# HKUST-Aerial-Robotics/MIND

Measured on AMD Instinct MI355X. Metric: sim steps/sec (whole node) + scenario-tree nodes expanded/sec, AV2 demo scenes, higher is better.
Workload: dtype f32-class (bf16 hi+mid+lo split operands = 24 significand bits, six products, fp32 accumulate) pair kernel + ActorNet, f32 elsewhere in the predictor, f64 iLQR

## Files before the change

### include/mind_hip.h

```cpp
#ifndef MIND_HIP_H
#define MIND_HIP_H

#include <stddef.h>
#include <stdint.h>

#ifdef __cplusplus
extern "C" {
#endif

#define MIND_OK 0
#define MIND_EINVAL (-1)
#define MIND_ENOMEM (-2)
#define MIND_EHIP (-3)
#define MIND_ESTATE (-4)
#define MIND_ENOTFOUND (-5)

typedef struct mind_ctx mind_ctx;

int mind_ctx_create(int device, void *stream, mind_ctx **out);
int mind_ctx_destroy(mind_ctx *ctx);
const char *mind_last_error_string(mind_ctx *ctx);
int mind_ctx_synchronize(mind_ctx *ctx);

typedef struct {
  const char *name;
  const float *data;
  int64_t numel;
} mind_tensor_desc;

int mind_weights_load(mind_ctx *ctx, const mind_tensor_desc *tensors, int n_tensors);

typedef struct {
  int n_scenes;
  const int32_t *actor_off;
  const int32_t *lane_off;
  const float *actors;
  const float *lanes;
  const float *lane_feat;
  const float *actor_ctrs;
  const float *actor_vecs;
  const float *lane_ctrs;
  const float *lane_vecs;
  const float *const *rpe;
  const float *tgt_nodes;
  const float *tgt_rpe;
} mind_scene_batch;

typedef struct {
  float *cls;
  float *reg;
  float *vel;
  float *lane_feat;
  float *actor_emb;
  float *cls_emb;
} mind_pred_out;

int mind_predict_batch(mind_ctx *ctx, const mind_scene_batch *in, mind_pred_out *out);

typedef struct {
  float *cov_vel;
  float *param;
} mind_pred_aux;
int mind_predict_batch_aux(mind_ctx *ctx, const mind_scene_batch *in, mind_pred_out *out, const mind_pred_aux *aux);

#define MIND_BASIS_BEZIER 0
#define MIND_BASIS_MONOMIAL 1
int mind_set_decoder_basis(mind_ctx *ctx, int basis);
int mind_get_decoder_basis(mind_ctx *ctx);

#define MIND_CURVE_MAX_POINTS (1LL << 26)
int mind_curve_eval(mind_ctx *ctx, int basis, const float *param, long long n_rows, const double *tau, int n_tau,
                    float *reg, float *vel, float *cov_vel);
int mind_debug_curve_basis(int basis, const double *tau, int n_tau, float *T, float *Tp);

int mind_last_fusion_stats(mind_ctx *ctx, int *n_launches, float *total_ms, double *pairs_processed);
int mind_last_actor_stats(mind_ctx *ctx, int *layerwise, int *n_launches, int *n_chunks, float *total_ms);
int mind_last_token_stats(mind_ctx *ctx, int *layerwise, int *n_launches, int *n_chunks, float *total_ms);
int mind_last_token_stage_ms(mind_ctx *ctx, float *out_ms, int cap);
int mind_last_ilqr_stats(mind_ctx *ctx, float *kernel_ms, int *n_trees, int *workgroups_per_tree);
int mind_last_ilqr_profile(mind_ctx *ctx, double *out9);
int mind_last_ilqr_trace(mind_ctx *ctx, int tree, int phase, double *out, int cap_rows, int *n_rows);
int mind_set_profiling(mind_ctx *ctx, int enable);
int mind_debug_launch_times(mind_ctx *ctx, int kind, float *clock_ms, float *event_ms, int cap, int *n_clock, int *n_event);
int mind_debug_launch_clock(int n_blocks, int block_slots, int rate_khz, const long long *ops, int n_ops, const unsigned long long *stamps,
                            long long n_slots, double *out, int cap);

#define MIND_PAIR_F32 0
#define MIND_PAIR_BF16X3 1
#define MIND_PAIR_BF16 2
#define MIND_PAIR_BF16X6 3
int mind_set_pair_precision(mind_ctx *ctx, int mode);

int mind_set_tuning(mind_ctx *ctx, const char *name, int value);
int mind_get_tuning(mind_ctx *ctx, const char *name, int *value);
int mind_debug_tuning(int index, const char *name, const char *text, int value, const char **out_name, const char **out_env, int *out_value);
int mind_debug_live_handles(void);
int mind_get_pair_precision(mind_ctx *ctx);
int mind_debug_pack_bfrag(const float *w, int row_stride, uint32_t *out);

int mind_debug_pair_schedule(const int *scene_tokens, const int *scene_actors, int n_scenes, int n_cu, int last_layer, int *out_jobs, int cap,
                             int *out_info);

int mind_debug_predict_choice(const char *const *knob_names, const int *knob_values, int n_knobs, int pair_prec, int n_cu, int have_side,
                              const int *scene_actors, const int *scene_lanes, int n_scenes, long long *out, int cap);

int mind_debug_ilqr_plan(const char *const *knob_names, const int *knob_values, int n_knobs, int n_cu, int mode, int n_trees, const int *n_nodes,
                         const int32_t *parents, long long *out, int cap, int *bad);

int mind_debug_aime_book(int pred_len, int max_depth, int max_rounds, int n_agents, int world, int rank, int force, int n_rounds, const int *dec_len,
                         const float *dec, int n_tokens, int bytes_per_pair, int plan_chunk_mb, int per_scene, long long *out, int cap, char *msg,
                         int msg_cap);

int mind_debug_wait_word(const unsigned *word, unsigned want, double timeout_s, double (*clock)(void *user), void *user, int spins_per_look);

int mind_debug_actor_lw_plan(int n_actors, int np, int chunk, long long *out_launches, int cap, long long *out_info);

int mind_debug_token_lw_plan(int n_tokens, int mode, int chunk, long long *out_launches, int cap, long long *out_info);

int mind_debug_pack_conv_frag(const float *w, int co, int ci, int ksz, uint32_t *out, size_t cap);

int mind_debug_pack(const char *what, const float *w, int a, int b, int c, float *out, size_t cap);
int mind_debug_weight_image(const mind_tensor_desc *tensors, int n_tensors, float *blob, size_t blob_cap, char *names, size_t names_cap,
                            long long *entries, int entries_cap, long long *out_info, char *msg, int msg_cap);
int mind_debug_weight_bind(const mind_tensor_desc *tensors, int n_tensors, const char *drop, char *msg, int msg_cap);

int mind_debug_trig(mind_ctx *ctx, const double *x, int n, double *out);

int mind_debug_set_layers(mind_ctx *ctx, int n);
int64_t mind_debug_read(mind_ctx *ctx, const char *name, float *host, int64_t max_floats);

typedef struct {
  int n_nodes;
  const int32_t *parent;
  const float *prob;
  int n_agents;
  const float *agent_mean;
  const float *agent_cov;
  const double *field;
  const double *node_w;
} mind_cost_tree;

typedef struct {
  double dt, wheelbase;
  double w_des_state[6];
  double w_state_con[6];
  double state_lower[6], state_upper[6];
  double w_ctrl[2];
  double w_tgt, w_ego, w_ego_cov_offset, w_exo, w_exo_cov_offset, w_exo_cost_offset;
  double grid_res; int grid_w, grid_h;
  int max_iter;
} mind_ilqr_cfg;

typedef struct { int iterations; int converged; double J; double mu; } mind_ilqr_stats;

int mind_ilqr_solve_trees(mind_ctx *ctx, const mind_ilqr_cfg *cfg, const mind_cost_tree *trees,
                          int n_trees, const double *x0, const double *target_lane, int n_lane_pts,
                          double target_vel, int use_exo, const double *us_init, double *xs,
                          double *us, mind_ilqr_stats *stats);

int mind_ilqr_contingency(mind_ctx *ctx, const mind_ilqr_cfg *cfg_warm, const mind_ilqr_cfg *cfg_full,
                          const mind_cost_tree *trees, int n_trees, const double *x0,
                          const double *target_lane, int n_lane_pts, double target_vel, double *xs,
                          double *us, mind_ilqr_stats *stats_warm, mind_ilqr_stats *stats_full);
int mind_ilqr_contingency_begin(mind_ctx *ctx, const mind_ilqr_cfg *cfg_warm, const mind_ilqr_cfg *cfg_full,
                                const mind_cost_tree *trees, int n_trees, const double *x0,
                                const double *target_lane, int n_lane_pts, double target_vel, double *xs,
                                double *us, mind_ilqr_stats *stats_warm, mind_ilqr_stats *stats_full);
int mind_ilqr_contingency_begin_plan(mind_ctx *ctx, const mind_ilqr_cfg *cfg_warm, const mind_ilqr_cfg *cfg_full, const double *x0,
                                     const double *target_lane, int n_lane_pts, double target_vel, double *xs, double *us,
                                     mind_ilqr_stats *stats_warm, mind_ilqr_stats *stats_full);
int mind_ilqr_finish(mind_ctx *ctx);

typedef struct {
  int n_scenes;
  const int32_t *actor_off;
  const float *reg, *vel;
  const float *actor_ctrs, *actor_vecs;
  const float *rot, *orig;
  const float *cov_last;
  const int32_t *last;
  const float *target_lane;
  int n_lane_pts;
  const float *cls;
  const float *scen_prob;
  int lane_check;
  float dist_thres;
} mind_world_in;

typedef struct {
  float *world;
  float *topo;
  float *ego_end;
  float *sel, *sel_prob;
} mind_world_out;

int mind_aime_world(mind_ctx *ctx, const mind_world_in *in, const mind_world_out *out);

int mind_debug_aime_decide(mind_ctx *ctx, int n_scenes, const int32_t *actor_off, const int32_t *cmp, const float *cls, const float *scen_prob,
                           const float *topo, const float *ego_end, const float *world, int lane_check, float dist_thres, float prob_floor,
                           int fused, int by_value, float *sel, float *sel_prob, uint32_t *hit);

typedef struct {
  int n_scenes, n_agents, n_lanes;
  const float *pos, *ang, *vel;
  const float *types;
  const float *pad;
  const float *lane_ctrs, *lane_vecs;
  const float *target_lane;
  const float *target_lane_info;
  int n_lane_pts;
  float time_ahead, min_vel;
// ... 303 lines not shown
```

### mind_amd/_lib.py

```python
import ctypes as C
import os

_HERE = os.path.dirname(os.path.abspath(__file__))
LIB_PATH = os.environ.get("MIND_HIP_LIB", os.path.join(_HERE, "libmind_hip.so"))

WAIT_CLOCK = C.CFUNCTYPE(C.c_double, C.c_void_p)
MIND_OK = 0
MIND_EINVAL, MIND_ENOMEM, MIND_EHIP, MIND_ESTATE, MIND_ENOTFOUND = -1, -2, -3, -4, -5


class TensorDesc(C.Structure):
    _fields_ = [("name", C.c_char_p), ("data", C.POINTER(C.c_float)), ("numel", C.c_int64)]


class SceneBatch(C.Structure):
    _fields_ = [("n_scenes", C.c_int), ("actor_off", C.POINTER(C.c_int32)), ("lane_off", C.POINTER(C.c_int32)),
                ("actors", C.c_void_p), ("lanes", C.c_void_p), ("lane_feat", C.c_void_p),
                ("actor_ctrs", C.c_void_p), ("actor_vecs", C.c_void_p), ("lane_ctrs", C.c_void_p),
                ("lane_vecs", C.c_void_p), ("rpe", C.POINTER(C.c_void_p)), ("tgt_nodes", C.c_void_p),
                ("tgt_rpe", C.c_void_p)]


class PredOut(C.Structure):
    _fields_ = [("cls", C.c_void_p), ("reg", C.c_void_p), ("vel", C.c_void_p), ("lane_feat", C.c_void_p),
# ... 117 lines not shown


class AimeNode(C.Structure):
    _fields_ = [("round", C.c_int), ("scene", C.c_int), ("mode", C.c_int), ("parent", C.c_int), ("prob", C.c_float),
                ("cur_t", C.c_int), ("end_t", C.c_int), ("flags", C.c_int), ("dur", C.c_int), ("row_off", C.c_int64),
                ("tgt_pts", C.c_float * 22)]


class AimePlanOut(C.Structure):
    _fields_ = [("nodes", C.POINTER(AimeNode)), ("n_nodes", C.c_int), ("rows", C.POINTER(C.c_float)), ("n_row_floats", C.c_int64),
                ("n_expanded", C.c_int), ("n_rounds", C.c_int), ("root_flags", C.c_int), ("round_scenes", C.c_int * 32),
                ("pair_ms", C.c_float), ("pair_launches", C.c_int), ("n_trees", C.c_int), ("tree_top", C.POINTER(C.c_int32)),
                ("tree_off", C.POINTER(C.c_int32)), ("flat_parent", C.POINTER(C.c_int32)), ("flat_prob", C.POINTER(C.c_float)),
                ("flat_mean", C.POINTER(C.c_float)), ("flat_cov", C.POINTER(C.c_float)), ("solves_begun", C.c_int)]


class IlqrCfg(C.Structure):
    _fields_ = [("dt", C.c_double), ("wheelbase", C.c_double), ("w_des_state", C.c_double * 6),
                ("w_state_con", C.c_double * 6), ("state_lower", C.c_double * 6), ("state_upper", C.c_double * 6),
                ("w_ctrl", C.c_double * 2), ("w_tgt", C.c_double), ("w_ego", C.c_double),
                ("w_ego_cov_offset", C.c_double), ("w_exo", C.c_double), ("w_exo_cov_offset", C.c_double),
                ("w_exo_cost_offset", C.c_double), ("grid_res", C.c_double), ("grid_w", C.c_int), ("grid_h", C.c_int),
                ("max_iter", C.c_int)]


class IlqrStats(C.Structure):
    _fields_ = [("iterations", C.c_int), ("converged", C.c_int), ("J", C.c_double), ("mu", C.c_double)]


LOOP_TAN_FN = C.CFUNCTYPE(C.c_double, C.c_double)
LOOP_SINCOS_FN = C.CFUNCTYPE(None, C.c_double, C.POINTER(C.c_double))


class LoopDesc(C.Structure):
    _fields_ = [("n_tracks", C.c_int), ("n_steps", C.c_int), ("clamp_last", C.c_int), ("ego_state", C.c_void_p), ("ego_state_is_f32", C.c_int), ("ego_obs", C.c_void_p), ("ego_trig32", C.c_void_p),
                ("tan_fn", C.c_void_p), ("sincos_fn", C.c_void_p), ("exo_obs", C.c_void_p),
                ("exo_valid", C.c_void_p), ("timestep", C.c_void_p), ("type_slot", C.c_void_p),
                ("sim_step", C.c_double), ("plan_step", C.c_double), ("enable_time", C.c_double),
                ("wheelbase", C.c_double), ("max_speed", C.c_double), ("max_steer", C.c_double), ("max_acc", C.c_double), ("max_dec", C.c_double),
                ("n_lanes", C.c_int), ("lane_pts", C.c_void_p), ("lane_flags", C.c_void_p),
                ("n_lane_pts", C.c_int), ("target_lane", C.c_void_p), ("target_lane_info", C.c_void_p),
                ("time_ahead", C.c_double), ("min_vel", C.c_float), ("dist_thres", C.c_float), ("max_depth", C.c_int), ("max_rounds", C.c_int),
                ("pred_len", C.c_int), ("prob_floor", C.c_float),
                ("cfg_warm", C.c_void_p), ("cfg_full", C.c_void_p), ("solve_n_lane_pts", C.c_int), ("solve_lane", C.c_void_p), ("target_vel", C.c_double),
                ("eval_n_lane_pts", C.c_int), ("eval_lane_is_f32", C.c_int), ("eval_lane", C.c_void_p), ("speculative", C.c_int)]


class LoopTotals(C.Structure):
    _fields_ = [("plans", C.c_longlong), ("expansions", C.c_longlong), ("scen_trees", C.c_longlong), ("rounds", C.c_longlong),
                ("aime_s", C.c_double), ("ilqr_s", C.c_double), ("total_s", C.c_double),
                ("iterations", C.c_longlong), ("node_iterations", C.c_longlong), ("node_iterations_exo", C.c_longlong),
                ("warm_speculated", C.c_longlong), ("warm_hits", C.c_longlong),
                ("pair_ms", C.c_double), ("pair_launches", C.c_longlong), ("scene_n2", C.c_double), ("scene_n_a1", C.c_double),
                ("ilqr_ms", C.c_double), ("ilqr_launches", C.c_longlong), ("ilqr_trees", C.c_longlong), ("ilqr_workgroups_per_tree", C.c_int),
                ("ilqr_prof", C.c_double * 9), ("ilqr_node_steps", C.c_double)]


class LoopOut(C.Structure):
    _fields_ = [("planned", C.c_int), ("enabled", C.c_int), ("n_steps", C.c_longlong), ("n_plans", C.c_longlong), ("episode_steps", C.c_longlong),
                ("sim_time", C.c_double), ("last_trigger", C.c_double), ("state", C.c_double * 4), ("ctrl", C.c_double * 2),
                ("n_agents", C.c_int), ("n_trees", C.c_int), ("best", C.c_int), ("n_expanded", C.c_int), ("n_rounds", C.c_int), ("n_traj_nodes", C.c_int),
                ("costs", C.POINTER(C.c_double)), ("aime_s", C.c_double), ("ilqr_s", C.c_double), ("total_s", C.c_double),
                ("tot", LoopTotals)]


PLANNER_EGO_KEY = -(1 << 63)


class PlannerDesc(C.Structure):
    _fields_ = [("time_ahead", C.c_double), ("min_vel", C.c_float), ("dist_thres", C.c_float), ("max_depth", C.c_int), ("max_rounds", C.c_int),
                ("pred_len", C.c_int), ("prob_floor", C.c_float), ("cfg_warm", C.c_void_p), ("cfg_full", C.c_void_p), ("speculative", C.c_int),
                ("ego_type_slot", C.c_int)]


class PlannerOut(C.Structure):
    _fields_ = [("n_plans", C.c_longlong),
                ("n_agents", C.c_int), ("n_trees", C.c_int), ("best", C.c_int), ("n_expanded", C.c_int), ("n_rounds", C.c_int), ("n_traj_nodes", C.c_int),
                ("costs", C.POINTER(C.c_double)), ("ctrl", C.c_double * 2), ("aime_s", C.c_double), ("ilqr_s", C.c_double), ("total_s", C.c_double),
                ("tot", LoopTotals)]


EXPORTS = ["mind_ctx_create", "mind_ctx_destroy", "mind_last_error_string", "mind_ctx_synchronize",
           "mind_weights_load", "mind_predict_batch", "mind_last_fusion_stats", "mind_last_actor_stats", "mind_debug_actor_lw_plan", "mind_last_token_stats", "mind_last_token_stage_ms", "mind_debug_token_lw_plan", "mind_set_profiling", "mind_debug_launch_times", "mind_debug_launch_clock",
           "mind_ilqr_solve_trees", "mind_ilqr_contingency", "mind_ilqr_solve_fields", "mind_cost_eval", "mind_ilqr_score_trees", "mind_ilqr_gains", "mind_ilqr_policy_rollouts", "mind_lane_dist_field", "mind_aime_world", "mind_aime_rebase", "mind_debug_aime_decide", "mind_debug_set_layers",
           "mind_debug_read", "mind_set_pair_precision", "mind_get_pair_precision", "mind_debug_pack_bfrag", "mind_debug_pack_conv_frag", "mind_debug_pack", "mind_debug_weight_image", "mind_debug_weight_bind", "mind_debug_pair_schedule", "mind_debug_predict_choice", "mind_debug_ilqr_plan", "mind_debug_aime_book", "mind_set_tuning", "mind_get_tuning", "mind_debug_tuning", "mind_debug_live_handles", "mind_last_ilqr_stats", "mind_aime_plan", "mind_last_ilqr_profile", "mind_eval_traj_trees", "mind_last_ilqr_trace", "mind_ilqr_contingency_begin", "mind_ilqr_finish", "mind_fill_tracks", "mind_ilqr_contingency_begin_plan", "mind_debug_trig", "mind_aime_plan_begin", "mind_aime_plan_poll", "mind_aime_plan_finish", "mind_ctx_busy", "mind_ilqr_finish_plan",
           "mind_set_exchange", "mind_last_exchange_stats", "mind_debug_wait_word",
           "mind_predict_batch_aux", "mind_set_decoder_basis", "mind_get_decoder_basis", "mind_curve_eval", "mind_debug_curve_basis",
           "mind_audit_plan", "mind_audit_episode", "mind_debug_box_clearance",
           "mind_forecast_score", "mind_debug_forecast_score",
           "mind_audit_road_plan", "mind_audit_road_episode", "mind_debug_road_margin",
           "mind_audit_ttc", "mind_debug_box_ttc",
           "mind_loop_create", "mind_loop_destroy", "mind_loop_reset", "mind_loop_advance", "mind_loop_state", "mind_loop_last_plan", "mind_loop_export",
           "mind_planner_create", "mind_planner_destroy", "mind_planner_reset", "mind_planner_observe", "mind_planner_set_lanes", "mind_planner_set_target_lane",
           "mind_planner_set_solve_lane", "mind_planner_set_eval_lane", "mind_planner_plan", "mind_planner_last_plan", "mind_planner_export"]

EXCHANGE_FN = C.CFUNCTYPE(C.c_int, C.c_void_p, C.c_int, C.c_void_p, C.c_void_p, C.c_int64)
XCHG_ALLGATHER, XCHG_ALLREDUCE, XCHG_ALLTOALLV = 0, 1, 2

_lib = None


def load():
    global _lib
    if _lib is not None:
        return _lib
    if not os.path.exists(LIB_PATH):
        raise ImportError(f"{LIB_PATH} is missing: the HIP extension must be built (hipcc --offload-arch=gfx950); "
                          "there is no CPU fallback for the product path")
    lib = C.CDLL(LIB_PATH)
    lib.mind_ctx_create.argtypes = [C.c_int, C.c_void_p, C.POINTER(C.c_void_p)]
    lib.mind_ctx_destroy.argtypes = [C.c_void_p]
    lib.mind_last_error_string.argtypes = [C.c_void_p]
    lib.mind_last_error_string.restype = C.c_char_p
    lib.mind_ctx_synchronize.argtypes = [C.c_void_p]
    lib.mind_weights_load.argtypes = [C.c_void_p, C.POINTER(TensorDesc), C.c_int]
    lib.mind_predict_batch.argtypes = [C.c_void_p, C.POINTER(SceneBatch), C.POINTER(PredOut)]
    lib.mind_predict_batch_aux.argtypes = [C.c_void_p, C.POINTER(SceneBatch), C.POINTER(PredOut), C.POINTER(PredAux)]
    lib.mind_set_decoder_basis.argtypes = [C.c_void_p, C.c_int]
    lib.mind_get_decoder_basis.argtypes = [C.c_void_p]
    lib.mind_curve_eval.argtypes = [C.c_void_p, C.c_int, C.c_void_p, C.c_longlong, C.POINTER(C.c_double), C.c_int, C.c_void_p, C.c_void_p, C.c_void_p]
    lib.mind_debug_curve_basis.argtypes = [C.c_int, C.POINTER(C.c_double), C.c_int, C.POINTER(C.c_float), C.POINTER(C.c_float)]
    lib.mind_last_fusion_stats.argtypes = [C.c_void_p, C.POINTER(C.c_int), C.POINTER(C.c_float), C.POINTER(C.c_double)]
    lib.mind_last_actor_stats.argtypes = [C.c_void_p, C.POINTER(C.c_int), C.POINTER(C.c_int), C.POINTER(C.c_int), C.POINTER(C.c_float)]
    lib.mind_debug_actor_lw_plan.argtypes = [C.c_int, C.c_int, C.c_int, C.POINTER(C.c_longlong), C.c_int, C.POINTER(C.c_longlong)]
    lib.mind_last_token_stats.argtypes = [C.c_void_p, C.POINTER(C.c_int), C.POINTER(C.c_int), C.POINTER(C.c_int), C.POINTER(C.c_float)]
    lib.mind_last_token_stage_ms.argtypes = [C.c_void_p, C.POINTER(C.c_float), C.c_int]
    lib.mind_debug_token_lw_plan.argtypes = [C.c_int, C.c_int, C.c_int, C.POINTER(C.c_longlong), C.c_int, C.POINTER(C.c_longlong)]
    lib.mind_set_profiling.argtypes = [C.c_void_p, C.c_int]
    lib.mind_debug_launch_times.argtypes = [C.c_void_p, C.c_int, C.POINTER(C.c_float), C.POINTER(C.c_float), C.c_int, C.POINTER(C.c_int), C.POINTER(C.c_int)]
    lib.mind_debug_launch_clock.argtypes = [C.c_int, C.c_int, C.c_int, C.POINTER(C.c_longlong), C.c_int, C.POINTER(C.c_ulonglong), C.c_longlong,
                                            C.POINTER(C.c_double), C.c_int]
    lib.mind_ilqr_solve_trees.argtypes = [C.c_void_p, C.POINTER(IlqrCfg), C.POINTER(CostTree), C.c_int,
                                          C.POINTER(C.c_double), C.POINTER(C.c_double), C.c_int, C.c_double, C.c_int,
                                          C.POINTER(C.c_double), C.POINTER(C.c_double), C.POINTER(C.c_double),
                                          C.POINTER(IlqrStats)]
    lib.mind_ilqr_contingency.argtypes = [C.c_void_p, C.POINTER(IlqrCfg), C.POINTER(IlqrCfg), C.POINTER(CostTree), C.c_int,
                                          C.POINTER(C.c_double), C.POINTER(C.c_double), C.c_int, C.c_double,
                                          C.POINTER(C.c_double), C.POINTER(C.c_double), C.POINTER(IlqrStats), C.POINTER(IlqrStats)]
    lib.mind_ilqr_contingency_begin.argtypes = [C.c_void_p, C.POINTER(IlqrCfg), C.POINTER(IlqrCfg), C.POINTER(CostTree), C.c_int,
                                          C.POINTER(C.c_double), C.POINTER(C.c_double), C.c_int, C.c_double,
                                          C.POINTER(C.c_double), C.POINTER(C.c_double), C.POINTER(IlqrStats), C.POINTER(IlqrStats)]
    lib.mind_ilqr_finish.argtypes = [C.c_void_p]
    lib.mind_ilqr_contingency_begin_plan.argtypes = [C.c_void_p, C.POINTER(IlqrCfg), C.POINTER(IlqrCfg), C.c_void_p, C.c_void_p, C.c_int, C.c_double,
                                                     C.c_void_p, C.c_void_p, C.c_void_p, C.c_void_p]
    lib.mind_fill_tracks.argtypes = [C.c_void_p, C.c_int, C.c_int, C.c_void_p, C.c_void_p, C.c_void_p, C.c_void_p, C.c_void_p, C.c_void_p]
    lib.mind_ilqr_solve_fields.argtypes = [C.c_void_p, C.POINTER(IlqrCfg), C.POINTER(FieldGrid), C.POINTER(CostTree), C.c_int,
                                           C.POINTER(C.c_double), C.POINTER(C.c_double), C.POINTER(C.c_double),
                                           C.POINTER(C.c_double), C.POINTER(IlqrStats)]
    lib.mind_cost_eval.argtypes = [C.c_void_p, C.POINTER(IlqrCfg), C.POINTER(FieldGrid), C.POINTER(CostTree),
                                   C.POINTER(C.c_double), C.POINTER(C.c_double), C.c_int, C.c_double, C.c_int, C.c_int,
                                   C.POINTER(C.c_int32), C.POINTER(C.c_double), C.POINTER(C.c_double), C.POINTER(C.c_double)]
    lib.mind_ilqr_score_trees.argtypes = [C.c_void_p, C.POINTER(IlqrCfg), C.POINTER(FieldGrid), C.POINTER(CostTree), C.c_int,
                                          C.POINTER(C.c_double), C.POINTER(C.c_double), C.c_int, C.c_double, C.c_int, C.c_int,
                                          C.POINTER(C.c_double), C.POINTER(C.c_double), C.POINTER(C.c_double), C.POINTER(C.c_double)]
    lib.mind_ilqr_gains.argtypes = [C.c_void_p, C.POINTER(IlqrCfg), C.POINTER(FieldGrid), C.POINTER(CostTree), C.c_int,
                                    C.POINTER(C.c_double), C.POINTER(C.c_double), C.c_int, C.c_double, C.c_int,
                                    C.POINTER(C.c_double), C.POINTER(C.c_double), C.POINTER(IlqrGainsOut)]
    lib.mind_ilqr_policy_rollouts.argtypes = [C.c_void_p, C.POINTER(IlqrCfg), C.POINTER(FieldGrid), C.POINTER(CostTree), C.c_int,
                                              C.POINTER(C.c_double), C.POINTER(C.c_double), C.c_int, C.c_double, C.c_int,
                                              C.POINTER(C.c_double), C.POINTER(C.c_double), C.POINTER(C.c_double), C.c_int,
                                              C.POINTER(C.c_double), C.POINTER(C.c_double), C.POINTER(C.c_double), C.POINTER(C.c_double),
                                              C.POINTER(C.c_double), C.POINTER(C.c_double)]
    lib.mind_lane_dist_field.argtypes = [C.c_void_p, C.POINTER(C.c_double), C.POINTER(C.c_double), C.c_int, C.c_int, C.c_int,
                                         C.c_double] + [C.POINTER(C.c_double)] * 4
    lib.mind_aime_world.argtypes = [C.c_void_p, C.POINTER(WorldIn), C.POINTER(WorldOut)]
    lib.mind_aime_rebase.argtypes = [C.c_void_p, C.POINTER(RebaseIn), C.POINTER(RebaseOut)]
    lib.mind_debug_aime_decide.argtypes = [C.c_void_p, C.c_int, C.POINTER(C.c_int32), C.POINTER(C.c_int32), C.c_void_p, C.POINTER(C.c_float), C.c_void_p,
                                           C.c_void_p, C.c_void_p, C.c_int, C.c_float, C.c_float, C.c_int, C.c_int, C.c_void_p, C.c_void_p, C.c_void_p]
    lib.mind_aime_plan.argtypes = [C.c_void_p, C.POINTER(AimePlanIn), C.POINTER(AimePlanOut)]
    lib.mind_aime_plan_begin.argtypes = [C.c_void_p, C.POINTER(AimePlanIn)]
    lib.mind_aime_plan_poll.argtypes = [C.c_void_p]
    lib.mind_aime_plan_finish.argtypes = [C.c_void_p, C.POINTER(AimePlanOut)]
    lib.mind_ctx_busy.argtypes = [C.c_void_p]
    lib.mind_ilqr_finish_plan.argtypes = [C.c_void_p, C.c_int, C.c_int, C.c_void_p, C.c_void_p, C.c_void_p, C.c_void_p]
    lib.mind_set_pair_precision.argtypes = [C.c_void_p, C.c_int]
    lib.mind_set_tuning.argtypes = [C.c_void_p, C.c_char_p, C.c_int]
    lib.mind_get_tuning.argtypes = [C.c_void_p, C.c_char_p, C.POINTER(C.c_int)]
    lib.mind_debug_tuning.argtypes = [C.c_int, C.c_char_p, C.c_char_p, C.c_int, C.POINTER(C.c_char_p), C.POINTER(C.c_char_p), C.POINTER(C.c_int)]
    lib.mind_debug_live_handles.argtypes = []
    lib.mind_last_ilqr_stats.argtypes = [C.c_void_p, C.POINTER(C.c_float), C.POINTER(C.c_int), C.POINTER(C.c_int)]
    lib.mind_last_ilqr_profile.argtypes = [C.c_void_p, C.POINTER(C.c_double)]
    lib.mind_last_ilqr_trace.argtypes = [C.c_void_p, C.c_int, C.c_int, C.POINTER(C.c_double), C.c_int, C.POINTER(C.c_int)]
    lib.mind_eval_traj_trees.argtypes = [C.POINTER(C.c_double), C.POINTER(C.c_double), C.POINTER(C.c_int32), C.c_int, C.c_void_p, C.c_int, C.c_int,
                                         C.c_double, C.POINTER(C.c_double)]
    lib.mind_get_pair_precision.argtypes = [C.c_void_p]
    lib.mind_debug_pack_bfrag.argtypes = [C.POINTER(C.c_float), C.c_int, C.POINTER(C.c_uint32)]
    lib.mind_debug_pair_schedule.argtypes = [C.POINTER(C.c_int), C.POINTER(C.c_int), C.c_int, C.c_int, C.c_int, C.POINTER(C.c_int), C.c_int, C.POINTER(C.c_int)]
    lib.mind_debug_predict_choice.argtypes = [C.POINTER(C.c_char_p), C.POINTER(C.c_int), C.c_int, C.c_int, C.c_int, C.c_int, C.POINTER(C.c_int), C.POINTER(C.c_int),
                                              C.c_int, C.POINTER(C.c_longlong), C.c_int]
    lib.mind_debug_ilqr_plan.argtypes = [C.POINTER(C.c_char_p), C.POINTER(C.c_int), C.c_int, C.c_int, C.c_int, C.c_int, C.POINTER(C.c_int), C.POINTER(C.c_int32),
                                         C.POINTER(C.c_longlong), C.c_int, C.POINTER(C.c_int)]
    lib.mind_debug_wait_word.argtypes = [C.POINTER(C.c_uint), C.c_uint, C.c_double, WAIT_CLOCK, C.c_void_p, C.c_int]
    lib.mind_debug_aime_book.argtypes = [C.c_int] * 8 + [C.POINTER(C.c_int), C.POINTER(C.c_float)] + [C.c_int] * 4 + [C.POINTER(C.c_longlong), C.c_int, C.c_char_p, C.c_int]
    lib.mind_debug_trig.argtypes = [C.c_void_p, C.POINTER(C.c_double), C.c_int, C.POINTER(C.c_double)]
    lib.mind_debug_pack_conv_frag.argtypes = [C.POINTER(C.c_float), C.c_int, C.c_int, C.c_int, C.POINTER(C.c_uint32), C.c_size_t]
    lib.mind_debug_pack.argtypes = [C.c_char_p, C.POINTER(C.c_float), C.c_int, C.c_int, C.c_int, C.POINTER(C.c_float), C.c_size_t]
    lib.mind_debug_weight_image.argtypes = [C.POINTER(TensorDesc), C.c_int, C.POINTER(C.c_float), C.c_size_t, C.c_char_p, C.c_size_t,
                                            C.POINTER(C.c_longlong), C.c_int, C.POINTER(C.c_longlong), C.c_char_p, C.c_int]
    lib.mind_debug_weight_bind.argtypes = [C.POINTER(TensorDesc), C.c_int, C.c_char_p, C.c_char_p, C.c_int]
    lib.mind_debug_set_layers.argtypes = [C.c_void_p, C.c_int]
    lib.mind_debug_read.argtypes = [C.c_void_p, C.c_char_p, C.POINTER(C.c_float), C.c_int64]
    lib.mind_set_exchange.argtypes = [C.c_void_p, C.c_int, C.c_int, EXCHANGE_FN, C.c_void_p, C.c_int]
    lib.mind_last_exchange_stats.argtypes = [C.c_void_p, C.POINTER(C.c_longlong), C.POINTER(C.c_longlong)]
    lib.mind_loop_create.argtypes = [C.c_void_p, C.POINTER(LoopDesc), C.POINTER(C.c_void_p)]
    lib.mind_loop_destroy.argtypes = [C.c_void_p]
    lib.mind_loop_reset.argtypes = [C.c_void_p]
    lib.mind_loop_advance.argtypes = [C.c_void_p, C.c_int, C.c_double, C.c_longlong, C.POINTER(LoopOut)]
    lib.mind_loop_state.argtypes = [C.c_void_p, C.POINTER(LoopOut)]
    lib.mind_loop_last_plan.argtypes = [C.c_void_p, C.POINTER(AimePlanOut)] + [C.POINTER(C.c_void_p)] * 6 + [C.c_void_p]
    lib.mind_loop_export.argtypes = [C.c_void_p, C.c_int, C.POINTER(C.c_int), C.c_void_p, C.c_void_p, C.c_void_p]
    lib.mind_planner_create.argtypes = [C.c_void_p, C.POINTER(PlannerDesc), C.POINTER(C.c_void_p)]
    lib.mind_planner_destroy.argtypes = [C.c_void_p]
    lib.mind_planner_reset.argtypes = [C.c_void_p]
    lib.mind_planner_observe.argtypes = [C.c_void_p, C.c_int, C.c_void_p, C.c_int, C.c_void_p, C.c_void_p, C.c_void_p]
    lib.mind_planner_set_lanes.argtypes = [C.c_void_p, C.c_int, C.c_void_p, C.c_void_p]
    lib.mind_planner_set_target_lane.argtypes = [C.c_void_p, C.c_int, C.c_void_p, C.c_void_p]
    lib.mind_planner_set_solve_lane.argtypes = [C.c_void_p, C.c_int, C.c_void_p, C.c_double]
    lib.mind_planner_set_eval_lane.argtypes = [C.c_void_p, C.c_int, C.c_void_p, C.c_int]
    lib.mind_planner_plan.argtypes = [C.c_void_p, C.c_void_p, C.c_void_p, C.POINTER(PlannerOut)]
    lib.mind_planner_last_plan.argtypes = [C.c_void_p, C.POINTER(AimePlanOut)] + [C.POINTER(C.c_void_p)] * 6 + [C.c_void_p]
    lib.mind_planner_export.argtypes = [C.c_void_p, C.c_int, C.POINTER(C.c_int), C.c_void_p, C.c_void_p, C.c_void_p]
    lib.mind_audit_plan.argtypes = [C.c_void_p, C.POINTER(AuditBox), C.c_double, C.POINTER(CostTree), C.c_int, C.c_int, C.POINTER(C.c_double),
                                    C.POINTER(AuditPlanOut)]
    lib.mind_audit_episode.argtypes = [C.c_void_p, C.POINTER(AuditBox), C.c_int, C.c_int, C.c_int, C.POINTER(C.c_double), C.POINTER(C.c_double),
                                       C.POINTER(C.c_uint8), C.POINTER(C.c_double), C.POINTER(AuditEpisodeOut)]
    lib.mind_debug_box_clearance.argtypes = [C.c_int, C.c_int, C.POINTER(C.c_double), C.POINTER(C.c_double), C.POINTER(C.c_double), C.POINTER(C.c_double)]
    fc_tail = [C.POINTER(ForecastCfg), C.c_int, C.POINTER(C.c_int32), C.c_void_p, C.c_void_p, C.POINTER(C.c_double), C.POINTER(C.c_uint8),
               C.POINTER(C.c_uint8), C.POINTER(ForecastOut)]
    lib.mind_forecast_score.argtypes = [C.c_void_p] + fc_tail
    lib.mind_debug_forecast_score.argtypes = fc_tail
    road = [C.POINTER(C.c_double), C.POINTER(C.c_int32), C.c_int]
    lib.mind_audit_road_plan.argtypes = [C.c_void_p, C.POINTER(AuditBox)] + road + [C.POINTER(CostTree), C.c_int, C.c_int, C.POINTER(C.c_double),
                                                                                   C.POINTER(AuditRoadPlanOut)]
    lib.mind_audit_road_episode.argtypes = [C.c_void_p, C.POINTER(AuditBox)] + road + [C.c_int, C.c_int, C.POINTER(C.c_double),
                                                                                      C.POINTER(AuditRoadEpisodeOut)]
    lib.mind_debug_road_margin.argtypes = [C.c_int, C.POINTER(C.c_double), C.POINTER(AuditBox)] + road + [C.POINTER(C.c_double), C.POINTER(C.c_double)] + \
        [C.POINTER(C.c_int32)] * 3
    lib.mind_audit_ttc.argtypes = [C.c_void_p, C.POINTER(AuditBox), C.POINTER(AuditTtcCfg), C.c_int, C.c_int, C.c_int, C.POINTER(C.c_double),
                                   C.POINTER(C.c_double), C.POINTER(C.c_uint8), C.POINTER(C.c_double), C.POINTER(AuditTtcOut)]
    lib.mind_debug_box_ttc.argtypes = [C.c_int, C.POINTER(C.c_double), C.POINTER(C.c_double), C.POINTER(C.c_double), C.POINTER(C.c_double)]
    for n in EXPORTS:
        getattr(lib, n)
        if n not in ("mind_last_error_string", "mind_debug_read"):
            getattr(lib, n).restype = C.c_int
    lib.mind_debug_read.restype = C.c_int64
    _lib = lib
    return lib


PRED_CHOICE_FIELDS = ("header", "n_runs", "np", "actor_form", "actor_arg", "actor_grid", "actor_chunk", "actor_chunks", "actor_launches", "qsplit", "qk_stride",
                      "tiled", "edge_bf16", "edge_pair_bytes", "tok_chunk", "tok_lw", "tok_chunks", "pair_family", "pair_np", "l5_jobs5", "xcd_lanes",
                      "xcd_lanes5", "dec_actor", "dec_np", "fp32_dec", "split_dec", "want_mw", "mw_blocks", "cls_on_side", "tgt_wait_first",
                      "dec_head_ra")
PAIR_PREC = ("f32", "bf16x3", "bf16", "bf16x6")


def predict_choice(knobs, prec, scenes, n_cu=256, have_side=True):
    lib = load()
    names = (C.c_char_p * max(1, len(knobs)))(*[k.encode() for k in knobs])
    vals = (C.c_int * max(1, len(knobs)))(*[int(v) for v in knobs.values()])
    sa = (C.c_int * len(scenes))(*[a for a, _ in scenes])
    sl = (C.c_int * len(scenes))(*[l for _, l in scenes])
    cap = 32 + 6 * len(scenes)
    out = (C.c_longlong * cap)()
    n = lib.mind_debug_predict_choice(names, vals, len(knobs), PAIR_PREC.index(prec) if isinstance(prec, str) else prec, n_cu, int(have_side),
                                      sa, sl, len(scenes), out, cap)
    if n == MIND_EINVAL:
        return None
    assert 0 < n <= cap and out[0] == 32 and n == 32 + 6 * out[1], n
    d = dict(zip(PRED_CHOICE_FIELDS, out[:31]))
    d["runs"] = [tuple(out[32 + 6 * i:38 + 6 * i]) for i in range(out[1])]
    return d


def knobs():
    lib = load()
    name, env, val = C.c_char_p(), C.c_char_p(), C.c_int()
    rows = []
    while not rows or len(rows) < n:
        n = lib.mind_debug_tuning(len(rows), None, None, 0, C.byref(name), C.byref(env), C.byref(val))
        assert n > 0, n
        rows.append((name.value.decode(), env.value.decode() if env.value else None, val.value))
    return rows


def knob_stored(name, value=None, text=None):
    val = C.c_int()
    rc = load().mind_debug_tuning(-1, name.encode(), None if text is None else text.encode(), 0 if value is None else int(value), None, None, C.byref(val))
    return val.value if rc == MIND_OK else None


ILQR_PLAN_FIELDS = ("header", "n_trees", "form", "G", "GS", "spec", "nslot", "grid", "workgroups_per_tree", "host_out", "early", "starve_followers")
ILQR_TREE_FIELDS = ("M", "nl", "nseg", "nsl", "maxls", "nfs")
ILQR_TREE_TABLES = ("level_start", "level_nodes", "child_start", "child_list", "seg_start", "seg_nodes", "slevel_start", "slevel_segs", "seg_rec",
                    "fstep_start", "fstep_items", "fstep_q1", "fstep_nstart", "fstep_nodes")


def ilqr_plan(knobs, parents, n_cu=256, generic=False, evaluate=False, two_fits=False):
    lib = load()
    names = (C.c_char_p * max(1, len(knobs)))(*[k.encode() for k in knobs])
    vals = (C.c_int * max(1, len(knobs)))(*[int(v) for v in knobs.values()])
    nn = (C.c_int * len(parents))(*[len(p) for p in parents])
    flat = [int(v) for p in parents for v in p]
    par = (C.c_int32 * max(1, len(flat)))(*flat)
    bad = (C.c_int * 2)()
    mode = int(generic) | int(evaluate) << 1 | int(two_fits) << 2
    n = lib.mind_debug_ilqr_plan(names, vals, len(knobs), n_cu, mode, len(parents), nn, par, None, 0, bad)
    if n == MIND_EINVAL:
        return {"bad": (bad[0], bad[1])} if bad[0] >= 0 else None
    out = (C.c_longlong * n)()
    assert lib.mind_debug_ilqr_plan(names, vals, len(knobs), n_cu, mode, len(parents), nn, par, out, n, bad) == n and out[0] == 16
    d = dict(zip(ILQR_PLAN_FIELDS, out[:12]))
    d["trees"], o = [], 16
    for _ in parents:
        tr = dict(zip(ILQR_TREE_FIELDS, out[o:o + 6]))
        lens, o = out[o + 6:o + 20], o + 20
        for name, ln in zip(ILQR_TREE_TABLES, lens):
            tr[name], o = list(out[o:o + ln]), o + ln
        d["trees"].append(tr)
    assert o == n
    return d


AIME_ROUND_FIELDS = ("B", "lo", "hi", "Bmax", "chunk", "S", "s0", "Sm", "any")
AIME_NODE_FIELDS = ("round", "scene", "mode", "parent", "prob", "cur_t", "end_t", "flags", "dur", "row_off", "owner", "lscene")


def aime_book(pred_len, max_depth, n_agents, rounds, world=1, rank=0, force=False, max_rounds=32, n_tokens=0, bytes_per_pair=512, plan_chunk_mb=96 * 1024,
              per_scene=1):
    import numpy as np
    lib = load()
    arrs = [np.ascontiguousarray(r, np.float32).ravel() for r in rounds]
    lens = (C.c_int * max(1, len(arrs)))(*[a.size for a in arrs])
    dec = np.concatenate(arrs + [np.zeros(1, np.float32)])
    msg = C.create_string_buffer(256)
    args = [pred_len, max_depth, max_rounds, n_agents, world, rank, int(force), len(arrs), lens, dec.ctypes.data_as(C.POINTER(C.c_float)), n_tokens,
            bytes_per_pair, plan_chunk_mb, per_scene]
    n = lib.mind_debug_aime_book(*args, None, 0, msg, 256)
    if n == MIND_EINVAL:
        return None
    out = (C.c_longlong * n)()
    assert lib.mind_debug_aime_book(*args, out, n, msg, 256) == n and out[0] == 16
    o, take = [16], lambda k: (list(out[o[0]:o[0] + k]), o.__setitem__(0, o[0] + k))[0]
    d = dict(code=out[1], error=msg.value.decode() if out[1] else None, args=(out[2], out[3]), n_rows=out[8], root_flags=out[9], rounds=[])
    for _ in range(out[4]):
        r = dict(zip(AIME_ROUND_FIELDS, take(9)))
        for k, ln in (("todo", r["S"]), ("cnt_r", world), ("s0_r", world + 1), ("win", 3 * r["Sm"]), ("tab", 2 * world), ("snd", 2 * world), ("rcv", 2 * world)):
            r[k] = take(ln)
        d["rounds"].append(r)
    if not out[1]:
        d["nodes"] = [dict(zip(AIME_NODE_FIELDS, take(12))) for _ in range(out[5])]
        for name in ("gather", "flat"):
            nj, nb, nbytes = take(3)
            d[name] = dict(jobs=[tuple(take(5)) for _ in range(nj)], job_of_block=take(nb), agent_of_block=take(nb), bytes=nbytes)
        d["tree_top"], d["tree_off"], d["flat_parent"], d["flat_prob"] = take(out[6]), take(out[6] + 1), take(out[7]), take(out[7])
    assert o[0] == n
    return d


def tensor_descs(sd):
    import numpy as np
    descs = (TensorDesc * max(1, len(sd)))()
    keep = []
    for i, (k, v) in enumerate(sd.items()):
        a = np.ascontiguousarray(v.detach().cpu().numpy() if hasattr(v, "detach") else np.asarray(v), dtype=np.float32)
        keep.append(a)
        descs[i].name = k.encode()
        descs[i].data = a.ctypes.data_as(C.POINTER(C.c_float))
        descs[i].numel = a.size
    return descs, keep


def weight_image(sd):
    import numpy as np
    lib = load()
    descs, keep = tensor_descs(sd)
    msg = C.create_string_buffer(256)
    info = (C.c_longlong * 3)()
    rc = lib.mind_debug_weight_image(descs, len(sd), None, 0, None, 0, None, 0, info, msg, 256)
    if rc == MIND_ENOTFOUND:
        raise KeyError(msg.value.decode())
    assert rc == MIND_OK, rc
    ne, nf, nb = info
    blob, names, ents = np.zeros(nf, np.float32), C.create_string_buffer(nb), (C.c_longlong * (2 * ne))()
    assert lib.mind_debug_weight_image(descs, len(sd), blob.ctypes.data_as(C.POINTER(C.c_float)), nf, names, nb, ents, ne, info, msg, 256) == MIND_OK
    keys = names.value.decode().split("\n")[:-1]
    assert len(keys) == ne
    return blob, [(k, ents[2 * i], ents[2 * i + 1]) for i, k in enumerate(keys)]


def curve_basis(basis, tau):
    import numpy as np
    lib = load()
    tau = np.ascontiguousarray(tau, np.float64).ravel()
    b = BASIS.index(basis) if isinstance(basis, str) else int(basis)
    T, Tp = np.zeros((max(1, tau.size), 8), np.float32), np.zeros((max(1, tau.size), 7), np.float32)
    rc = lib.mind_debug_curve_basis(b, tau.ctypes.data_as(C.POINTER(C.c_double)), tau.size, T.ctypes.data_as(C.POINTER(C.c_float)),
                                    Tp.ctypes.data_as(C.POINTER(C.c_float)))
    if rc == MIND_EINVAL:
        raise ValueError(f"mind_debug_curve_basis rejects basis {basis!r}, tau {tau!r}")
    assert rc == MIND_OK, rc
    return T[:tau.size], Tp[:tau.size]

# ... 161 lines not shown
```

### mind_amd/csrc/ilqr_choice.h

```cpp
#pragma once
#include <algorithm>
#include <cstdint>
#include <cstring>
#include <vector>

#include "tuning.h"

struct IlqrChoice {
  int form = 0;
  int G = 1, GS = 1, spec = 0;
  int nslot = IL_SPEC;
  int grid = 0;
  int wgs_per_tree = 1;
  bool host_out = false;
  bool early = false;
  bool starve_followers = false;
};

static IlqrChoice il_choose(const IlqrTuning &t, int n_cu, int n_trees, int max_nodes, long total_nodes, bool gen, bool eval) {
  IlqrChoice ch;
  const int blocks8 = ((n_trees + 7) / 8) * 8;
  int G = t.ilqr_wgs;
  if (G > 1 && G < t.ilqr_wgs_big && max_nodes >= t.ilqr_big_min) G = t.ilqr_wgs_big;
  while (G > 1 && blocks8 * G > n_cu) G >>= 1;
  const bool multi = !gen && !eval && G > 1 && max_nodes >= t.ilqr_multi_min;
  int GS = (multi || gen || eval || t.ilqr_wgs <= 1) ? 1 : t.ilqr_slots;
  while (GS > 1 && blocks8 * GS > n_cu) --GS;
  const bool slots = GS > 1;
  ch.form = multi ? 1 : slots ? 2 : 0;
  ch.G = multi ? G : 1;
  ch.GS = GS;
  ch.spec = slots && t.ilqr_spec_deriv && GS < 31 && blocks8 * (GS + 1) <= n_cu ? 1 : 0;
  ch.nslot = slots ? std::max(GS, IL_SPEC) : IL_SPEC;
  ch.grid = ch.form == 2 ? blocks8 * (GS + ch.spec) : ch.form == 1 ? blocks8 * G - (t.ilqr_test_starve ? 8 : 0) : n_trees;
  ch.wgs_per_tree = ch.form == 1 ? G : ch.form == 2 ? GS + ch.spec : 1;
  ch.starve_followers = ch.form == 2 && t.ilqr_test_starve;
  ch.host_out = !eval && t.ilqr_host_out_max > 0 && total_nodes <= t.ilqr_host_out_max;
  ch.early = ch.host_out && !multi && !gen;
  return ch;
}

static int il_score_block(const IlqrTuning &t, int n_cu, int n_trees, int n_cand) {
  if (t.ilqr_score_block > 0) return t.ilqr_score_block;
  int cb = 64;
  while (cb > 4 && (long)n_trees * ((n_cand + cb - 1) / cb) < 2L * n_cu) cb >>= 1;
  return cb;
}

struct IlTables {
  std::vector<int> lvl_start, lvl_nodes;
  std::vector<int> child_start, child_list;
  std::vector<int> seg_start, seg_nodes;
  std::vector<int> slvl_start, slvl_segs;
  std::vector<int> seg_rec;
  std::vector<int> fs_start, fs_items, fs_q1, fs_nstart, fs_nodes;
  int nl = 0, nseg = 0, nsl = 0, maxls = 0, nfs = 0;
  std::vector<int> depth, fill, child_fill, seg_of, seg_depth, slvl_fill;
};

static int il_tree_tables(const int32_t *parent, int M, int ilqr_chunk, IlTables &out) {
  IlTables &T = out;
  T.depth.assign(M, 0);
  int maxd = 0;
  for (int i = 0; i < M; ++i) {
    const int p = parent[i];
    if (i == 0 ? p != -1 : (p < 0 || p >= i)) return i;
    T.depth[i] = i == 0 ? 0 : T.depth[p] + 1;
    maxd = std::max(maxd, T.depth[i]);
  }
  T.nl = maxd + 1;
  T.lvl_start.assign(maxd + 2, 0);
  for (int i = 0; i < M; ++i) T.lvl_start[T.depth[i] + 1]++;
  for (int d = 0; d <= maxd; ++d) T.lvl_start[d + 1] += T.lvl_start[d];
  T.lvl_nodes.resize(M);
  T.fill.assign(maxd + 1, 0);
  for (int i = 0; i < M; ++i) T.lvl_nodes[T.lvl_start[T.depth[i]] + T.fill[T.depth[i]]++] = i;
  T.child_start.assign(M + 1, 0);
  for (int i = 1; i < M; ++i) T.child_start[parent[i] + 1]++;
  for (int i = 0; i < M; ++i) T.child_start[i + 1] += T.child_start[i];
  T.child_list.assign(M > 1 ? M : 1, 0);
  T.child_fill.assign(M, 0);
  for (int i = 1; i < M; ++i) T.child_list[T.child_start[parent[i]] + T.child_fill[parent[i]]++] = i;
  const auto nchild = [&T](int i) { return T.child_start[i + 1] - T.child_start[i]; };
  T.seg_of.assign(M, -1); T.seg_depth.clear();
  T.seg_start.clear(); T.seg_nodes.clear();
  for (int i = 0; i < M; ++i) {
    if (!(i == 0 || nchild(parent[i]) >= 2)) continue;
    const int sidx = (int)T.seg_start.size();
    T.seg_start.push_back((int)T.seg_nodes.size());
    T.seg_depth.push_back(i == 0 ? 0 : T.seg_depth[T.seg_of[parent[i]]] + 1);
    for (int n = i;; n = T.child_list[T.child_start[n]]) {
      T.seg_of[n] = sidx;
      T.seg_nodes.push_back(n);
      if (nchild(n) != 1) break;
    }
  }
  T.seg_start.push_back((int)T.seg_nodes.size());
  const int nseg = (int)T.seg_depth.size();
  int maxsd = 0;
  for (int d : T.seg_depth) maxsd = std::max(maxsd, d);
  T.slvl_start.assign(maxsd + 2, 0);
  for (int d : T.seg_depth) T.slvl_start[d + 1]++;
  for (int d = 0; d <= maxsd; ++d) T.slvl_start[d + 1] += T.slvl_start[d];
  T.slvl_segs.resize(nseg);
  T.slvl_fill.assign(maxsd + 1, 0);
  for (int s = 0; s < nseg; ++s) T.slvl_segs[T.slvl_start[T.seg_depth[s]] + T.slvl_fill[T.seg_depth[s]]++] = s;
  T.nseg = nseg; T.nsl = maxsd + 1;
  T.maxls = 1;
  for (int d = 0; d <= maxsd; ++d) T.maxls = std::max(T.maxls, T.slvl_start[d + 1] - T.slvl_start[d]);
  T.seg_rec.assign((size_t)nseg * 16, 0);
  for (int s = 0; s < nseg; ++s) {
    int *r = T.seg_rec.data() + (size_t)s * 16;
    const int s0 = T.seg_start[s], s1 = T.seg_start[s + 1], last = T.seg_nodes[s1 - 1];
    r[0] = s0; r[1] = s1; r[2] = last; r[3] = T.seg_nodes[s0]; r[4] = T.seg_nodes[s1 - 2 >= s0 ? s1 - 2 : s1 - 1];
    r[5] = nchild(last); r[6] = T.child_start[last];
    for (int e = 0; e < 6 && e < r[5]; ++e) r[8 + e] = T.child_list[T.child_start[last] + e];
  }
  const int chunk = (ilqr_chunk > 0 && T.maxls <= 6) ? ilqr_chunk : M;
  T.fs_start.assign(1, 0); T.fs_nstart.assign(1, 0);
  T.fs_items.clear(); T.fs_q1.clear(); T.fs_nodes.clear();
  for (int d = 0; d <= maxsd; ++d) {
    int maxlen = 0;
    for (int e = T.slvl_start[d]; e < T.slvl_start[d + 1]; ++e) { const int s = T.slvl_segs[e]; maxlen = std::max(maxlen, T.seg_start[s + 1] - T.seg_start[s]); }
    for (int k0 = 0; k0 < maxlen; k0 += chunk) {
      for (int e = T.slvl_start[d]; e < T.slvl_start[d + 1]; ++e) {
        const int s = T.slvl_segs[e], q0 = T.seg_start[s] + k0, q1 = std::min(T.seg_start[s + 1], q0 + chunk);
        if (q0 >= q1) continue;
        const int c0 = T.seg_nodes[q0], c1 = T.seg_nodes[q0 + 1 < q1 ? q0 + 1 : q1 - 1];
        for (int v : {q0, q1, c0, c1, c0 == 0 ? -1 : (int)parent[c0], 0, 0, 0}) T.fs_items.push_back(v);
        T.fs_q1.push_back(q1);
        for (int q = q0; q < q1; ++q) T.fs_nodes.push_back(T.seg_nodes[q]);
      }
      T.fs_start.push_back((int)T.fs_q1.size()); T.fs_nstart.push_back((int)T.fs_nodes.size());
    }
  }
  T.nfs = (int)T.fs_start.size() - 1;
  return -1;
}

struct IlTreeOff {
  size_t us, nodew, xs, stats, trace;
  size_t relag, Fx, L, Lx, Lxx, relag2, Fx2, L2, Lx2, Lxx2;
  size_t k, K, Vx, Vxx, xsn, usn, Ln;
  size_t prob, mean, cov;
  size_t parent, lnodes, cstart, clist, rel, rel2, lstart, sstart, snodes, slstart, slsegs, segrec, fsstart, fsitems, fsq1, fsnstart, fsnodes;
  size_t field;
};
struct IlArena {
  size_t nd = 0, nf = 0, ni = 0, nd_in = 0;
  size_t o_gx, o_gy, o_lane, o_evx, o_evu, o_quad, o_evo;
  size_t o_scu, o_scx, o_scl, o_scj;
  size_t o_gmu, o_gk, o_gK, o_gdv, o_gvx, o_gvxx, o_gxs, o_gl, o_gj, o_gbad;
  size_t o_pk, o_pK, o_pal, o_pdx, o_pxn, o_pxs, o_pus, o_pl, o_pj;
  size_t o_evn, o_bars, o_ctl, ctl_ints;
  size_t bytesIn, bytesF, bytesI, o_structs, o_consts, o_work, total;
  std::vector<IlTreeOff> tree;
  size_t takeD(size_t n) { const size_t o = nd; nd += (n + 1) & ~(size_t)1; return o; }
  size_t takeF(size_t n) { const size_t o = nf; nf += (n + 3) & ~(size_t)3; return o; }
  size_t takeI(size_t n) { const size_t o = ni; ni += (n + 3) & ~(size_t)3; return o; }
};
struct IlShape {
  int W, H, n_lane_pts, nq;
  int n_trees;
  const int *n_agents;
  bool gen, use_exo, dev_flat;
  int trace_cap;
  int n_cand = 0;
  bool gains = false;
  int n_pol = 0, n_pol_blk = 0;
};

static void il_layout(const IlShape &s, const IlqrChoice &ch, const IlTables *tab, IlArena &A) {
  const int n_trees = s.n_trees;
  const bool spec = ch.spec != 0;
  const size_t nslot = (size_t)ch.nslot;
  A = IlArena();
  A.tree.resize(n_trees);
  const auto nodes = [tab](int t) { return tab[t].lvl_nodes.size(); };
  A.o_gx = A.takeD(s.W); A.o_gy = A.takeD(s.H); A.o_lane = A.takeD((size_t)s.n_lane_pts * 2 + 2);
  A.o_evx = A.takeD((size_t)s.nq * 6); A.o_evu = A.takeD((size_t)s.nq * 2);
  A.o_evn = A.takeI(s.nq);
  A.o_bars = A.takeI(4 * (size_t)n_trees + 4);
  A.ctl_ints = (sizeof(IlSlotCtl) + 15) / 16 * 4;
  A.o_ctl = A.takeI(ch.form == 2 ? A.ctl_ints * (size_t)n_trees : 0);
  for (int t = 0; t < n_trees; ++t) A.tree[t].us = A.takeD(2 * nodes(t));
  for (int t = 0; t < n_trees; ++t) A.tree[t].nodew = A.takeD(s.gen ? nodes(t) * IL_NW : 0);
  size_t Mtot = 0;
  for (int t = 0; t < n_trees; ++t) Mtot += nodes(t);
  const size_t n_sc = (size_t)s.n_cand * Mtot;
  A.o_scu = A.takeD(2 * n_sc);
  const size_t n_g = s.gains ? Mtot : 0, n_gt = s.gains ? (size_t)n_trees : 0, n_pm = s.n_pol > 0 ? Mtot : 0, n_po = (size_t)s.n_pol * Mtot;
  A.o_gmu = A.takeD(n_gt);
  A.o_pk = A.takeD(2 * n_pm); A.o_pK = A.takeD(12 * n_pm); A.o_pal = A.takeD((size_t)s.n_pol); A.o_pdx = A.takeD(6 * (size_t)s.n_pol);
  A.nd_in = A.nd;
  A.o_quad = A.takeD(s.gen ? 2 : (size_t)s.W * s.H); A.o_evo = A.takeD((size_t)s.nq * IL_EVAL_OUT);
  for (int t = 0; t < n_trees; ++t) A.tree[t].xs = A.takeD(6 * nodes(t));
  for (int t = 0; t < n_trees; ++t) A.tree[t].stats = A.takeD(2 * IL_NSTAT);
  for (int t = 0; t < n_trees; ++t) {
    IlTreeOff &L = A.tree[t];
    const size_t M = nodes(t), a = (size_t)s.n_agents[t];
    L.trace = A.takeD((size_t)2 * s.trace_cap * IL_TRACE_W);
    L.relag = A.takeD(s.use_exo ? M * IL_RA : 0); L.Fx = A.takeD(36 * M); L.L = A.takeD(M); L.Lx = A.takeD(6 * M); L.Lxx = A.takeD(36 * M);
    L.relag2 = A.takeD(spec && s.use_exo ? M * IL_RA : 0); L.Fx2 = A.takeD(spec ? 36 * M : 0); L.L2 = A.takeD(spec ? M : 0); L.Lx2 = A.takeD(spec ? 6 * M : 0);
    L.Lxx2 = A.takeD(spec ? 36 * M : 0);
    L.k = A.takeD(nslot * 2 * M); L.K = A.takeD(nslot * 12 * M); L.Vx = A.takeD(nslot * 6 * M); L.Vxx = A.takeD(nslot * 36 * M);
    L.xsn = A.takeD(nslot * 60 * M); L.usn = A.takeD(nslot * 20 * M); L.Ln = A.takeD(nslot * 10 * M);
    L.prob = A.takeF(M); L.mean = A.takeF(s.dev_flat ? 0 : M * a * 2); L.cov = A.takeF(s.dev_flat ? 0 : M * a);
    L.parent = A.takeI(M); L.lnodes = A.takeI(M); L.cstart = A.takeI(M + 1); L.clist = A.takeI(M); L.rel = A.takeI(M); L.rel2 = A.takeI(spec ? M : 0);
  }
  for (int t = 0; t < n_trees; ++t) {
    IlTreeOff &L = A.tree[t];
    const IlTables &T = tab[t];
    L.lstart = A.takeI(T.lvl_start.size());
    L.sstart = A.takeI(T.seg_start.size()); L.snodes = A.takeI(nodes(t)); L.slstart = A.takeI(T.slvl_start.size()); L.slsegs = A.takeI(T.slvl_segs.size());
    L.segrec = A.takeI(T.seg_rec.size());
    L.fsstart = A.takeI(T.fs_start.size()); L.fsitems = A.takeI(T.fs_items.size()); L.fsq1 = A.takeI(T.fs_q1.size());
    L.fsnstart = A.takeI(T.fs_nstart.size()); L.fsnodes = A.takeI(nodes(t));
  }
  A.o_scx = A.takeD(6 * n_sc); A.o_scl = A.takeD(n_sc); A.o_scj = A.takeD((size_t)s.n_cand * n_trees);
  A.o_gk = A.takeD(2 * n_g); A.o_gK = A.takeD(12 * n_g); A.o_gdv = A.takeD(n_g); A.o_gvx = A.takeD(6 * n_g); A.o_gvxx = A.takeD(36 * n_g);
  A.o_gxs = A.takeD(6 * n_g); A.o_gl = A.takeD(n_g); A.o_gj = A.takeD(n_gt); A.o_gbad = A.takeD(n_gt);
  A.o_pxn = A.takeD(6 * (size_t)s.n_pol_blk * n_pm); A.o_pxs = A.takeD(6 * n_po); A.o_pus = A.takeD(2 * n_po); A.o_pl = A.takeD(n_po);
  A.o_pj = A.takeD((size_t)s.n_pol * (s.n_pol > 0 ? n_trees : 0));
  A.bytesIn = A.nd_in * sizeof(double); A.bytesF = A.nf * sizeof(float); A.bytesI = A.ni * sizeof(int);
  A.o_structs = A.bytesIn + A.bytesF + A.bytesI;
  A.o_consts = (A.o_structs + (size_t)n_trees * sizeof(IlqrTreeDev) + 15) & ~(size_t)15;
  A.o_work = (A.o_consts + 2 * sizeof(IlqrConst) + 15) & ~(size_t)15;
  A.total = (A.o_work + (A.nd - A.nd_in) * sizeof(double) + 15) & ~(size_t)15;
  for (int t = 0; t < n_trees; ++t) {
    A.tree[t].field = A.total;
    if (s.gen) A.total += nodes(t) * s.W * s.H * sizeof(double);
  }
}

static void il_stage_ints(const IlTreeOff &L, const int32_t *parent, const IlTables &T, int *hI) {
  const auto put = [hI](size_t o, const std::vector<int> &v) { if (!v.empty()) memcpy(hI + o, v.data(), v.size() * sizeof(int)); };
  memcpy(hI + L.parent, parent, T.lvl_nodes.size() * sizeof(int));
  put(L.lstart, T.lvl_start); put(L.lnodes, T.lvl_nodes); put(L.cstart, T.child_start); put(L.clist, T.child_list);
  put(L.sstart, T.seg_start); put(L.snodes, T.seg_nodes); put(L.slstart, T.slvl_start); put(L.slsegs, T.slvl_segs); put(L.segrec, T.seg_rec);
  put(L.fsstart, T.fs_start); put(L.fsitems, T.fs_items); put(L.fsq1, T.fs_q1); put(L.fsnstart, T.fs_nstart); put(L.fsnodes, T.fs_nodes);
}
```

### mind_amd/csrc/ilqr_host.hip

```cpp
static void il_make_grid(int W, int H, double res, const double *ego_xy, double *gx, double *gy, double &offx, double &offy) {
  const double fsx = (double)(W - 1) * res, fsy = (double)(H - 1) * res;
  offx = ego_xy[0] - 0.5 * fsx; offy = ego_xy[1] - 0.5 * fsy;
  const double sx = fsx / (double)(W - 1), sy = fsy / (double)(H - 1);
  for (int i = 0; i < W; ++i) gx[i] = (double)i * sx + 0.0;
  gx[W - 1] = fsx;
  for (int i = 0; i < H; ++i) gy[i] = (double)i * sy + 0.0;
  gy[H - 1] = fsy;
  for (int i = 0; i < W; ++i) gx[i] += offx;
  for (int i = 0; i < H; ++i) gy[i] += offy;
}

extern "C" int mind_lane_dist_field(mind_ctx *c, const double *ego_xy, const double *lane, int n_pts, int W, int H,
                                    double res, double *offset, double *gx, double *gy, double *dist) {
  if (!c || !ego_xy || !lane || n_pts < 2 || W < 2 || H < 2 || !(res > 0) || !offset || !gx || !gy || !dist)
    return fail(c, MIND_EINVAL, "mind_lane_dist_field: bad argument");
  HIPCHK(c, hipSetDevice(c->device));
  hipStream_t st = c->stream;
  il_make_grid(W, H, res, ego_xy, gx, gy, offset[0], offset[1]);
  const size_t nd = (size_t)W + H + 2 * (size_t)n_pts + (size_t)W * H;
  int rc;
  if ((rc = ensure(c, c->ilqr_dev, nd * sizeof(double)))) return rc;
  double *d = (double *)c->ilqr_dev.p;
  HIPCHK(c, hipMemcpyAsync(d, gx, W * sizeof(double), hipMemcpyHostToDevice, st));
  HIPCHK(c, hipMemcpyAsync(d + W, gy, H * sizeof(double), hipMemcpyHostToDevice, st));
// ... 236 lines not shown

static int il_stage(mind_ctx *c, IlRun &R) {
  const IlqrCall &q = R.q;
  const IlArena &A = R.A;
  const IlqrChoice &ch = R.ch;
  const IlqrEvalReq *ev = q.ev;
  const int n_trees = q.n_trees;
  const bool gen = R.gen;
  int rc;
  if ((rc = ensure(c, c->ilqr_dev, A.total))) return rc;
  R.base = (char *)c->ilqr_dev.p;
  auto &hD = c->il_img.hD; auto &hF = c->il_img.hF; auto &hI = c->il_img.hI;
  hD.assign(A.nd_in, 0.0); hF.assign(A.nf, 0.f); hI.assign(A.ni, 0);
  memcpy(hD.data() + A.o_gx, R.gx.data(), R.W * sizeof(double));
  memcpy(hD.data() + A.o_gy, R.gy.data(), R.H * sizeof(double));
  if (R.n_lane_pts) memcpy(hD.data() + A.o_lane, q.lane, (size_t)R.n_lane_pts * 2 * sizeof(double));
  if (ev) {
    memcpy(hD.data() + A.o_evx, ev->x, (size_t)ev->nq * 6 * sizeof(double));
    memcpy(hD.data() + A.o_evu, ev->u, (size_t)ev->nq * 2 * sizeof(double));
    memcpy(hI.data() + A.o_evn, ev->node, (size_t)ev->nq * sizeof(int));
  }
  if (q.sc) memcpy(hD.data() + A.o_scu, q.sc->us_cand, (size_t)q.sc->n_cand * (size_t)R.Mtot * 2 * sizeof(double));
  if (q.ga) memcpy(hD.data() + A.o_gmu, q.ga->mu, (size_t)n_trees * sizeof(double));
  if (q.po) {
    const IlqrPolicyReq *po = q.po;
    memcpy(hD.data() + A.o_pk, po->k, (size_t)R.Mtot * 2 * sizeof(double));
    memcpy(hD.data() + A.o_pK, po->K, (size_t)R.Mtot * 12 * sizeof(double));
    memcpy(hD.data() + A.o_pal, po->alpha, (size_t)po->n_cand * sizeof(double));
    if (po->dx0) memcpy(hD.data() + A.o_pdx, po->dx0, (size_t)po->n_cand * 6 * sizeof(double));
  }
  const IlTreeOff &L0 = A.tree[0];
  R.n_xs = L0.stats - L0.xs;
  R.n_hx = R.n_xs + (size_t)2 * IL_NSTAT * n_trees; R.n_us = (size_t)R.Mtot * 2;
  if ((rc = pl_pin(c, 5, (R.n_hx + R.n_us + 2) * sizeof(double) + (size_t)n_trees * sizeof(unsigned)))) return rc;
  R.hx = c->pl_pin[5].as<double>(); R.hus = R.hx + R.n_hx;
  R.h_abort = (unsigned *)(R.hus + R.n_us);
  R.h_done = R.h_abort + 4;
  c->il_early = mind_ctx::IlEarly();
  if (ch.early) {
    c->il_gen += 1u;
    if (c->il_gen == 0u) c->il_gen = 1u;
    for (int t = 0; t < n_trees; ++t) R.h_done[t] = 0u;
    c->il_early.xs = R.hx; c->il_early.us = R.hus; c->il_early.done = R.h_done; c->il_early.gen = c->il_gen; c->il_early.n_trees = n_trees; c->il_early.nodes = R.Mtot;
  }
  float *dF = R.dF();
  int *dI = R.dI();
  R.hT.resize(n_trees);
  long moff = 0;
  for (int t = 0; t < n_trees; ++t) {
    const mind_cost_tree &tr = q.trees[t];
    const IlTreeOff &L = A.tree[t];
    const IlTables &T = c->il_tab[t];
    const size_t M = tr.n_nodes, a = R.n_agents[t];
    if (q.us_init) memcpy(hD.data() + L.us, q.us_init + moff * 2, 2 * M * sizeof(double));
    if (tr.prob) memcpy(hF.data() + L.prob, tr.prob, M * sizeof(float));
    if (gen) memcpy(hD.data() + L.nodew, tr.node_w, M * IL_NW * sizeof(double));
    if (tr.agent_mean && !gen && !R.dev_flat) memcpy(hF.data() + L.mean, tr.agent_mean, M * a * 2 * sizeof(float));
    if (tr.agent_cov && !gen && !R.dev_flat) memcpy(hF.data() + L.cov, tr.agent_cov, M * a * sizeof(float));
    il_stage_ints(L, tr.parent, T, hI.data());
    IlqrTreeDev &D = R.hT[t];
    D.M = tr.n_nodes; D.n_agents = (int)a; D.n_levels = T.nl; D.pad = 0;
    D.parent = dI + L.parent; D.level_start = dI + L.lstart; D.level_nodes = dI + L.lnodes;
    D.child_start = dI + L.cstart; D.child_list = dI + L.clist;
    D.rel = dI + L.rel;
    D.relag = R.Dp(L.relag);
    D.field = gen ? (const double *)(R.base + L.field) : nullptr;
    D.node_w = gen ? R.Dp(L.nodew) : nullptr;
    D.n_segs = T.nseg; D.n_slevels = T.nsl; D.max_level_segs = T.maxls; D.pad2 = 0;
    D.seg_start = dI + L.sstart; D.seg_nodes = dI + L.snodes; D.slevel_start = dI + L.slstart; D.slevel_segs = dI + L.slsegs; D.seg_rec = dI + L.segrec;
    D.n_fsteps = T.nfs; D.padf = 0;
    D.trace = R.trace_cap > 0 ? R.Dp(L.trace) : nullptr; D.trace_cap = R.trace_cap; D.padt = 0;
    D.fstep_start = dI + L.fsstart; D.fstep_q0 = dI + L.fsitems; D.fstep_q1 = dI + L.fsq1; D.fstep_nstart = dI + L.fsnstart; D.fstep_nodes = dI + L.fsnodes;
    D.prob = dF + L.prob; D.mean = dF + L.mean; D.cov = dF + L.cov;
    if (R.dev_flat) { D.mean = c->plan.dev_fmean + (size_t)moff * a * 2; D.cov = c->plan.dev_fcov + (size_t)moff * a; }
    D.xs = R.Dp(L.xs); D.us = R.Dp(L.us); D.Fx = R.Dp(L.Fx); D.L = R.Dp(L.L); D.Lx = R.Dp(L.Lx); D.Lxx = R.Dp(L.Lxx);
    D.k = R.Dp(L.k); D.K = R.Dp(L.K); D.Vx = R.Dp(L.Vx); D.Vxx = R.Dp(L.Vxx);
    D.xs_new = R.Dp(L.xsn); D.us_new = R.Dp(L.usn); D.L_new = R.Dp(L.Ln); D.stats = R.Dp(L.stats);
    D.ctl = ch.form == 2 ? (IlSlotCtl *)(dI + A.o_ctl + A.ctl_ints * (size_t)t) : nullptr;
    D.h_xs = ch.host_out ? R.hx + (L.xs - L0.xs) : nullptr; D.h_us = ch.host_out ? R.hus + (L.us - L0.us) : nullptr;
    D.h_stats = ch.host_out ? R.hx + (L.stats - L0.xs) : nullptr;
    D.h_done = ch.early ? R.h_done + t : nullptr; D.h_gen = c->il_gen; D.pad_h = 0;
    if (ch.early && ((L.xs - L0.xs) != (size_t)moff * 6 || (L.us - L0.us) != (size_t)moff * 2)) return fail(c, MIND_EINVAL, "tree-iLQR arena: results are not contiguous");
    D.dset = ch.spec ? (long long)L.Fx2 - (long long)L.Fx : 0; D.drel = ch.spec ? (long long)L.rel2 - (long long)L.rel : 0;
    if (ch.spec && (L.L2 - L.L != L.Fx2 - L.Fx || L.Lx2 - L.Lx != L.Fx2 - L.Fx || L.Lxx2 - L.Lxx != L.Fx2 - L.Fx || (R.use_exo && L.relag2 - L.relag != L.Fx2 - L.Fx)))
      return fail(c, MIND_EINVAL, "tree-iLQR arena: the two derivative sets are laid out differently");
    moff += (long)M;
  }
  R.field_ahead = !gen && !ev && !q.sc && !q.ga && !q.po && c->il_field_valid && c->il_field_key[0] == q.x0[0] && c->il_field_key[1] == q.x0[1] && c->il_field_key[2] == (double)R.W &&
                  c->il_field_key[3] == (double)R.H && c->il_field_key[4] == R.grid_res && c->il_field_lane.size() == 2 * (size_t)R.n_lane_pts &&
                  memcmp(c->il_field_lane.data(), q.lane, c->il_field_lane.size() * sizeof(double)) == 0;
  c->il_field_valid = false;
  double *quad = R.field_ahead ? (double *)c->il_field.p + (size_t)R.W + R.H + 2 * (size_t)R.n_lane_pts : R.Dp(A.o_quad);
  il_fill_const(R.K[0], q.cfg, R.use_exo_first, R, quad);
  if (q.cfg2) il_fill_const(R.K[1], q.cfg2, 1, R, quad);
  else R.K[1] = R.K[0];
  {
    const auto off = [&R](size_t o) { return (size_t)((const char *)R.Dp(o) - R.base); };
    c->il_dbg[0] = off(L0.L); c->il_dbg[1] = off(L0.Lx); c->il_dbg[2] = off(L0.Lxx); c->il_dbg[3] = off(L0.Fx); c->il_dbg[4] = off(L0.xs);
    c->il_dbg[5] = (size_t)q.trees[0].n_nodes;
  }
  return MIND_OK;
}

static int il_upload(mind_ctx *c, IlRun &R, hipStream_t st) {
  const IlArena &A = R.A;
  const int n_trees = R.q.n_trees;
  for (int t = 0; t < n_trees && R.gen; ++t)
    HIPCHK(c, hipMemcpyAsync(R.base + A.tree[t].field, R.q.trees[t].field, (size_t)R.q.trees[t].n_nodes * R.W * R.H * sizeof(double), hipMemcpyHostToDevice, st));
  int rc;
  if ((rc = pl_pin(c, 4, A.o_work))) return rc;
  char *up = c->pl_pin[4].as<char>();
  memset(up, 0, A.o_work);
  memcpy(up, c->il_img.hD.data(), A.bytesIn);
  if (A.bytesF) memcpy(up + A.bytesIn, c->il_img.hF.data(), A.bytesF);
  if (A.bytesI) memcpy(up + A.bytesIn + A.bytesF, c->il_img.hI.data(), A.bytesI);
  if (R.ch.starve_followers) ((unsigned *)(up + A.bytesIn + A.bytesF))[A.o_bars + 4 * (size_t)n_trees + 1] = 1u;
  memcpy(up + A.o_structs, R.hT.data(), (size_t)n_trees * sizeof(IlqrTreeDev));
  memcpy(up + A.o_consts, R.K, 2 * sizeof(IlqrConst));
  R.up = up;
  return pl_upload(c, R.base, up, A.o_work, st);
}

struct IlPending {
  hipStream_t st;
  bool gen;
  int n_trees, n_phases, use_exo, trace_cap;
  long Mtot;
  IlqrChoice ch;
  const IlqrTreeDev *dT;
  const IlqrConst *dK;
  unsigned *dBars;
  size_t il_lds, o_work;
  char *base;
  const char *up;
  const double *d_xs, *d_us;
  double *hx, *hus;
  const unsigned *h_abort;
  size_t n_xs, n_hx, n_us;
  double *xs, *us;
  mind_ilqr_stats *stats, *stats2;
  struct Tree { int M, nl, nseg, nsl, maxls, a; const double *trace; };
  std::vector<Tree> tree;
};

static void il_launch_kernel(const IlPending &P, int form) {
  const IlqrChoice &ch = P.ch;
  const int nt = P.n_trees;
  const dim3 block(IL_THREADS);
  if (P.gen) hipLaunchKernelGGL((k_ilqr<true, 0>), dim3(nt), block, P.il_lds, P.st, P.dT, P.dK, P.n_phases, nt, 1, P.dBars, 0);
  else if (form == 2) hipLaunchKernelGGL((k_ilqr<false, 2>), dim3(ch.grid), block, P.il_lds, P.st, P.dT, P.dK, P.n_phases, nt, ch.GS, P.dBars, ch.spec);
  else if (form == 1) hipLaunchKernelGGL((k_ilqr<false, 1>), dim3(ch.grid), block, P.il_lds, P.st, P.dT, P.dK, P.n_phases, nt, ch.G, P.dBars, 0);
  else hipLaunchKernelGGL((k_ilqr<false, 0>), dim3(nt), block, P.il_lds, P.st, P.dT, P.dK, P.n_phases, nt, 1, P.dBars, 0);
}

static int il_read_back(mind_ctx *c, const IlPending &P) {
  if (P.ch.host_out) return MIND_OK;
  HIPCHK(c, hipMemcpyAsync(P.hx, P.d_xs, P.n_hx * sizeof(double), hipMemcpyDeviceToHost, P.st));
  HIPCHK(c, hipMemcpyAsync(P.hus, P.d_us, P.n_us * sizeof(double), hipMemcpyDeviceToHost, P.st));
  return MIND_OK;
}

static int il_finish_run(mind_ctx *c, const IlPending &P) {
  static const bool trace = getenv("MIND_ILQR_TRACE") != nullptr;
  const int n_trees = P.n_trees, n_phases = P.n_phases;
  int rc;
  HIPCHK(c, hipStreamSynchronize(P.st));
  if (c->profiling) HIPCHK(c, hipEventElapsedTime(&c->ilqr_ms, c->ev_il0, c->ev_il1));
  if (P.ch.form == 1 && *P.h_abort) {
    c->n_ilqr_fallbacks++;
    HIPCHK(c, hipMemcpyAsync(P.base, P.up, P.o_work, hipMemcpyHostToDevice, P.st));
    il_launch_kernel(P, 0);
    HIPCHK(c, hipGetLastError());
    c->ilqr_multi = 1;
    if ((rc = il_read_back(c, P))) return rc;
    HIPCHK(c, hipStreamSynchronize(P.st));
  }
  memcpy(P.xs, P.hx, (size_t)P.Mtot * 6 * sizeof(double));
  memcpy(P.us, P.hus, P.n_us * sizeof(double));
  const auto hstat = [&P](int t, int ph) { return P.hx + P.n_xs + (size_t)2 * IL_NSTAT * t + (size_t)ph * IL_NSTAT; };
  c->il_trace_dev.assign(n_trees, nullptr);
  c->il_trace_its.assign((size_t)2 * n_trees, 0);
  c->il_trace_cap = P.trace_cap; c->il_trace_phases = n_phases;
  for (int t = 0; t < n_trees; ++t) {
    c->il_trace_dev[t] = P.trace_cap > 0 ? P.tree[t].trace : nullptr;
    for (int ph = 0; ph < n_phases; ++ph) c->il_trace_its[2 * t + ph] = (int)hstat(t, ph)[0];
  }
  c->il_spec_req = 0; c->il_spec_hit = 0;
#ifndef IL_PROFILE
  for (int t = 0; t < n_trees; ++t)
    for (int ph = 0; ph < n_phases; ++ph) { c->il_spec_req += (long long)hstat(t, ph)[9]; c->il_spec_hit += (long long)hstat(t, ph)[10]; }
#endif
  double best = -1.0;
  for (int t = 0; t < n_trees; ++t) {
    double tot = 0.0, ph_c[5] = {0, 0, 0, 0, 0}, passes = 0.0;
    for (int ph = 0; ph < n_phases; ++ph) {
      const double *h = hstat(t, ph);
      ph_c[0] += h[4]; ph_c[1] += h[5]; ph_c[2] += h[8]; ph_c[3] += h[6]; ph_c[4] += h[7];
      passes += h[IL_NSTAT - 1];
    }
    for (double v : ph_c) tot += v;
    if (tot > best) {
      best = tot;
      double *o = c->il_prof;
      o[0] = P.tree[t].M; o[1] = P.tree[t].nl; o[2] = passes;
      for (int k = 0; k < 5; ++k) o[3 + k] = ph_c[k];
      o[8] = (double)n_trees;
    }
  }
  for (int ph = 0; ph < n_phases; ++ph) {
    mind_ilqr_stats *so = ph == 0 ? P.stats : P.stats2;
    if (!so) continue;
    for (int t = 0; t < n_trees; ++t) {
      const double *h = hstat(t, ph);
      const IlPending::Tree &T = P.tree[t];
      so[t].iterations = (int)h[0]; so[t].converged = (int)h[1];
      so[t].J = h[2]; so[t].mu = h[3];
      if (!trace) continue;
      fprintf(stderr, "[k_ilqr] tree %d exo %d M %d segs %d seg-levels %d widest %d agents %d it %d passes %.0f: cycles derivatives %.0f backward %.0f state chain %.0f cost pass %.0f select %.0f\n", t,
              n_phases == 2 ? ph : P.use_exo, T.M, T.nseg, T.nsl, T.maxls, T.a, so[t].iterations, h[IL_NSTAT - 1], h[4], h[5], h[8], h[6], h[7]);
#ifdef IL_PROFILE
      fprintf(stderr, "[k_ilqr prof] wave0: chain node (n=%.0f): stage %.0f u+dyn+store %.0f | cost chunk (n=%.0f): stage+loads %.0f field %.0f cost+store %.0f | riccati node (n=%.0f): products %.0f Qxx %.0f solve %.0f update %.0f | deriv block (n=%.0f): setup %.0f tasks %.0f assemble %.0f\n",
              h[13], h[8] / fmax(h[13], 1), h[9] / fmax(h[13], 1),
              h[23], h[10] / fmax(h[23], 1), h[11] / fmax(h[23], 1), h[12] / fmax(h[23], 1),
              h[18], h[14] / fmax(h[18], 1), h[15] / fmax(h[18], 1), h[16] / fmax(h[18], 1), h[17] / fmax(h[18], 1),
              h[22], h[19] / fmax(h[22], 1), h[20] / fmax(h[22], 1), h[21] / fmax(h[22], 1));
#endif
    }
  }
  return MIND_OK;
}

static int il_eval(mind_ctx *c, const IlRun &R, hipStream_t st) {
  const IlqrEvalReq *ev = R.q.ev;
  const IlArena &A = R.A;
  const IlqrTreeDev *dT = (const IlqrTreeDev *)(R.base + A.o_structs);
  const size_t lds = (IL_SCR + (size_t)4 * R.amax) * sizeof(double);
  if (R.gen) hipLaunchKernelGGL(k_cost_eval<true>, dim3(ev->nq), dim3(64), lds, st, dT, R.K[0], ev->nq, R.dI() + A.o_evn, R.Dp(A.o_evx), R.Dp(A.o_evu), R.Dp(A.o_evo));
  else hipLaunchKernelGGL(k_cost_eval<false>, dim3(ev->nq), dim3(64), lds, st, dT, R.K[0], ev->nq, R.dI() + A.o_evn, R.Dp(A.o_evx), R.Dp(A.o_evu), R.Dp(A.o_evo));
  HIPCHK(c, hipGetLastError());
  HIPCHK(c, hipMemcpyAsync(ev->out, R.Dp(A.o_evo), (size_t)ev->nq * IL_EVAL_OUT * sizeof(double), hipMemcpyDeviceToHost, st));
  HIPCHK(c, hipStreamSynchronize(st));
  return MIND_OK;
}

static int il_score(mind_ctx *c, const IlRun &R, hipStream_t st) {
  const IlqrScoreReq *sc = R.q.sc;
  const IlArena &A = R.A;
  const int n_trees = R.q.n_trees;
  const IlqrTreeDev *dT = (const IlqrTreeDev *)(R.base + A.o_structs);
  const int cb = il_score_block(c->it, c->n_cu, n_trees, sc->n_cand);
  const dim3 grid((sc->n_cand + cb - 1) / cb, n_trees), block(IL_SC_THREADS);
  const size_t lds = il_score_lds_bytes(R.amax);
  const size_t rows = (size_t)sc->n_cand * (size_t)R.Mtot;
  if (R.gen) hipLaunchKernelGGL(k_ilqr_score<true>, grid, block, lds, st, dT, R.K[0], n_trees, sc->n_cand, cb, R.Mtot, il_ag_doubles(R.amax), R.Dp(A.o_scu), R.Dp(A.o_scx), R.Dp(A.o_scl), R.Dp(A.o_scj));
  else hipLaunchKernelGGL(k_ilqr_score<false>, grid, block, lds, st, dT, R.K[0], n_trees, sc->n_cand, cb, R.Mtot, il_ag_doubles(R.amax), R.Dp(A.o_scu), R.Dp(A.o_scx), R.Dp(A.o_scl), R.Dp(A.o_scj));
  HIPCHK(c, hipGetLastError());
  if (sc->xs) HIPCHK(c, hipMemcpyAsync(sc->xs, R.Dp(A.o_scx), rows * 6 * sizeof(double), hipMemcpyDeviceToHost, st));
  if (sc->L) HIPCHK(c, hipMemcpyAsync(sc->L, R.Dp(A.o_scl), rows * sizeof(double), hipMemcpyDeviceToHost, st));
  HIPCHK(c, hipMemcpyAsync(sc->J, R.Dp(A.o_scj), (size_t)sc->n_cand * n_trees * sizeof(double), hipMemcpyDeviceToHost, st));
  HIPCHK(c, hipStreamSynchronize(st));
  return MIND_OK;
}

static int il_gains(mind_ctx *c, const IlRun &R, hipStream_t st) {
  const mind_ilqr_gains_out *o = R.q.ga->out;
  const IlArena &A = R.A;
  const int n_trees = R.q.n_trees;
  const IlqrTreeDev *dT = (const IlqrTreeDev *)(R.base + A.o_structs);
  const size_t lds = il_gains_lds_bytes(R.amax), M = (size_t)R.Mtot;
  if (R.gen) hipLaunchKernelGGL(k_ilqr_gains<true>, dim3(n_trees), dim3(IL_PG_THREADS), lds, st, dT, R.K[0], n_trees, il_ag_doubles(R.amax), R.Dp(A.o_gmu), R.Dp(A.o_gk), R.Dp(A.o_gK), R.Dp(A.o_gdv), R.Dp(A.o_gvx), R.Dp(A.o_gvxx), R.Dp(A.o_gxs), R.Dp(A.o_gl), R.Dp(A.o_gj), R.Dp(A.o_gbad));
  else hipLaunchKernelGGL(k_ilqr_gains<false>, dim3(n_trees), dim3(IL_PG_THREADS), lds, st, dT, R.K[0], n_trees, il_ag_doubles(R.amax), R.Dp(A.o_gmu), R.Dp(A.o_gk), R.Dp(A.o_gK), R.Dp(A.o_gdv), R.Dp(A.o_gvx), R.Dp(A.o_gvxx), R.Dp(A.o_gxs), R.Dp(A.o_gl), R.Dp(A.o_gj), R.Dp(A.o_gbad));
  HIPCHK(c, hipGetLastError());
  const size_t span = A.o_gbad + (size_t)n_trees - A.o_gk;
  int rc;
  if ((rc = pl_pin(c, 5, span * sizeof(double)))) return rc;
  const double *h = c->pl_pin[5].as<double>();
  HIPCHK(c, hipMemcpyAsync(c->pl_pin[5], R.Dp(A.o_gk), span * sizeof(double), hipMemcpyDeviceToHost, st));
  HIPCHK(c, hipStreamSynchronize(st));
  const struct { double *dst; size_t src, n; } outs[8] = {{o->k, A.o_gk, 2 * M}, {o->K, A.o_gK, 12 * M}, {o->dV, A.o_gdv, M}, {o->V_x, A.o_gvx, 6 * M},
                                                          {o->V_xx, A.o_gvxx, 36 * M}, {o->xs, A.o_gxs, 6 * M}, {o->L, A.o_gl, M}, {o->J, A.o_gj, (size_t)n_trees}};
  for (const auto &e : outs)
    if (e.dst) memcpy(e.dst, h + (e.src - A.o_gk), e.n * sizeof(double));
  for (int t = 0; t < n_trees; ++t) o->bad_node[t] = (int32_t)h[A.o_gbad - A.o_gk + t];
  return MIND_OK;
}

static int il_policy(mind_ctx *c, const IlRun &R, hipStream_t st, int cb) {
  const IlqrPolicyReq *po = R.q.po;
  const IlArena &A = R.A;
  const int n_trees = R.q.n_trees;
  const IlqrTreeDev *dT = (const IlqrTreeDev *)(R.base + A.o_structs);
  const dim3 grid((po->n_cand + cb - 1) / cb, n_trees), block(IL_SC_THREADS);
  const size_t lds = il_score_lds_bytes(R.amax);
  const size_t rows = (size_t)po->n_cand * (size_t)R.Mtot;
  if (R.gen) hipLaunchKernelGGL(k_ilqr_policy<true>, grid, block, lds, st, dT, R.K[0], n_trees, po->n_cand, cb, R.Mtot, il_ag_doubles(R.amax), R.Dp(A.o_pk), R.Dp(A.o_pK), R.Dp(A.o_pal), R.Dp(A.o_pdx), R.Dp(A.o_pxn), R.Dp(A.o_pxs), R.Dp(A.o_pus), R.Dp(A.o_pl), R.Dp(A.o_pj));
  else hipLaunchKernelGGL(k_ilqr_policy<false>, grid, block, lds, st, dT, R.K[0], n_trees, po->n_cand, cb, R.Mtot, il_ag_doubles(R.amax), R.Dp(A.o_pk), R.Dp(A.o_pK), R.Dp(A.o_pal), R.Dp(A.o_pdx), R.Dp(A.o_pxn), R.Dp(A.o_pxs), R.Dp(A.o_pus), R.Dp(A.o_pl), R.Dp(A.o_pj));
  HIPCHK(c, hipGetLastError());
  if (po->xs) HIPCHK(c, hipMemcpyAsync(po->xs, R.Dp(A.o_pxs), rows * 6 * sizeof(double), hipMemcpyDeviceToHost, st));
  if (po->us_out) HIPCHK(c, hipMemcpyAsync(po->us_out, R.Dp(A.o_pus), rows * 2 * sizeof(double), hipMemcpyDeviceToHost, st));
  if (po->L) HIPCHK(c, hipMemcpyAsync(po->L, R.Dp(A.o_pl), rows * sizeof(double), hipMemcpyDeviceToHost, st));
  HIPCHK(c, hipMemcpyAsync(po->J, R.Dp(A.o_pj), (size_t)po->n_cand * n_trees * sizeof(double), hipMemcpyDeviceToHost, st));
  HIPCHK(c, hipStreamSynchronize(st));
  return MIND_OK;
}

static int il_launch(mind_ctx *c, const IlRun &R, hipStream_t st, IlPending &P) {
  const IlqrCall &q = R.q;
  const IlArena &A = R.A;
  const IlqrChoice &ch = R.ch;
  const int n_trees = q.n_trees;
  if (R.field_ahead) HIPCHK(c, hipStreamWaitEvent(st, c->ev_field, 0));
  else if (!R.gen) hipLaunchKernelGGL(k_lane_field, dim3((R.W * R.H + 255) / 256), dim3(256), 0, st, R.K[0].gx.p, R.K[0].gy.p, R.W, R.H, R.Dp(A.o_lane), R.n_lane_pts, R.Dp(A.o_quad));
  if (q.ev) return il_eval(c, R, st);
  if (q.sc) return il_score(c, R, st);
  if (q.ga) return il_gains(c, R, st);
  if (q.po) return il_policy(c, R, st, R.pol_cb);
  P.st = st; P.gen = R.gen; P.n_trees = n_trees; P.n_phases = R.n_phases; P.use_exo = R.use_exo; P.trace_cap = R.trace_cap; P.Mtot = R.Mtot; P.ch = ch;
  P.dT = (const IlqrTreeDev *)(R.base + A.o_structs); P.dK = (const IlqrConst *)(R.base + A.o_consts);
  P.dBars = (unsigned *)(R.dI() + A.o_bars);
  P.il_lds = il_lds_bytes(R.amax); P.o_work = A.o_work; P.base = R.base; P.up = R.up;
  P.d_xs = R.Dp(A.tree[0].xs); P.d_us = R.Dp(A.tree[0].us);
  P.hx = R.hx; P.hus = R.hus; P.h_abort = R.h_abort; P.n_xs = R.n_xs; P.n_hx = R.n_hx; P.n_us = R.n_us;
  P.xs = q.xs; P.us = q.us; P.stats = q.stats; P.stats2 = q.stats2;
  P.tree.resize(n_trees);
  for (int t = 0; t < n_trees; ++t) {
    const IlTables &T = c->il_tab[t];
    P.tree[t] = {q.trees[t].n_nodes, T.nl, T.nseg, T.nsl, T.maxls, R.n_agents[t], R.Dp(A.tree[t].trace)};
  }
  if (c->profiling) {
    if (!c->ev_il0) { HIPCHK(c, c->ev_il0.create()); HIPCHK(c, c->ev_il1.create()); }
    HIPCHK(c, hipEventRecord(c->ev_il0, st));
  }
  c->ilqr_trees = n_trees; c->ilqr_multi = ch.wgs_per_tree; c->ilqr_ms = 0.f;
  il_launch_kernel(P, ch.form);
  HIPCHK(c, hipGetLastError());
  if (c->profiling) HIPCHK(c, hipEventRecord(c->ev_il1, st));
  int rc;
  if ((rc = il_read_back(c, P))) return rc;
  if (ch.form == 1) HIPCHK(c, hipMemcpyAsync(R.h_abort, P.dBars + 4 * (size_t)n_trees, sizeof(unsigned), hipMemcpyDeviceToHost, st));
  return MIND_OK;
}

static int il_solve(mind_ctx *c, const IlqrCall &q) {
  IlRun R(q);
  int rc;
  if ((rc = il_check(c, q, R))) return rc;
  HIPCHK(c, hipSetDevice(c->device));
  hipStream_t st = c->stream;
  IlStamp stamp;
  il_grid(R);
  int maxM = 0;
  for (int t = 0; t < q.n_trees; ++t) maxM = std::max(maxM, q.trees[t].n_nodes);
  const bool other = q.ev || q.sc || q.ga || q.po;
  R.ch = il_choose(c->it, c->n_cu, q.n_trees, maxM, R.Mtot, R.gen, other);
  if ((rc = il_build_tables(c, q))) return rc;
  IlShape shape{R.W, R.H, R.n_lane_pts, q.ev ? q.ev->nq : 0, q.n_trees, R.n_agents.data(), R.gen, R.use_exo != 0, R.dev_flat, R.trace_cap, q.sc ? q.sc->n_cand : 0};
  shape.gains = q.ga != nullptr;
  if (q.po) {
    R.pol_cb = il_score_block(c->it, c->n_cu, q.n_trees, q.po->n_cand);
    shape.n_pol = q.po->n_cand; shape.n_pol_blk = (q.po->n_cand + R.pol_cb - 1) / R.pol_cb;
  }
  il_layout(shape, R.ch, c->il_tab.data(), R.A);
  stamp("tables built");
  if ((rc = il_stage(c, R))) return rc;
  stamp("staged in vectors");
  if ((rc = il_upload(c, R, st))) return rc;
  stamp("upload queued");
  IlPending P;
  if ((rc = il_launch(c, R, st, P)) || other) return rc;
  stamp("kernel launched");
  if (!q.begin_only) return il_finish_run(c, P);
  c->il_finish = [c, P = std::move(P)]() { return il_finish_run(c, P); };
  return MIND_OK;
}

static IlqrCall il_contingency_call(const mind_ilqr_cfg *cfg_warm, const mind_ilqr_cfg *cfg_full, const mind_cost_tree *trees, int n_trees, const double *x0,
                                    const double *target_lane, int n_lane_pts, double target_vel, double *xs, double *us, mind_ilqr_stats *stats_warm,
                                    mind_ilqr_stats *stats_full) {
  IlqrCall q;
  q.cfg = cfg_warm; q.cfg2 = cfg_full; q.trees = trees; q.n_trees = n_trees; q.x0 = x0; q.lane = target_lane; q.n_lane_pts = n_lane_pts;
  q.target_vel = target_vel; q.xs = xs; q.us = us; q.stats = stats_warm; q.stats2 = stats_full;
  return q;
}

extern "C" int mind_ilqr_contingency_begin(mind_ctx *c, const mind_ilqr_cfg *cfg_warm, const mind_ilqr_cfg *cfg_full,
                                           const mind_cost_tree *trees, int n_trees, const double *x0, const double *target_lane,
                                           int n_lane_pts, double target_vel, double *xs, double *us,
                                           mind_ilqr_stats *stats_warm, mind_ilqr_stats *stats_full) {
  if (!c || !cfg_full) return fail(c, MIND_EINVAL, "mind_ilqr_contingency_begin: null configuration");
  IlqrCall q = il_contingency_call(cfg_warm, cfg_full, trees, n_trees, x0, target_lane, n_lane_pts, target_vel, xs, us, stats_warm, stats_full);
  q.begin_only = true;
  return il_solve(c, q);
}

extern "C" int mind_ilqr_contingency_begin_plan(mind_ctx *c, const mind_ilqr_cfg *cfg_warm, const mind_ilqr_cfg *cfg_full, const double *x0,
                                                const double *target_lane, int n_lane_pts, double target_vel, double *xs, double *us,
                                                mind_ilqr_stats *stats_warm, mind_ilqr_stats *stats_full) {
  if (!c || !cfg_full) return fail(c, MIND_EINVAL, "mind_ilqr_contingency_begin_plan: null configuration");
  const int nt = (int)c->plan.book.tree_top.size();
  if (nt <= 0 || c->plan.agents <= 0) return fail(c, MIND_ESTATE, "mind_ilqr_contingency_begin_plan: the context holds no planned cost trees");
  const int a = c->plan.agents;
  std::vector<mind_cost_tree> trees(nt);
  for (int t = 0; t < nt; ++t) {
    const size_t lo = (size_t)c->plan.book.tree_off[t];
    mind_cost_tree &T = trees[t];
    memset(&T, 0, sizeof(T));
    T.n_nodes = c->plan.book.tree_off[t + 1] - c->plan.book.tree_off[t];
    T.parent = c->plan.book.flat_parent.data() + lo; T.prob = c->plan.book.flat_prob.data() + lo;
    T.n_agents = a;
    T.agent_mean = c->plan.fmean_p ? c->plan.fmean_p + lo * a * 2 : nullptr; T.agent_cov = c->plan.fcov_p ? c->plan.fcov_p + lo * a : nullptr;
  }
  IlqrCall q = il_contingency_call(cfg_warm, cfg_full, trees.data(), nt, x0, target_lane, n_lane_pts, target_vel, xs, us, stats_warm, stats_full);
  q.begin_only = true;
  q.dev_flat = true;
  return il_solve(c, q);
}

extern "C" int mind_ilqr_finish(mind_ctx *c) {
  if (!c) return MIND_EINVAL;
  if (!c->il_finish) return fail(c, MIND_ESTATE, "mind_ilqr_finish: no tree-iLQR call was begun on this context");
  std::function<int()> fin = std::move(c->il_finish);
  c->il_finish = nullptr;
  c->il_finish_owned = false;
  c->il_early = mind_ctx::IlEarly();
  return fin();
}

extern "C" int mind_ilqr_contingency(mind_ctx *c, const mind_ilqr_cfg *cfg_warm, const mind_ilqr_cfg *cfg_full,
                                     const mind_cost_tree *trees, int n_trees, const double *x0, const double *target_lane,
                                     int n_lane_pts, double target_vel, double *xs, double *us,
                                     mind_ilqr_stats *stats_warm, mind_ilqr_stats *stats_full) {
  if (!cfg_full) return fail(c, MIND_EINVAL, "mind_ilqr_contingency: null configuration");
  return il_solve(c, il_contingency_call(cfg_warm, cfg_full, trees, n_trees, x0, target_lane, n_lane_pts, target_vel, xs, us, stats_warm, stats_full));
}

extern "C" int mind_ilqr_solve_trees(mind_ctx *c, const mind_ilqr_cfg *cfg, const mind_cost_tree *trees, int n_trees,
                                     const double *x0, const double *target_lane, int n_lane_pts, double target_vel,
                                     int use_exo, const double *us_init, double *xs, double *us,
                                     mind_ilqr_stats *stats) {
  IlqrCall q;
  q.cfg = cfg; q.trees = trees; q.n_trees = n_trees; q.x0 = x0; q.lane = target_lane; q.n_lane_pts = n_lane_pts; q.target_vel = target_vel;
  q.use_exo = use_exo; q.us_init = us_init; q.xs = xs; q.us = us; q.stats = stats;
  return il_solve(c, q);
}

extern "C" int mind_ilqr_solve_fields(mind_ctx *c, const mind_ilqr_cfg *cfg, const mind_field_grid *grid,
                                      const mind_cost_tree *trees, int n_trees, const double *x0,
                                      const double *us_init, double *xs, double *us, mind_ilqr_stats *stats) {
  if (!grid) return fail(c, MIND_EINVAL, "mind_ilqr_solve_fields: null grid");
  IlqrCall q;
  q.cfg = cfg; q.grid = grid; q.trees = trees; q.n_trees = n_trees; q.x0 = x0; q.us_init = us_init; q.xs = xs; q.us = us; q.stats = stats;
  return il_solve(c, q);
}

extern "C" int mind_cost_eval(mind_ctx *c, const mind_ilqr_cfg *cfg, const mind_field_grid *grid, const mind_cost_tree *tree,
                              const double *x0, const double *target_lane, int n_lane_pts, double target_vel, int use_exo,
                              int n_query, const int32_t *node, const double *x, const double *u, double *out) {
  if (n_query <= 0 || !node || !x || !u || !out) return fail(c, MIND_EINVAL, "mind_cost_eval: bad argument");
  const IlqrEvalReq ev{n_query, node, x, u, out};
  IlqrCall q;
  q.cfg = cfg; q.grid = grid; q.trees = tree; q.n_trees = 1; q.x0 = x0; q.lane = target_lane; q.n_lane_pts = n_lane_pts; q.target_vel = target_vel;
  q.use_exo = use_exo; q.ev = &ev;
  return il_solve(c, q);
}

extern "C" int mind_ilqr_score_trees(mind_ctx *c, const mind_ilqr_cfg *cfg, const mind_field_grid *grid, const mind_cost_tree *trees, int n_trees,
                                     const double *x0, const double *target_lane, int n_lane_pts, double target_vel, int use_exo, int n_cand,
                                     const double *us_cand, double *xs, double *L, double *J) {
  const IlqrScoreReq sc{n_cand, us_cand, xs, L, J};
  IlqrCall q;
  q.cfg = cfg; q.grid = grid; q.trees = trees; q.n_trees = n_trees; q.x0 = x0; q.lane = target_lane; q.n_lane_pts = n_lane_pts; q.target_vel = target_vel;
  q.use_exo = use_exo; q.sc = &sc;
  return il_solve(c, q);
}

extern "C" int mind_ilqr_gains(mind_ctx *c, const mind_ilqr_cfg *cfg, const mind_field_grid *grid, const mind_cost_tree *trees, int n_trees,
                               const double *x0, const double *target_lane, int n_lane_pts, double target_vel, int use_exo, const double *us,
                               const double *mu, const mind_ilqr_gains_out *out) {
  const IlqrGainsReq ga{us, mu, out};
  IlqrCall q;
  q.cfg = cfg; q.grid = grid; q.trees = trees; q.n_trees = n_trees; q.x0 = x0; q.lane = target_lane; q.n_lane_pts = n_lane_pts; q.target_vel = target_vel;
  q.use_exo = use_exo; q.us_init = us; q.ga = &ga;
  return il_solve(c, q);
}

extern "C" int mind_ilqr_policy_rollouts(mind_ctx *c, const mind_ilqr_cfg *cfg, const mind_field_grid *grid, const mind_cost_tree *trees, int n_trees,
                                         const double *x0, const double *target_lane, int n_lane_pts, double target_vel, int use_exo,
                                         const double *us, const double *k, const double *K, int n_cand, const double *alpha, const double *dx0,
                                         double *xs, double *us_out, double *L, double *J) {
  const IlqrPolicyReq po{n_cand, us, k, K, alpha, dx0, xs, us_out, L, J};
  IlqrCall q;
  q.cfg = cfg; q.grid = grid; q.trees = trees; q.n_trees = n_trees; q.x0 = x0; q.lane = target_lane; q.n_lane_pts = n_lane_pts; q.target_vel = target_vel;
  q.use_exo = use_exo; q.us_init = us; q.po = &po;
  return il_solve(c, q);
}

#define IL_PLAN_HEADER 16
extern "C" int mind_debug_ilqr_plan(const char *const *knob_names, const int *knob_values, int n_knobs, int n_cu, int mode, int n_trees,
                                    const int *n_nodes, const int32_t *parents, long long *out, int cap, int *bad) {
  if (bad) bad[0] = bad[1] = -1;
  if (n_knobs < 0 || (n_knobs > 0 && (!knob_names || !knob_values)) || n_cu <= 0 || mode < 0 || mode > 7 || n_trees <= 0 || !n_nodes || !parents ||
      cap < 0 || (cap > 0 && !out))
    return MIND_EINVAL;
  IlqrTuning t;
  const TnRefs own{nullptr, &t, nullptr};
  for (int k = 0; k < n_knobs; ++k)
    if (!knob_names[k] || !tn_set(own, knob_names[k], knob_values[k])) return MIND_EINVAL;
  int maxM = 0;
  long Mtot = 0;
  for (int i = 0; i < n_trees; ++i) {
    if (n_nodes[i] <= 0) return MIND_EINVAL;
    maxM = std::max(maxM, n_nodes[i]); Mtot += n_nodes[i];
  }
  const IlqrChoice ch = il_choose(t, n_cu, n_trees, maxM, Mtot, (mode & 1) != 0, (mode & 2) != 0);
  std::vector<long long> rec = {IL_PLAN_HEADER, n_trees, ch.form, ch.G, ch.GS, ch.spec, ch.nslot, ch.grid, ch.wgs_per_tree, ch.host_out, ch.early,
                                ch.starve_followers, 0, 0, 0, 0};
  IlTables T;
  const int32_t *parent = parents;
  for (int i = 0; i < n_trees; parent += n_nodes[i], ++i) {
    const int node = il_tree_tables(parent, n_nodes[i], t.ilqr_chunk, T);
    if (node >= 0) {
      if (bad) { bad[0] = i; bad[1] = node; }
      return MIND_EINVAL;
    }
    const std::vector<int> *tabs[14] = {&T.lvl_start, &T.lvl_nodes, &T.child_start, &T.child_list, &T.seg_start, &T.seg_nodes, &T.slvl_start,
                                        &T.slvl_segs, &T.seg_rec, &T.fs_start, &T.fs_items, &T.fs_q1, &T.fs_nstart, &T.fs_nodes};
    rec.insert(rec.end(), {n_nodes[i], T.nl, T.nseg, T.nsl, T.maxls, T.nfs});
    for (const std::vector<int> *v : tabs) rec.push_back((long long)v->size());
    for (const std::vector<int> *v : tabs) rec.insert(rec.end(), v->begin(), v->end());
  }
  for (size_t i = 0; i < rec.size() && (int)i < cap; ++i) out[i] = rec[i];
  return (int)rec.size();
}
```

### mind_amd/csrc/ilqr_kernels.hip

```cpp
#include <hip/hip_runtime.h>
#include <stdint.h>

#pragma clang fp contract(off)
#include "mind_trig.h"

#define IL_NS 6
#define IL_NU 2
#define IL_NA 10
#define IL_THREADS 512
#define IL_WAVES (IL_THREADS / 64)
#ifndef IL_SPEC_OVERSUB
#define IL_SPEC_OVERSUB 3
#endif
#define IL_SPEC 4
#define IL_SLOTS 12
#define IL_MAXA 128
#define IL_REL 15
#define IL_RA 64
#define IL_SCR 288
#define IL_CST 192
#define IL_LSUM 2048
#define IL_RMARGIN 3.0

#define IL_AS1 __attribute__((address_space(1)))
typedef double il_d2 __attribute__((ext_vector_type(2)));
typedef float il_f2 __attribute__((ext_vector_type(2)));
template <class T> struct GP {
  T *p;
  GP() = default;
  __host__ __device__ GP(T *q) : p(q) {}
  template <class U> __host__ __device__ GP(const GP<U> &o) : p(o.p) {}
  __device__ __forceinline__ T IL_AS1 *g() const { return (T IL_AS1 *)p; }
  __device__ __forceinline__ T IL_AS1 &operator[](size_t i) const { return g()[i]; }
  __device__ __forceinline__ T IL_AS1 &operator*() const { return *g(); }
  template <class V> __device__ __forceinline__ V IL_AS1 *as() const { return (V IL_AS1 *)p; }
  __host__ __device__ __forceinline__ GP operator+(size_t o) const { return GP(p + o); }
  __host__ __device__ __forceinline__ GP &operator+=(size_t o) { p += o; return *this; }
  __host__ __device__ __forceinline__ explicit operator bool() const { return p != nullptr; }
};
struct IlSlotCtl {
  unsigned gen, cmd, alive, pad;
  double mu, delta;
  unsigned done[IL_SLOTS];
  unsigned sing[IL_SLOTS];
  double Jnew[IL_SLOTS][IL_NA];
  unsigned sreq, sdone, spad0, spad1;
};

struct IlqrTreeDev {
  int M, n_agents, n_levels, pad;
  GP<const int> parent;
  GP<const int> level_start;
  GP<const int> level_nodes;
  GP<const int> child_start;
  GP<const int> child_list;
  int n_segs, n_slevels, max_level_segs, pad2;
  GP<const int> seg_start;
  GP<const int> seg_nodes;
  GP<const int> slevel_start;
  GP<const int> slevel_segs;
  GP<const int> seg_rec;
  int n_fsteps, padf;
  GP<const int> fstep_start;
  GP<const int> fstep_q0;
  GP<const int> fstep_q1;
  GP<const int> fstep_nstart;
  GP<const int> fstep_nodes;
  GP<const float> prob;
  GP<const float> mean;
  GP<const float> cov;
  GP<double> xs, us, Fx, L, Lx, Lxx;
  GP<double> k, K, Vx, Vxx;
  GP<double> xs_new, us_new, L_new;
  GP<int> rel;
  GP<double> relag;
  GP<const double> field;
  GP<const double> node_w;
  long long dset, drel;
  GP<double> h_xs, h_us, h_stats;
  unsigned *h_done;
  unsigned h_gen, pad_h;
  GP<double> stats;
  GP<double> trace;
  int trace_cap, padt;
  IlSlotCtl *ctl;
};

struct IlqrConst {
  double dt, wb;
  double w_des[6], w_con[6], lb[6], ub[6], w_ctrl[2];
  double w_tgt, w_ego, w_ego_off, w_exo, w_exo_off, w_exo_cost;
  double res, off_x, off_y, target_vel;
  double x0[6];
  int W, H, max_iter, use_exo;
  double alphas[IL_NA];
  GP<const double> gx, gy;
  int lin, pad_;
  double stepx, stepy, fsx, fsy;
  double in_x0, in_x1, in_y0, in_y1;
  GP<const double> quad;
};

#ifdef IL_HW_FENCE
#define IL_WFENCE() asm volatile("s_waitcnt lgkmcnt(0)" ::: "memory")
#else
#define IL_WFENCE() asm volatile("" ::: "memory")
#endif
#define IL_TRACE_W 4
#define IL_NSTAT 25

#ifdef IL_PROFILE
#define IL_PROF_ARG , long long *prof
#define IL_PROF_PASS , prof
#define IL_PT0() long long tp_ = clock64()
#define IL_PT(i) do { const long long n_ = clock64(); prof[i] += n_ - tp_; tp_ = n_; } while (0)
#define IL_PCNT(i) prof[i] += 1
#else
#define IL_PROF_ARG
#define IL_PROF_PASS
#define IL_PT0() do {} while (0)
#define IL_PT(i) do {} while (0)
#define IL_PCNT(i) do {} while (0)
#endif

__device__ __forceinline__ double il_shfl_down(double v, int d) {
  return __shfl_down(v, d, 64);
}

__device__ __forceinline__ double il_gx(const IlqrConst &C, int i) {
  return C.lin ? (i == C.W - 1 ? C.fsx : (double)i * C.stepx) + C.off_x : C.gx[i];
}
__device__ __forceinline__ double il_gy(const IlqrConst &C, int i) {
  return C.lin ? (i == C.H - 1 ? C.fsy : (double)i * C.stepy) + C.off_y : C.gy[i];
}

__global__ void k_lane_field(const double *__restrict__ gx, const double *__restrict__ gy, int W, int H,
                             const double *__restrict__ lane, int P, double *__restrict__ quad, int squared = 1) {
  const int idx = blockIdx.x * blockDim.x + threadIdx.x;
  if (idx >= W * H) return;
  const double px = gx[idx % W], py = gy[idx / W];
  double d = INFINITY;
  for (int j = 0; j < P - 1; ++j) {
    const double ax = lane[2 * j], ay = lane[2 * j + 1];
    const double lvx = lane[2 * j + 2] - ax, lvy = lane[2 * j + 3] - ay;
    const double len2 = lvx * lvx + lvy * lvy;
    double t = ((px - ax) * lvx + (py - ay) * lvy) / len2;
    t = t < 0 ? 0 : (t > 1 ? 1 : t);
    const double dx = px - (ax + t * lvx), dy = py - (ay + t * lvy);
    const double dj = sqrt(dx * dx + dy * dy);
    d = dj < d ? dj : d;
  }
  quad[idx] = squared ? d * d : d;
}

__device__ __forceinline__ void il_window_src(int xi, int yi, int W, int H, int r, int c, int &sy, int &sx) {
  sy = -1; sx = -1;
  const bool x0 = xi == 0, xL = xi == W - 1, y0 = yi == 0, yL = yi == H - 1;
  if (x0 && y0) { if (r >= 1 && c >= 1) { sy = r - 1; sx = c - 1; } }
  else if (x0 && yL) { if (r >= 1 && c <= 1) { sy = H - 2 + (r - 1); sx = c; } }
  else if (xL && y0) { if (r <= 1 && c >= 1) { sy = r; sx = W - 2 + (c - 1); } }
  else if (xL && yL) { if (r <= 1 && c <= 1) { sy = H - 2 + r; sx = W - 2 + c; } }
// ... 934 lines not shown
                     -4.0 * v1 * v1 * s01 + -4.0 * v1 * 2.0 * vv * s11 + -4.0 * vv * vv * s21 +
                     2.0 * v1 * v1 * s02 + 2.0 * v1 * 2.0 * vv * s12 + 2.0 * vv * vv * s22);
      fe.hyy = r2 * (2.0 * u1 * u1 * s00 + -4.0 * u1 * u1 * s10 + 2.0 * u1 * u1 * s20 +
                     2.0 * u1 * 2.0 * uu * s01 + -4.0 * u1 * 2.0 * uu * s11 + 2.0 * u1 * 2.0 * uu * s21 +
                     2.0 * uu * uu * s02 + -4.0 * uu * uu * s12 + 2.0 * uu * uu * s22);
      fe.hxy = r2 * (a * av * s00 + a * bv * s10 + a * cv * s20 +
                     b * av * s01 + b * bv * s11 + b * cv * s21 +
                     2.0 * uu * av * s02 + 2.0 * uu * bv * s12 + 2.0 * uu * cv * s22);
      const IlNodeW<GEN> NW{C, GEN ? (T.node_w + (size_t)c * IL_NW).p : nullptr, (double)pf};
      const double Lc = il_node_cost<GEN>(NW, x, u, fe);
      if (valid) {
        const GP<double> Lxx = T.Lxx + (size_t)c * 36, Lx = T.Lx + (size_t)c * 6;
        T.L[c] = Lc;
#pragma unroll
        for (int k = 0; k < 6; ++k) {
          double h = 0.0, gk = 0.0;
          if (k == 0) { h += fe.hxx; gk += fe.gx; }
          if (k == 1) { h += fe.hyy; gk += fe.gy; }
          h += 2.0 * NW.wdes(k);
          gk += 2.0 * (NW.wdes(k) * (x[k] - NW.des(k)));
          const double w = NW.wcon(k);
          if (x[k] > NW.ub(k) || x[k] < NW.lb(k)) h += 2.0 * w;
          if (x[k] > NW.ub(k)) gk += 2.0 * w * (x[k] - NW.ub(k));
          else if (x[k] < NW.lb(k)) gk += 2.0 * w * (x[k] - NW.lb(k));
          Lxx[k * 7] = h;
          Lx[k] = gk;
        }
        { double h = 0.0; h += fe.hxy; Lxx[1] = h; Lxx[6] = h; }
      }
    }
    IL_PT(13); IL_PCNT(14);
    __syncthreads();
  }
}

#define IL_SYNC_SPINS (1u << 24)
#ifndef IL_SLEEP_FOLLOW
#define IL_SLEEP_FOLLOW 8
#endif
#ifndef IL_SLEEP_SPEC
#define IL_SLEEP_SPEC 2
#endif
#ifndef IL_SLEEP_DONE
#define IL_SLEEP_DONE 2
#endif
__device__ __forceinline__ bool il_tree_sync(unsigned *bar, int G, unsigned *abort_word) {
  __shared__ int sh_aborted;
  __syncthreads();
  if (threadIdx.x == 0) {
    int aborted = 0;
    __builtin_amdgcn_fence(__ATOMIC_RELEASE, "agent");
    const unsigned gen = __hip_atomic_load(&bar[1], __ATOMIC_RELAXED, __HIP_MEMORY_SCOPE_AGENT);
    const unsigned prev = __hip_atomic_fetch_add(&bar[0], 1u, __ATOMIC_RELAXED, __HIP_MEMORY_SCOPE_AGENT);
    if (prev == (unsigned)G - 1u) {
      __hip_atomic_store(&bar[0], 0u, __ATOMIC_RELAXED, __HIP_MEMORY_SCOPE_AGENT);
      __hip_atomic_fetch_add(&bar[1], 1u, __ATOMIC_RELEASE, __HIP_MEMORY_SCOPE_AGENT);
    } else {
      unsigned spins = 0;
      while (__hip_atomic_load(&bar[1], __ATOMIC_RELAXED, __HIP_MEMORY_SCOPE_AGENT) == gen) {
        __builtin_amdgcn_s_sleep(4);
        if ((++spins & 0xfffu) == 0u) {
          if (spins >= IL_SYNC_SPINS) __hip_atomic_store(abort_word, 1u, __ATOMIC_RELAXED, __HIP_MEMORY_SCOPE_AGENT);
          if (__hip_atomic_load(abort_word, __ATOMIC_RELAXED, __HIP_MEMORY_SCOPE_AGENT)) { aborted = 1; break; }
        }
      }
    }
    __builtin_amdgcn_fence(__ATOMIC_ACQUIRE, "agent");
    sh_aborted = aborted;
  }
  __syncthreads();
  return sh_aborted != 0;
}

__device__ __forceinline__ void il_reject_update(double &mu, double &delta) {
  delta = fmax(1.0, delta) * 2.0;
  mu = fmax(1e-6, mu * delta);
}

__device__ __forceinline__ void il_flip_sets(IlqrTreeDev &T) {
  T.relag.p += T.dset; T.Fx.p += T.dset; T.L.p += T.dset; T.Lx.p += T.dset; T.Lxx.p += T.dset; T.rel.p += T.drel;
  T.dset = -T.dset; T.drel = -T.drel;
}

template <bool GEN, bool MULTI, bool SLOTS>
__device__ __forceinline__ void il_fit(IlqrTreeDev &T, int &cur, const IlqrConst &C, int ph, double *stats, double *trace, int wg, int G, unsigned *bar, unsigned *abort_word) {
  extern __shared__ double il_dsm[];
  double *scr = il_dsm + (size_t)(threadIdx.x >> 6) * IL_SCR;
  double *lsum = il_dsm + (size_t)IL_WAVES * IL_SCR;
  double *recs0 = lsum + IL_LSUM;
  double *recs = recs0 + (size_t)(threadIdx.x >> 6) * 6 * IL_RA;
  float *dstg = reinterpret_cast<float *>(recs0 + IL_RECS);
  if ((threadIdx.x & 63) < 12) {
    const int l = threadIdx.x & 63;
    scr[IL_CST + l] = l == 0 ? 1.0 : (l == 6 ? C.dt : 0.0);
  }
  __shared__ double Jnew[IL_SLOTS][IL_NA];
  __shared__ double sh_mu, sh_delta, sh_J;
  __shared__ int sh_accepted, sh_converged, sh_stop, sh_sing, sh_pick, sh_slot, sh_it, sh_nspec, sh_hint, sh_ntot;
  __shared__ int sh_spec, sh_hit, sh_nreq, sh_nhit;
  __shared__ unsigned sh_gen;
  __shared__ unsigned sh_fsing[IL_SLOTS];
  const int tid = threadIdx.x, lane = tid & 63, wave = tid >> 6;
  const int M = T.M;
  const int gw = MULTI ? wg * IL_WAVES + wave : wave, nw = MULTI ? G * IL_WAVES : IL_WAVES;
  const int gt = MULTI ? wg * IL_THREADS + tid : tid, nt = MULTI ? G * IL_THREADS : IL_THREADS;
#define IL_SYNC() do { if (MULTI) { if (il_tree_sync(bar, G, abort_word)) return; } else { __threadfence_block(); __syncthreads(); } } while (0)
#ifdef IL_PROFILE
  long long prof[16] = {0, 0, 0, 0, 0, 0, 0, 0, 0, 0, 0, 0, 0, 0, 0, 0};
#endif
  if (tid == 0) {
    sh_mu = 1.0; sh_delta = 2.0; sh_accepted = 1; sh_converged = 0; sh_stop = 0; sh_J = 0.0; sh_pick = 0; sh_slot = 0; sh_it = 0; sh_hint = 1; sh_ntot = 1;
    sh_spec = 0; sh_hit = 0; sh_nreq = 0; sh_nhit = 0;
    if (SLOTS) sh_gen = __hip_atomic_load(&T.ctl->gen, __ATOMIC_RELAXED, __HIP_MEMORY_SCOPE_AGENT);
  }
  if (MULTI && wg == 0 && tid == 0) {
    __hip_atomic_store(&bar[2], 0u, __ATOMIC_RELAXED, __HIP_MEMORY_SCOPE_AGENT);
    __hip_atomic_store(&bar[3], 0u, __ATOMIC_RELAXED, __HIP_MEMORY_SCOPE_AGENT);
  }
  for (int q = gt; q < M * 2; q += nt) T.k[q] = 0.0;
  for (int q = gt; q < M * 12; q += nt) T.K[q] = 0.0;
  for (int q = gt; q < M * 6; q += nt) T.xs[q] = 0.0;
  for (int q = gt; q < M * 36; q += nt) {
    const int e = q % 36;
    T.Fx[q] = (e % 7 == 0) ? 1.0 : (e == 16 ? C.dt : 0.0);
    T.Lxx[q] = 0.0;
    if (SLOTS && T.dset) { (T.Fx + T.dset)[q] = (e % 7 == 0) ? 1.0 : (e == 16 ? C.dt : 0.0); (T.Lxx + T.dset)[q] = 0.0; }
  }
  IL_SYNC();
  for (int s = 0; s < T.n_fsteps; ++s) {
    const int lo = T.fstep_start[s], ni = T.fstep_start[s + 1] - lo;
    for (int w = gw; w * IL_PACK < ni; w += nw) il_rollout_packed(C, T, lo, ni, ni, w, 1, 0 IL_PROF_PASS);
    IL_SYNC();
  }
  bool staged = false;
  long long t_der = 0, t_bw = 0, t_ls = 0, t_sel = 0, t_roll = 0, t_mark = clock64();
#define IL_MARK(acc) do { long long now_ = clock64(); acc += now_ - t_mark; t_mark = now_; } while (0)
  int n_pass = 0;
  while (sh_it < C.max_iter) {
    ++n_pass;
    if (sh_accepted) {
      const size_t off = ((size_t)sh_slot * IL_NA + sh_pick) * M;
      const GP<double> xn = T.xs_new + off * 6, un = T.us_new + off * 2;
      for (int q = gt; q < M * 6; q += nt) T.xs[q] = xn[q];
      for (int q = gt; q < M * 2; q += nt) T.us[q] = un[q];
      if (SLOTS && sh_hit) {
        if (tid == 0) {
          IlSlotCtl *ctl = T.ctl;
          while (__hip_atomic_load(&ctl->sdone, __ATOMIC_RELAXED, __HIP_MEMORY_SCOPE_AGENT) != sh_gen) __builtin_amdgcn_s_sleep(1);
          __builtin_amdgcn_fence(__ATOMIC_ACQUIRE, "agent");
        }
        il_flip_sets(T);
        cur ^= 1;
      } else {
        IL_SYNC();
        il_deriv_pass<GEN>(C, T, lsum, dstg, recs0, reinterpret_cast<unsigned *>(lsum + 9 * 64), MULTI ? wg : 0, MULTI ? G : 1, staged IL_PROF_PASS);
      }
      IL_SYNC();
      if (M <= IL_LSUM) {
        for (int q = tid; q < M; q += IL_THREADS) lsum[q] = T.L[q];
        __syncthreads();
        if (tid == 0) { sh_J = il_np_sum(lsum, M); sh_accepted = 0; }
      } else if (M <= 64 * (IL_LSUM / 3)) {
        const double Jn = il_np_sum_wg(T.L, M, lsum);
        if (tid == 0) { sh_J = Jn; sh_accepted = 0; }
      } else if (tid == 0) { sh_J = il_np_sum(T.L.p, M); sh_accepted = 0; }
      __syncthreads();
    }
    IL_MARK(t_der);
    if (tid == 0) {
      int ns = sh_hint;
      const int maxseg = T.max_level_segs > 0 ? T.max_level_segs : 1;
      while (ns > 1 && ns * maxseg > IL_SPEC_OVERSUB * nw) --ns;
      const unsigned alive = SLOTS ? __hip_atomic_load(&T.ctl->alive, __ATOMIC_RELAXED, __HIP_MEMORY_SCOPE_AGENT) : 0u;
      const bool fol = SLOTS && G > 1 && ((alive | 1u) & ((1u << G) - 1u)) == (1u << G) - 1u;
      sh_spec = SLOTS && fol && T.dset && ((alive >> G) & 1u);
      sh_hit = 0;
      if (fol) ns = G < IL_SLOTS ? G : IL_SLOTS;
      if (ns > C.max_iter - sh_it) ns = C.max_iter - sh_it;
      double mu = sh_mu, de = sh_delta;
      int cnt = 1;
      for (; cnt < ns; ++cnt) { il_reject_update(mu, de); if (mu >= 1e10) break; }
      sh_ntot = cnt < ns ? cnt : ns;
      sh_nspec = fol ? 1 : sh_ntot;
      sh_sing = 0;
      if (SLOTS) {
        IlSlotCtl *ctl = T.ctl;
        ctl->mu = sh_mu; ctl->delta = sh_delta;
        __hip_atomic_store(&ctl->cmd, (unsigned)(fol ? sh_ntot : 1) | ((unsigned)ph << 8) | ((unsigned)cur << 24), __ATOMIC_RELAXED, __HIP_MEMORY_SCOPE_AGENT);
        sh_gen += 1u;
        __hip_atomic_store(&ctl->gen, sh_gen, __ATOMIC_RELEASE, __HIP_MEMORY_SCOPE_AGENT);
      }
      if (MULTI && wg == 0) __hip_atomic_store(&bar[2 + ((n_pass + 1) & 1)], 0u, __ATOMIC_RELAXED, __HIP_MEMORY_SCOPE_AGENT);
    }
    __syncthreads();
    const int nspec = sh_nspec;
    for (int d = T.n_slevels - 1; d >= 0; --d) {
      const int lo = T.slevel_start[d], hi = T.slevel_start[d + 1];
      for (int w = gw; w < (hi - lo) * nspec; w += nw) {
        const int slot = w / (hi - lo), seg = T.slevel_segs[lo + w % (hi - lo)];
        double mu = sh_mu, de = sh_delta;
        for (int e = 0; e < slot; ++e) il_reject_update(mu, de);
        IlqrTreeDev Ts = T;
        Ts.k += (size_t)slot * M * 2; Ts.K += (size_t)slot * M * 12; Ts.Vx += (size_t)slot * M * 6; Ts.Vxx += (size_t)slot * M * 36;
        int rec[14];
        {
          const int IL_AS1 *sr = T.seg_rec.g() + (size_t)seg * 16;
#pragma unroll
          for (int e = 0; e < 14; ++e) rec[e] = __builtin_amdgcn_readfirstlane(sr[e]);
        }
        const int s0 = rec[0], s1 = rec[1];
        {
          const int nch = rec[5];
          double acc = 0.0;
          if (lane < 42) {
            double v[6];
#pragma unroll
            for (int e = 0; e < 6; ++e) {
              const int ch = rec[8 + e];
              v[e] = lane < 36 ? Ts.Vxx[(size_t)ch * 36 + lane] : Ts.Vx[(size_t)ch * 6 + (lane - 36)];
            }
#pragma unroll
            for (int e = 0; e < 6; ++e) if (e < nch) acc += v[e];
            for (int e = rec[6] + 6; e < rec[6] + nch; ++e) {
              const int ch = T.child_list[e];
              acc += lane < 36 ? Ts.Vxx[(size_t)ch * 36 + lane] : Ts.Vx[(size_t)ch * 6 + (lane - 36)];
            }
          }
          IL_WFENCE();
          if (lane < 36) scr[36 + lane] = acc;
          else if (lane < 42) scr[176 + lane - 36] = acc;
          IL_WFENCE();
        }
        const int sing = il_backward_segment<GEN>(C, T, Ts, s0, s1, rec[2], rec[4], mu, scr IL_PROF_PASS);
        if (sing) {
          if (lane == 0) {
            if (MULTI) __hip_atomic_fetch_or(&bar[2 + (n_pass & 1)], 1u << slot, __ATOMIC_RELAXED, __HIP_MEMORY_SCOPE_AGENT);
            else atomicOr(&sh_sing, 1 << slot);
          }
        }
        else {
          const int c = rec[3];
          if (lane < 36) Ts.Vxx[(size_t)c * 36 + lane] = scr[36 + lane];
          else if (lane < 42) Ts.Vx[(size_t)c * 6 + lane - 36] = scr[176 + lane - 36];
        }
      }
      IL_SYNC();
    }
    IL_MARK(t_bw);
    if (MULTI) {
      if (tid == 0) sh_sing = (int)__hip_atomic_load(&bar[2 + (n_pass & 1)], __ATOMIC_RELAXED, __HIP_MEMORY_SCOPE_AGENT);
      __syncthreads();
    }
    if (sh_sing & 1) {
      if (tid == 0) {
        if (trace && sh_it < T.trace_cap && (!MULTI || wg == 0)) {
          double *tr = trace + (size_t)sh_it * IL_TRACE_W;
          tr[0] = sh_mu; tr[1] = sh_J; tr[2] = -2.0; tr[3] = sh_J;
        }
        sh_it += 1;
      }
      __syncthreads();
      IL_SYNC();
      continue;
    }
    int nuse = nspec;
    for (int e = 1; e < nspec; ++e) if ((sh_sing >> e) & 1) { nuse = e; break; }
    for (int s = 0; s <= T.n_fsteps; ++s) {
      int R = 0;
      if (s < T.n_fsteps) {
        const int lo = T.fstep_start[s], ni = T.fstep_start[s + 1] - lo;
        R = (ni * nuse + IL_PACK - 1) / IL_PACK;
        for (int w = gw; w < R; w += nw) il_rollout_packed(C, T, lo, ni, ni * nuse, w, 0, 0 IL_PROF_PASS);
      } else {
        IL_MARK(t_roll);
      }
      if (s > 0) {
        const int n0 = T.fstep_nstart[s - 1], cnt = T.fstep_nstart[s] - n0;
        int rank = (gw + nw - R % nw) % nw;
        if (!MULTI && R < 4) {
          const int fr = 4 - R;
          rank = wave < R ? 2 * fr + R + wave : (wave < 4 ? wave - R : (wave < 4 + R ? 2 * fr + wave - 4 : fr + wave - 4 - R));
        }
        il_cost_pass<GEN>(C, T, nuse, recs, rank, nw, T.fstep_nodes + (size_t)n0, cnt, 0 IL_PROF_PASS);
      }
      IL_SYNC();
      if (SLOTS && s == T.n_fsteps - 1 && tid == 0 && sh_spec) {
        __hip_atomic_store(&T.ctl->sreq, sh_gen, __ATOMIC_RELEASE, __HIP_MEMORY_SCOPE_AGENT);
        sh_spec = 2; sh_nreq += 1;
      }
    }
    IL_MARK(t_ls);
    if (M * IL_NA * nuse <= IL_LSUM) {
      for (int q = tid; q < M * IL_NA * nuse; q += IL_THREADS) lsum[q] = T.L_new[q];
      __syncthreads();
    } else {
      const double J = il_seq_sums_tiled(T.L_new, M, IL_NA * nuse, lsum);
      if (tid < IL_NA * nuse) Jnew[tid / IL_NA][tid % IL_NA] = J;
    }
    if (M * IL_NA * nuse <= IL_LSUM && tid < IL_NA * nuse) {
      double J = 0.0;
      const double *Ln = lsum + (size_t)tid * M;
      int c = 0;
      for (; c + 8 <= M; c += 8) {
        double v[8];
#pragma unroll
        for (int k = 0; k < 8; ++k) v[k] = Ln[c + k];
#pragma unroll
        for (int k = 0; k < 8; ++k) J += v[k];
      }
      for (; c < M; ++c) J += Ln[c];
      Jnew[tid / IL_NA][tid % IL_NA] = J;
    }
    __syncthreads();
    bool gathered = false;
    if (SLOTS && sh_ntot > nspec) {
      bool own = false;
      for (int slot = 0; slot < nuse; ++slot)
        for (int a = 0; a < IL_NA; ++a) own |= Jnew[slot][a] < sh_J;
      if (!own) {
        if (tid >= nuse && tid < sh_ntot) {
          IlSlotCtl *ctl = T.ctl;
          while (__hip_atomic_load(&ctl->done[tid], __ATOMIC_RELAXED, __HIP_MEMORY_SCOPE_AGENT) != sh_gen) __builtin_amdgcn_s_sleep(IL_SLEEP_DONE);
          __builtin_amdgcn_fence(__ATOMIC_ACQUIRE, "agent");
          sh_fsing[tid] = __hip_atomic_load(&ctl->sing[tid], __ATOMIC_RELAXED, __HIP_MEMORY_SCOPE_AGENT);
          for (int a = 0; a < IL_NA; ++a) Jnew[tid][a] = ctl->Jnew[tid][a];
        }
        __syncthreads();
        gathered = true;
      }
    }
    if (tid == 0) {
      double mu = sh_mu, de = sh_delta;
      int it = sh_it;
      bool done = false;
      const int nsel = (SLOTS && sh_ntot > nspec) ? sh_ntot : nuse;
      for (int slot = 0; slot < nsel && !done; ++slot) {
        if (SLOTS && slot >= nuse && gathered) {
          if (sh_fsing[slot]) break;
        } else if (SLOTS && slot >= nuse) {
          IlSlotCtl *ctl = T.ctl;
          while (__hip_atomic_load(&ctl->done[slot], __ATOMIC_RELAXED, __HIP_MEMORY_SCOPE_AGENT) != sh_gen) __builtin_amdgcn_s_sleep(IL_SLEEP_DONE);
          __builtin_amdgcn_fence(__ATOMIC_ACQUIRE, "agent");
          if (__hip_atomic_load(&ctl->sing[slot], __ATOMIC_RELAXED, __HIP_MEMORY_SCOPE_AGENT)) break;
          for (int a = 0; a < IL_NA; ++a) Jnew[slot][a] = ctl->Jnew[slot][a];
        }
        int pick = -1;
        for (int a = 0; a < IL_NA; ++a)
          if (Jnew[slot][a] < sh_J) { pick = a; break; }
        if (trace && it < T.trace_cap && (!MULTI || wg == 0)) {
          double *tr = trace + (size_t)it * IL_TRACE_W;
          tr[0] = mu; tr[1] = sh_J; tr[2] = (double)pick; tr[3] = pick >= 0 ? Jnew[slot][pick] : sh_J;
        }
        it += 1;
        if (pick >= 0) {
          sh_pick = pick; sh_slot = slot;
          if (fabs((sh_J - Jnew[slot][pick]) / sh_J) < 1e-6) sh_converged = 1;
          sh_accepted = 1;
          de = fmin(1.0, de) / 2.0;
          mu *= de;
          if (mu <= 1e-6) mu = 0.0;
          done = true;
        } else {
          il_reject_update(mu, de);
          if (mu >= 1e10) { sh_stop = 1; done = true; }
        }
      }
      sh_mu = mu; sh_delta = de; sh_it = it;
      sh_hint = (sh_accepted && sh_slot == 0) ? 1 : IL_SPEC;
      if (SLOTS && sh_spec == 2 && sh_accepted && sh_slot == 0 && sh_pick == 0) { sh_hit = 1; sh_nhit += 1; }
    }
    __syncthreads();
    IL_MARK(t_sel);
    if (sh_converged || sh_stop) break;
  }
  if (sh_accepted) {
    const size_t off = ((size_t)sh_slot * IL_NA + sh_pick) * M;
    const GP<double> xn = T.xs_new + off * 6, un = T.us_new + off * 2;
    for (int q = gt; q < M * 6; q += nt) T.xs[q] = xn[q];
    for (int q = gt; q < M * 2; q += nt) T.us[q] = un[q];
  }
  if (tid == 0 && (!MULTI || wg == 0)) {
    stats[0] = (double)sh_it;
    stats[1] = (double)sh_converged;
    stats[2] = sh_J;
    stats[3] = sh_mu;
    stats[4] = (double)t_der; stats[5] = (double)t_bw; stats[6] = (double)t_ls; stats[7] = (double)t_sel;
#ifdef IL_PROFILE
    for (int q = 0; q < 16; ++q) stats[8 + q] = (double)prof[q];
#else
    stats[8] = (double)t_roll;
    stats[9] = (double)sh_nreq; stats[10] = (double)sh_nhit;
#endif
    stats[IL_NSTAT - 1] = (double)n_pass;
  }
  IL_SYNC();
#undef IL_SYNC
}

template <bool GEN>
__device__ __forceinline__ void il_follow(const IlqrTreeDev &T0, const IlqrConst *consts, int wg) {
  extern __shared__ double il_dsm[];
  double *scr = il_dsm + (size_t)(threadIdx.x >> 6) * IL_SCR;
  double *lsum = il_dsm + (size_t)IL_WAVES * IL_SCR;
  double *recs0 = lsum + IL_LSUM;
  double *recs = recs0 + (size_t)(threadIdx.x >> 6) * 6 * IL_RA;
  __shared__ unsigned f_gen, f_cmd;
  __shared__ double f_mu, f_de;
  __shared__ int f_sing, f_abort;
  const int tid = threadIdx.x, lane = tid & 63, wave = tid >> 6;
  const int M = T0.M;
  IlSlotCtl *ctl = T0.ctl;
  if (tid == 0) __hip_atomic_fetch_or(&ctl->alive, 1u << wg, __ATOMIC_RELAXED, __HIP_MEMORY_SCOPE_AGENT);
  unsigned last = 0;
  int ph_cst = -1;
  for (;;) {
    __syncthreads();
    if (tid == 0) {
      unsigned g;
      while ((g = __hip_atomic_load(&ctl->gen, __ATOMIC_RELAXED, __HIP_MEMORY_SCOPE_AGENT)) == last) __builtin_amdgcn_s_sleep(IL_SLEEP_FOLLOW);
      __builtin_amdgcn_fence(__ATOMIC_ACQUIRE, "agent");
      f_gen = g; f_cmd = __hip_atomic_load(&ctl->cmd, __ATOMIC_RELAXED, __HIP_MEMORY_SCOPE_AGENT);
      f_mu = ctl->mu; f_de = ctl->delta; f_sing = 0; f_abort = 0;
    }
    __syncthreads();
    const unsigned g = f_gen, cmd = f_cmd;
    last = g;
    if ((cmd >> 16) & 0xffu) return;
    const int ns = (int)(cmd & 0xffu), ph = (int)((cmd >> 8) & 0xffu);
    if (wg >= ns) continue;
    const IlqrConst &C = consts[ph];
    if (ph != ph_cst) {
      if (lane < 12) scr[IL_CST + lane] = lane == 0 ? 1.0 : (lane == 6 ? C.dt : 0.0);
      ph_cst = ph;
    }
    double mu = f_mu, de = f_de;
    for (int e = 0; e < wg; ++e) il_reject_update(mu, de);
    IlqrTreeDev T = T0;
    if ((cmd >> 24) & 1u) il_flip_sets(T);
    IlqrTreeDev Ts = T;
    Ts.k += (size_t)wg * M * 2; Ts.K += (size_t)wg * M * 12; Ts.Vx += (size_t)wg * M * 6; Ts.Vxx += (size_t)wg * M * 36;
    for (int d = T.n_slevels - 1; d >= 0; --d) {
      const int lo = T.slevel_start[d], hi = T.slevel_start[d + 1];
      for (int w = wave; w < hi - lo; w += IL_WAVES) {
        const int seg = T.slevel_segs[lo + w];
        int rec[14];
        {
          const int IL_AS1 *sr = T.seg_rec.g() + (size_t)seg * 16;
#pragma unroll
          for (int e = 0; e < 14; ++e) rec[e] = __builtin_amdgcn_readfirstlane(sr[e]);
        }
        {
          const int nch = rec[5];
          double acc = 0.0;
          if (lane < 42) {
            double v[6];
#pragma unroll
            for (int e = 0; e < 6; ++e) {
              const int ch = rec[8 + e];
              v[e] = lane < 36 ? Ts.Vxx[(size_t)ch * 36 + lane] : Ts.Vx[(size_t)ch * 6 + (lane - 36)];
            }
#pragma unroll
            for (int e = 0; e < 6; ++e) if (e < nch) acc += v[e];
            for (int e = rec[6] + 6; e < rec[6] + nch; ++e) {
              const int ch = T.child_list[e];
              acc += lane < 36 ? Ts.Vxx[(size_t)ch * 36 + lane] : Ts.Vx[(size_t)ch * 6 + (lane - 36)];
            }
          }
          IL_WFENCE();
          if (lane < 36) scr[36 + lane] = acc;
          else if (lane < 42) scr[176 + lane - 36] = acc;
          IL_WFENCE();
        }
#ifdef IL_PROFILE
        long long prof[16];
// ... 1 lines not shown
        const int sing = il_backward_segment<GEN>(C, T, Ts, rec[0], rec[1], rec[2], rec[4], mu, scr IL_PROF_PASS, &ctl->gen, g);
        if (sing) {
          if (lane == 0) { if (sing == 2) f_abort = 1; else f_sing = 1; }
        } else {
          const int c = rec[3];
          if (lane < 36) Ts.Vxx[(size_t)c * 36 + lane] = scr[36 + lane];
          else if (lane < 42) Ts.Vx[(size_t)c * 6 + lane - 36] = scr[176 + lane - 36];
        }
      }
      __threadfence_block();
      __syncthreads();
      if (f_abort) break;
    }
    if (f_abort) continue;
    if (!f_sing) {
      for (int s = 0; s <= T.n_fsteps; ++s) {
        int R = 0;
        if (s < T.n_fsteps) {
          const int lo = T.fstep_start[s], ni = T.fstep_start[s + 1] - lo;
          R = (ni + IL_PACK - 1) / IL_PACK;
#ifdef IL_PROFILE
          long long prof[16];
#endif
          for (int w = wave; w < R; w += IL_WAVES)
            if (il_rollout_packed(C, T, lo, ni, ni, w, 0, wg IL_PROF_PASS, &ctl->gen, g) && lane == 0) f_abort = 1;
        }
        if (s > 0) {
          const int n0 = T.fstep_nstart[s - 1], cnt = T.fstep_nstart[s] - n0;
          int rank = (wave + IL_WAVES - R % IL_WAVES) % IL_WAVES;
          if (R < 4) {
            const int fr = 4 - R;
            rank = wave < R ? 2 * fr + R + wave : (wave < 4 ? wave - R : (wave < 4 + R ? 2 * fr + wave - 4 : fr + wave - 4 - R));
          }
#ifdef IL_PROFILE
          long long prof[16];
#endif
          il_cost_pass<GEN>(C, T, 1, recs, rank, IL_WAVES, T.fstep_nodes + (size_t)n0, cnt, wg IL_PROF_PASS, &ctl->gen, g);
        }
        __threadfence_block();
        __syncthreads();
        if (f_abort) break;
      }
      if (tid == 0 && !f_abort && __hip_atomic_load(&ctl->gen, __ATOMIC_RELAXED, __HIP_MEMORY_SCOPE_AGENT) != g) f_abort = 1;
      __syncthreads();
      if (f_abort) continue;
      const GP<double> Lg = T.L_new + (size_t)wg * IL_NA * M;
      if (M * IL_NA <= IL_LSUM) {
        for (int q = tid; q < M * IL_NA; q += IL_THREADS) lsum[q] = Lg[q];
        __syncthreads();
      } else {
        const double J = il_seq_sums_tiled(Lg, M, IL_NA, lsum);
        if (tid < IL_NA) ctl->Jnew[wg][tid] = J;
      }
      if (M * IL_NA <= IL_LSUM && tid < IL_NA) {
        double J = 0.0;
        const double *Ln = lsum + (size_t)tid * M;
        int c = 0;
        for (; c + 8 <= M; c += 8) {
          double v[8];
#pragma unroll
          for (int k = 0; k < 8; ++k) v[k] = Ln[c + k];
#pragma unroll
          for (int k = 0; k < 8; ++k) J += v[k];
        }
        for (; c < M; ++c) J += Ln[c];
        ctl->Jnew[wg][tid] = J;
      }
    }
    __threadfence_block();
    __syncthreads();
    if (tid == 0) {
      __hip_atomic_store(&ctl->sing[wg], (unsigned)f_sing, __ATOMIC_RELAXED, __HIP_MEMORY_SCOPE_AGENT);
      __hip_atomic_store(&ctl->done[wg], g, __ATOMIC_RELEASE, __HIP_MEMORY_SCOPE_AGENT);
    }
  }
}

template <bool GEN>
__device__ __forceinline__ void il_speculate(const IlqrTreeDev &T0, const IlqrConst *consts, int wg) {
  extern __shared__ double il_dsm[];
  double *lsum = il_dsm + (size_t)IL_WAVES * IL_SCR;
  double *recs0 = lsum + IL_LSUM;
  float *dstg = reinterpret_cast<float *>(recs0 + IL_RECS);
  __shared__ unsigned s_req, s_cmd;
  const int tid = threadIdx.x;
  IlSlotCtl *ctl = T0.ctl;
  if (tid == 0) __hip_atomic_fetch_or(&ctl->alive, 1u << wg, __ATOMIC_RELAXED, __HIP_MEMORY_SCOPE_AGENT);
  unsigned last = 0;
  bool staged = false;
  for (;;) {
    __syncthreads();
    if (tid == 0) {
      unsigned r, cmd;
      for (;;) {
        r = __hip_atomic_load(&ctl->sreq, __ATOMIC_RELAXED, __HIP_MEMORY_SCOPE_AGENT);
        cmd = __hip_atomic_load(&ctl->cmd, __ATOMIC_RELAXED, __HIP_MEMORY_SCOPE_AGENT);
        if (r != last || (cmd >> 16) & 0xffu) break;
        __builtin_amdgcn_s_sleep(IL_SLEEP_SPEC);
      }
      __builtin_amdgcn_fence(__ATOMIC_ACQUIRE, "agent");
      s_req = r; s_cmd = __hip_atomic_load(&ctl->cmd, __ATOMIC_RELAXED, __HIP_MEMORY_SCOPE_AGENT);
    }
    __syncthreads();
    const unsigned r = s_req, cmd = s_cmd;
    if ((cmd >> 16) & 0xffu) return;
    last = r;
    const int ph = (int)((cmd >> 8) & 0xffu);
    IlqrTreeDev T = T0;
    if (!((cmd >> 24) & 1u)) il_flip_sets(T);
    T.xs = T0.xs_new; T.us = T0.us_new;
#ifdef IL_PROFILE
    long long prof[16];
#endif
    il_deriv_pass<GEN>(consts[ph], T, lsum, dstg, recs0, reinterpret_cast<unsigned *>(lsum + 9 * 64), 0, 1, staged IL_PROF_PASS);
    __threadfence_block();
    __syncthreads();
    if (tid == 0) __hip_atomic_store(&ctl->sdone, r, __ATOMIC_RELEASE, __HIP_MEMORY_SCOPE_AGENT);
  }
}

template <bool GEN, int MODE>
__global__ __launch_bounds__(IL_THREADS) void k_ilqr(const IlqrTreeDev *__restrict__ trees, const IlqrConst *__restrict__ consts,
                                                     int n_phases, int n_trees, int G, unsigned *__restrict__ bars, int spec) {
  constexpr bool MULTI = MODE == 1, SLOTS = MODE == 2;
  int t = blockIdx.x, wg = 0;
  if (MODE != 0) {
    const int Gl = G + (SLOTS ? spec : 0);
    const int r = blockIdx.x % (8 * Gl);
    t = 8 * (blockIdx.x / (8 * Gl)) + (r & 7);
    wg = r >> 3;
    if (t >= n_trees) return;
  }
  IlqrTreeDev T = trees[t];
  if (SLOTS && wg > 0) {
    if (bars[4 * n_trees + 1]) return;
    if (wg >= G) il_speculate<GEN>(T, consts, wg);
    else il_follow<GEN>(T, consts, wg);
    return;
  }
  int cur = 0;
  for (int ph = 0; ph < n_phases; ++ph)
    il_fit<GEN, MULTI, SLOTS>(T, cur, consts[ph], ph, (T.stats + (size_t)ph * IL_NSTAT).p, T.trace ? (T.trace + (size_t)ph * T.trace_cap * IL_TRACE_W).p : nullptr, wg, G, MULTI ? bars + 4 * t : nullptr, MULTI ? bars + 4 * n_trees : nullptr);
  if (T.h_xs && wg == 0) {
    const int M = T.M;
    for (int q = threadIdx.x; q < M * 6; q += IL_THREADS) T.h_xs[q] = T.xs[q];
    for (int q = threadIdx.x; q < M * 2; q += IL_THREADS) T.h_us[q] = T.us[q];
    for (int q = threadIdx.x; q < n_phases * IL_NSTAT; q += IL_THREADS) T.h_stats[q] = T.stats[q];
    if (T.h_done) {
      __threadfence_system();
      __syncthreads();
      if (threadIdx.x == 0) __hip_atomic_store(T.h_done, T.h_gen, __ATOMIC_RELEASE, __HIP_MEMORY_SCOPE_SYSTEM);
    }
  }
  if (SLOTS && threadIdx.x == 0) {
    __hip_atomic_store(&T.ctl->cmd, 1u << 16, __ATOMIC_RELAXED, __HIP_MEMORY_SCOPE_AGENT);
    __hip_atomic_store(&T.ctl->gen, __hip_atomic_load(&T.ctl->gen, __ATOMIC_RELAXED, __HIP_MEMORY_SCOPE_AGENT) + 1u, __ATOMIC_RELEASE, __HIP_MEMORY_SCOPE_AGENT);
  }
}

static inline size_t il_lds_bytes(int ) {
  return ((size_t)IL_WAVES * IL_SCR + IL_LSUM + (size_t)IL_RECS) * sizeof(double) + (size_t)IL_DSTG * sizeof(float);
}

#define IL_EVAL_OUT 47
template <bool GEN>
__global__ __launch_bounds__(64) void k_cost_eval(const IlqrTreeDev *__restrict__ trees, IlqrConst C, int nq,
                                                  const int *__restrict__ node, const double *__restrict__ xq,
                                                  const double *__restrict__ uq, double *__restrict__ out) {
  const IlqrTreeDev T = trees[0];
  extern __shared__ double il_dsm[];
  double *scr = il_dsm, *ag = il_dsm + IL_SCR;
  const int q = blockIdx.x, lane = threadIdx.x;
  if (q >= nq) return;
  const int c = node[q];
  double x[6], u[2];
#pragma unroll
  for (int k = 0; k < 6; ++k) x[k] = xq[(size_t)q * 6 + k];
  u[0] = uq[(size_t)q * 2]; u[1] = uq[(size_t)q * 2 + 1];
  if (C.use_exo) il_stage_agents(C, T, c, ag);
  double *o = out + (size_t)q * IL_EVAL_OUT;
  il_node_derivs<GEN>(C, T, c, x, u, scr, ag, o + 9, nullptr, o + 1, o);
  if (lane < 2) {
    const IlNodeW<GEN> NW{C, GEN ? (T.node_w + (size_t)c * IL_NW).p : nullptr, GEN ? 0.0 : (double)T.prob[c]};
    o[7 + lane] = 2.0 * (NW.wctrl(lane) * u[lane]);
    o[45 + lane] = 2.0 * NW.wctrl(lane);
  }
}
```

### mind_amd/csrc/mind_hip.hip

```cpp
#include <hip/hip_runtime.h>

#include <cmath>
#include <cstdarg>
#include <cstdio>
#include <cstdlib>
#include <algorithm>
#include <cstring>
#include <map>
#include <memory>
#include <string>
#include <thread>
#include <atomic>
#include <functional>
#include <vector>

#include "../../include/mind_hip.h"
#include "encdec_kernels.hip"
#include "fusion_kernels.hip"
#include "pair_bf16_kernels.hip"
#include "pair_tile_kernels.hip"
#include "pair_tile6_kernels.hip"
#include "token_mfma_kernels.hip"
#include "actor_mfma_kernels.hip"
#include "actor_lw_kernels.hip"
// ... 10 lines not shown
#include "ttc_kernels.hip"
#include "pair_jobs.h"
#include "pred_choice.h"
#include "ilqr_choice.h"
#include "aime_book.h"
#include "audit_arena.h"
#include "weight_pack.h"
#include "aime_kernels.hip"

static_assert(TN_RA == RA && TN_IL_SLOTS == IL_SLOTS, "tuning.h restates the two kernel constants its clamps need");

static std::atomic<long> live_handles{0};

template <class H, hipError_t (*Release)(H)> struct Owned {
  H p = nullptr;
  size_t cap = 0;
  Owned() = default;
  Owned(Owned &&o) noexcept : p(o.p), cap(o.cap) { o.p = nullptr; o.cap = 0; }
  Owned &operator=(Owned &&o) noexcept { if (this != &o) { reset(); p = o.p; cap = o.cap; o.p = nullptr; o.cap = 0; } return *this; }
  ~Owned() { reset(); }
  operator H() const { return p; }
  template <class T> T *as() const { return (T *)p; }
  void reset() {
    if (p) { (void)Release(p); live_handles.fetch_sub(1, std::memory_order_relaxed); }
    p = nullptr; cap = 0;
  }
  hipError_t took(hipError_t e, size_t bytes = 0) {
    if (e == hipSuccess) { live_handles.fetch_add(1, std::memory_order_relaxed); cap = bytes; } else p = nullptr;
    return e;
  }
};
struct Event : Owned<hipEvent_t, hipEventDestroy> { hipError_t create(unsigned flags = hipEventDefault) { reset(); return took(hipEventCreateWithFlags(&p, flags)); } };
struct Stream : Owned<hipStream_t, hipStreamDestroy> { hipError_t create() { reset(); return took(hipStreamCreateWithFlags(&p, hipStreamNonBlocking)); } };
struct Pinned : Owned<void *, hipHostFree> {
  hipError_t alloc(size_t bytes, unsigned flags = hipHostMallocDefault) { reset(); return took(hipHostMalloc(&p, bytes, flags), bytes); }
};
struct DevBuf : Owned<void *, hipFree> {
  hipError_t alloc(size_t bytes) { reset(); return took(hipMalloc(&p, bytes), bytes); }
};

struct TableSet {
  std::vector<int> key;
  DevBuf meta, jobs, jobs5, rows;
  std::vector<int> actor_row, cls_row, scene_n;
  long long edge_pairs = 0, edge_pairs_t = 0, stamp = 0;
  int ntok = 0, slot = 0, njobs = 0, njobs5 = 0;
  double pairs_full = 0, pairs_l5 = 0;
};
#define MIND_TABLE_SETS 8

struct mind_ctx {
  int device = 0;
  hipStream_t stream = nullptr;
  Stream side;
  Event ev_side, ev_main, ev_stage, ev_tgt, ev_cls;
  std::vector<char> aime_stage;
  bool aime_stage_busy = false;
  std::string err;
  DevBuf wdev;
  bool have_weights = false;
  WeightTables W = {};
  PredTuning pt; IlqrTuning it; CtxTuning ct;
  TnRefs knobs() { return {&pt, &it, &ct}; }
  int dec_basis = MIND_BASIS_BEZIER;
  DevBuf curve_tab;
  std::vector<double> curve_tau;
  int curve_tab_basis = -1;
  DevBuf tok_lw_arena;
  std::vector<TlLaunch> tok_lw_plan;
  int last_tok_lw = 0, last_tok_launches = 0, last_tok_chunks = 0;
  float tok_ms = 0.f, tok_stage_ms[TL_NSTAGE + 1] = {};
  std::vector<Event> ev_tok;
  std::vector<int> ev_tok_tag;
  TableSet tabs[MIND_TABLE_SETS];
  long long tab_clock = 0;
  long long n_table_hits = 0;
  unsigned dec_gen = 0;
  DevBuf pl_cnt;
  std::function<int(hipStream_t)> enc_pre, enc_post;
  std::vector<IlTables> il_tab;
  struct IlImage { std::vector<double> hD; std::vector<float> hF; std::vector<int> hI; } il_img;
  struct IlEarly { const double *xs = nullptr, *us = nullptr; volatile unsigned *done = nullptr; unsigned gen = 0; int n_trees = 0; long nodes = 0; } il_early;
  unsigned il_gen = 0;
  long long il_spec_req = 0, il_spec_hit = 0;
  DevBuf actor_lw_arena;
  std::vector<LwLaunch> actor_lw_plan;
  int last_actor_lw = 0, last_actor_launches = 0, last_actor_chunks = 0;
  float actor_ms = 0.f;
  Event ev_act0, ev_act1;
  int pair_prec = 3;
  std::vector<int> last_scene_n;
  bool last_edge_tiled = false, last_edge_bf16 = false;
  DevBuf edge, x, ST, QK, part, tokpos, meta, jobs, actor_feat, lane_feat, tgt_feat, cmode, tgt_emb,
      rows, rpe_ptrs;
  DevBuf ilqr_dev, aime_dev, rebase_dev2[2], dec_h2;
  DevBuf audit_dev;
  DevBuf pl_root, pl_in[2], pl_lf, pl_lrep, pl_pred, pl_small, pl_tab[2], pl_win[2];
  std::vector<DevBuf> pl_world;
  Pinned pl_pin[8];
  Event ev_pl, ev_tab, ev_root;
  DevBuf il_field;
  Pinned il_field_pin;
  Event ev_field;
  bool il_field_valid = false;
  double il_field_key[5] = {0, 0, 0, 0, 0};
  std::vector<double> il_field_lane;
  int xr = 0, xw = 1;
  mind_exchange_fn xfn = nullptr;
  void *xuser = nullptr;
  bool xforce = false;
  DevBuf x_send, x_recv, x_seg;
  long long x_collectives = 0, x_bytes = 0;
  Stream pl_copy;
  std::vector<double> pl_sol_xs, pl_sol_us;
  std::vector<mind_ilqr_stats> pl_sol_stw, pl_sol_stf;
  std::thread pa_thread;
  std::atomic<int> pa_state{0};
  mind_aime_plan_in pa_in;
  mind_aime_plan_out pa_out;
  int pa_rc = 0;
  struct Plan {
    AimeBook book;
    int agents = 0;
    long long gen = 0;
    const float *rows_p = nullptr, *fmean_p = nullptr, *fcov_p = nullptr;
    const float *dev_fmean = nullptr, *dev_fcov = nullptr;
  } plan;
  DevBuf pl_flat;
  DevBuf dec_xbuf, dec_bars;
  Pinned dec_abort;
  int rb_cur = 0, rb_gen = 0;
  size_t rb_S = 0, rb_a = 0;
  bool profiling = false;
  Event ev_il0, ev_il1;
  float ilqr_ms = 0.f;
  int ilqr_multi = 0, ilqr_trees = 0;
  std::function<int()> il_finish;
  bool il_finish_owned = false;
  Event ev_rows;
  std::vector<const double *> il_trace_dev;
  std::vector<int> il_trace_its;
  int il_trace_cap = 0, il_trace_phases = 0;
  double il_prof[9] = {0, 0, 0, 0, 0, 0, 0, 0, 0};
  long long n_ilqr_fallbacks = 0;
  int n_pair_launch = 0;
  float pair_ms = 0.f;
  double pairs_done = 0.0;
  std::vector<Event> ev;
  bool ev_defer = false;
  std::vector<Event> ev_pool;
  size_t ev_pool_used = 0;
  std::vector<size_t> ev_pending;
  int wall_khz = 0;
  LcRing lc;
  DevBuf lc_dev;
  Pinned lc_host;
  double lc_carry_ms[LC_KINDS] = {0, 0, 0};
  int lc_carry_n[LC_KINDS] = {0, 0, 0};
  std::vector<float> lc_last[LC_KINDS], ev_last[LC_KINDS];
  int n_cu = 256;
  int debug_layers = 6;
  int last_ntok = 0;
  size_t il_dbg[6] = {0, 0, 0, 0, 0, 0};
  long long last_edge_pairs = 0;
  int last_slots = 0, last_A = 0, last_B = 0;
};
// ... 799 lines not shown
extern "C" int mind_fill_tracks(const double *raw , int a, int T, const int32_t *slot ,
                                float *pos , float *ang , float *vel , int16_t *typ ,
                                int16_t *have ) {
  if (!raw || !slot || !pos || !ang || !vel || !typ || !have || a < 0 || T <= 0) return MIND_EINVAL;
  for (int i = 0; i < a; ++i) {
    const double *r = raw + (size_t)i * T * 6;
    int first = 0;
    for (int t = 0; t < T; ++t)
      if (r[t * 6] != 0.0) { first = t; break; }
    int src = -1;
    for (int t = 0; t < T; ++t) {
      const bool h = r[t * 6] != 0.0;
      if (h) src = t;
      const int f = src < 0 ? first : src;
      const bool hf = r[f * 6] != 0.0;
      const size_t o = (size_t)i * T + t;
      pos[2 * o] = hf ? (float)r[f * 6 + 1] : 0.f;
      pos[2 * o + 1] = hf ? (float)r[f * 6 + 2] : 0.f;
      ang[o] = hf ? (float)r[f * 6 + 3] : 0.f;
      vel[2 * o] = h ? (float)r[t * 6 + 4] : 0.f;
      vel[2 * o + 1] = h ? (float)r[t * 6 + 5] : 0.f;
      have[o] = h ? 1 : 0;
      for (int k = 0; k < 7; ++k) typ[o * 7 + k] = (h && k == slot[i]) ? 1 : 0;
    }
  }
  return MIND_OK;
}

extern "C" int mind_eval_traj_trees(const double *states, const double *ctrls, const int32_t *counts, int n_trees, const void *lane,
                                    int lane_is_f32, int n_lane_pts, double target_vel, double *out) {
  if (!states || !ctrls || !counts || n_trees <= 0 || !lane || n_lane_pts < 2 || !out) return MIND_EINVAL;
  long N = 0;
  for (int t = 0; t < n_trees; ++t) { if (counts[t] <= 0) return MIND_EINVAL; N += counts[t]; }
  std::vector<double> per(N);
  auto run = [&](long lo, long hi) {
    if (lane_is_f32) eval_nodes<float>(states + 6 * lo, ctrls + 2 * lo, hi - lo, (const float *)lane, n_lane_pts, target_vel, per.data() + lo);
    else eval_nodes<double>(states + 6 * lo, ctrls + 2 * lo, hi - lo, (const double *)lane, n_lane_pts, target_vel, per.data() + lo);
  };
  const long nth = std::min<long>(std::min<long>(8, (long)std::max(1u, std::thread::hardware_concurrency())), N / 8192);
  if (nth <= 1) run(0, N);
  else {
    std::vector<std::thread> th;
    for (long k = 0; k < nth; ++k) th.emplace_back(run, N * k / nth, N * (k + 1) / nth);
    for (std::thread &t : th) t.join();
  }
  long o = 0;
  for (int t = 0; t < n_trees; ++t) {
    const long n = counts[t];
    out[t] = (n > 1 ? per[o] + np_pairwise(per.data() + o + 1, n - 1) : per[o]) / (double)n;
    o += n;
  }
  return MIND_OK;
}

__global__ void k_debug_trig(const double *__restrict__ x, int n, double *__restrict__ out) {
  const int i = blockIdx.x * blockDim.x + threadIdx.x;
  const double v = i < n ? x[i] : 0.0;
  double s, c, t, c2;
  mind_sincos(v, &s, &c);
  mind_tan_cos(v, &t, &c2);
  if (i < n) { out[4 * i] = s; out[4 * i + 1] = c; out[4 * i + 2] = t; out[4 * i + 3] = c2; }
}
extern "C" int mind_debug_trig(mind_ctx *c, const double *x, int n, double *out) {
  if (!c || !x || !out || n <= 0) return MIND_EINVAL;
  HIPCHK(c, hipSetDevice(c->device));
  double *d = nullptr;
  HIPCHK(c, hipMalloc((void **)&d, (size_t)n * 5 * sizeof(double)));
  hipError_t e = hipMemcpy(d, x, (size_t)n * sizeof(double), hipMemcpyHostToDevice);
  if (e == hipSuccess) {
    hipLaunchKernelGGL(k_debug_trig, dim3((n + 63) / 64), dim3(64), 0, c->stream, d, n, d + n);
    e = hipStreamSynchronize(c->stream);
  }
  if (e == hipSuccess) e = hipMemcpy(out, d + n, (size_t)n * 4 * sizeof(double), hipMemcpyDeviceToHost);
  (void)hipFree(d);
  if (e != hipSuccess) return fail(c, MIND_EHIP, "mind_debug_trig: %s", hipGetErrorString(e));
  return MIND_OK;
}

extern "C" int mind_debug_set_layers(mind_ctx *c, int n) {
  if (!c || n < 0 || n > 6) return MIND_EINVAL;
  c->debug_layers = n;
  return MIND_OK;
}
extern "C" int64_t mind_debug_read(mind_ctx *c, const char *name, float *host, int64_t max_floats) {
  if (!c || !name) return MIND_EINVAL;
  const void *src = nullptr;
  int64_t n = 0;
  std::string k = name;
  if (k == "x") { src = c->x.p; n = (int64_t)c->last_ntok * 128; }
  else if (k == "ST") { src = c->ST.p; n = (int64_t)c->last_ntok * 256; }
  else if (k == "QK") { src = c->QK.p; n = (int64_t)c->last_ntok * 1024; }
  else if (k == "edge") { src = c->edge.p; n = c->last_edge_pairs * 128; }
  else if (k == "part") { src = c->part.p; n = (int64_t)c->last_slots * PART_STRIDE; }
  else if (k == "actor_feat") { src = c->actor_feat.p; n = (int64_t)c->last_A * 128; }
  else if (k == "tokpos") { src = c->tokpos.p; n = (int64_t)c->last_ntok * 4; }
  else if (k == "cmode") { src = c->cmode.p; n = (int64_t)c->last_B * 768; }
  else if (k == "tgt_emb") { src = c->tgt_emb.p; n = (int64_t)c->last_B * 128; }
  else if (k == "tgt_feat") { src = c->tgt_feat.p; n = (int64_t)c->last_B * 128; }
  else if (k == "pl_root") { src = c->pl_root.p; n = (int64_t)(c->pl_root.cap / sizeof(float)); }
  else if (k == "il_spec") {
    if (!host) return 2;
    if (max_floats < 2) return MIND_EINVAL;
    host[0] = (float)c->il_spec_req; host[1] = (float)c->il_spec_hit;
    return 2;
  }
  else if (k.rfind("il_", 0) == 0 && c->il_dbg[5]) {
    const size_t M = c->il_dbg[5];
    int w = -1; size_t per = 0;
    if (k == "il_L") { w = 0; per = 1; } else if (k == "il_Lx") { w = 1; per = 6; } else if (k == "il_Lxx") { w = 2; per = 36; }
    else if (k == "il_Fx") { w = 3; per = 36; } else if (k == "il_xs") { w = 4; per = 6; }
    if (w < 0) return MIND_EINVAL;
    src = (const char *)c->ilqr_dev.p + c->il_dbg[w];
    n = (int64_t)(M * per * 2);
  }
  else return MIND_EINVAL;
  if (!host) return n;
  if (n > max_floats) n = max_floats;
  if (hipStreamSynchronize(c->stream) != hipSuccess) return MIND_EHIP;
  if (k == "edge" && c->last_edge_tiled) {
    long long pt = 0;
    for (int N : c->last_scene_n) pt += (long long)N * (((N + 15) / 16) * 16);
    const bool eb = c->last_edge_bf16;
    std::vector<float> raw((size_t)pt * (eb ? 64 : 128));
    if (hipMemcpy(raw.data(), src, raw.size() * sizeof(float), hipMemcpyDeviceToHost) != hipSuccess) return MIND_EHIP;
    int64_t o = 0;
    size_t sb = 0;
    for (int N : c->last_scene_n) {
      const int rows = ((N + 15) / 16) * 16;
      for (int j = 0; j < N; ++j)
        for (int i = 0; i < N; ++i)
          for (int f = 0; f < 128 && o < n; ++f, ++o) {
            const int t = i >> 4, pp = i & 15, b = f >> 4, qq = (f >> 2) & 3, r = f & 3;
            const size_t tile0 = sb + (size_t)j * rows + (size_t)t * 16;
            if (!eb) host[o] = raw[tile0 * 128 + ((b * 64 + qq * 16 + pp) * 4 + r)];
            else {
              uint32_t w;
              memcpy(&w, &raw[tile0 * 64 + (((b >> 1) * 64 + qq * 16 + pp) * 4 + 2 * (b & 1) + (r >> 1))], 4);
              w = (r & 1) ? (w & 0xffff0000u) : (w << 16);
              memcpy(&host[o], &w, 4);
            }
          }
      sb += (size_t)N * rows;
    }
    return n;
  }
  if (hipMemcpy(host, src, (size_t)n * sizeof(float), hipMemcpyDeviceToHost) != hipSuccess) return MIND_EHIP;
  return n;
}

#include "loop.hip"

#include "audit_host.hip"

#include "forecast_host.hip"

#include "road_host.hip"

#include "ttc_host.hip"
```

### mind_amd/predictor.py

```python
import ctypes as C

import numpy as np
import torch

from . import _lib


AIME_NODE_DTYPE = np.dtype({"names": ["round", "scene", "mode", "parent", "prob", "cur_t", "end_t", "flags", "dur", "row_off", "tgt_pts"],
                            "formats": ["<i4", "<i4", "<i4", "<i4", "<f4", "<i4", "<i4", "<i4", "<i4", "<i8", ("<f4", (22,))],
                            "offsets": [0, 4, 8, 12, 16, 20, 24, 28, 32, 40, 48], "itemsize": 136})


class IlqrCall:

    def __init__(self, lib, cfg, flats, x0, lane, target_vel, cfg_full=None, use_exo=1, us_init=None, background=False):
        self.lib, self.cfg, self.cfg_full, self.use_exo = lib, cfg, cfg_full, int(use_exo)
        self.background = bool(background)
        n = self.n = len(flats)
        self.trees = (_lib.CostTree * n)()
        self.keep, self.Ms = [], []
        for i, f in enumerate(flats):
            par = np.ascontiguousarray(f["parent"], np.int32)
            prob = np.ascontiguousarray(f["prob"], np.float32)
            mean = np.ascontiguousarray(f["mean"], np.float32)
# ... 167 lines not shown
            self.lib.mind_set_tuning(self.ctx, b"ilqr_wgs", 1)
        elif not on and self._ilqr_wgs_saved is not None:
            self.lib.mind_set_tuning(self.ctx, b"ilqr_wgs", self._ilqr_wgs_saved)
            self._ilqr_wgs_saved = None

    def set_pair_precision(self, name):
        _lib.check(self.lib, self.ctx, self.lib.mind_set_pair_precision(self.ctx, self.PAIR_PREC.index(name)), "mind_set_pair_precision")

    def set_decoder_basis(self, name):
        if name not in _lib.BASIS:
            raise ValueError(f"unknown decoder basis {name!r}: one of {_lib.BASIS}")
        _lib.check(self.lib, self.ctx, self.lib.mind_set_decoder_basis(self.ctx, _lib.BASIS.index(name)), "mind_set_decoder_basis")

    def get_decoder_basis(self):
        return _lib.BASIS[self.lib.mind_get_decoder_basis(self.ctx)]

    def curve_eval(self, param, tau, basis=None, want=("reg", "vel", "cov_vel")):
        assert param.device == self.device and param.dtype == torch.float32 and tuple(param.shape[-2:]) == (8, 5), (param.device, param.dtype, param.shape)
        if basis is not None and basis not in _lib.BASIS:
            raise ValueError(f"unknown decoder basis {basis!r}: one of {_lib.BASIS}")
        widths = {"reg": 5, "vel": 2, "cov_vel": 3}
        if any(k not in widths for k in want):
            raise ValueError(f"curve_eval: want names {tuple(want)!r}, of {tuple(widths)}")
        param = param.contiguous()
        tau = np.ascontiguousarray(tau, np.float64).ravel()
        lead, n = tuple(param.shape[:-2]), param.numel() // 40
        out = {k: torch.empty(lead + (tau.size, w), device=self.device) for k, w in widths.items() if k in want}
        ptr = lambda k: C.c_void_p(out[k].data_ptr()) if k in out and out[k].numel() > 0 else None
        rc = self.lib.mind_curve_eval(self.ctx, -1 if basis is None else _lib.BASIS.index(basis), C.c_void_p(param.data_ptr()) if n else None, n,
                                      tau.ctypes.data_as(C.POINTER(C.c_double)), tau.size, ptr("reg"), ptr("vel"), ptr("cov_vel"))
        _lib.check(self.lib, self.ctx, rc, "mind_curve_eval")
        return out

    def set_profiling(self, on):
        self.lib.mind_set_profiling(self.ctx, 1 if on else 0)

    def ilqr_stats(self):
        ms, n, g = C.c_float(), C.c_int(), C.c_int()
        self.lib.mind_last_ilqr_stats(self.ctx, C.byref(ms), C.byref(n), C.byref(g))
        return ms.value, n.value, g.value

    def ilqr_profile(self):
        v = (C.c_double * 9)()
        self.lib.mind_last_ilqr_profile(self.ctx, v)
        keys = ("nodes", "depth", "passes", "derivatives", "backward", "state_chain", "cost_pass", "selection", "trees")
        return dict(zip(keys, [float(x) for x in v]))

    def ilqr_trace(self, tree, phase=0):
        n = C.c_int()
        buf = np.zeros((256, 4), np.float64)
        _lib.check(self.lib, self.ctx, self.lib.mind_last_ilqr_trace(self.ctx, int(tree), int(phase), buf.ctypes.data_as(C.POINTER(C.c_double)), 256,
                                                                    C.byref(n)), "mind_last_ilqr_trace")
        return buf[:min(n.value, 256)].copy()

    def fusion_stats(self):
        n = C.c_int()
        ms = C.c_float()
        pairs = C.c_double()
        self.lib.mind_last_fusion_stats(self.ctx, C.byref(n), C.byref(ms), C.byref(pairs))
        return n.value, ms.value, pairs.value

    def launch_times(self, kind="pair"):
        cap = 4096
        ck, ev = (C.c_float * cap)(), (C.c_float * cap)()
        nc, ne = C.c_int(), C.c_int()
        _lib.check(self.lib, self.ctx, self.lib.mind_debug_launch_times(self.ctx, {"pair": 0, "actor": 1}[kind], ck, ev, cap, C.byref(nc), C.byref(ne)),
                   "mind_debug_launch_times")
        return [float(v) for v in ck[:min(nc.value, cap)]], [float(v) for v in ev[:min(ne.value, cap)]]

    def last_actor_stats(self):
        lw, n, ch, ms = C.c_int(), C.c_int(), C.c_int(), C.c_float()
        _lib.check(self.lib, self.ctx, self.lib.mind_last_actor_stats(self.ctx, C.byref(lw), C.byref(n), C.byref(ch), C.byref(ms)), "mind_last_actor_stats")
        return dict(layerwise=lw.value, launches=n.value, chunks=ch.value, ms=ms.value)

    def last_token_stats(self):
        lw, n, ch, ms = C.c_int(), C.c_int(), C.c_int(), C.c_float()
        _lib.check(self.lib, self.ctx, self.lib.mind_last_token_stats(self.ctx, C.byref(lw), C.byref(n), C.byref(ch), C.byref(ms)), "mind_last_token_stats")
        st = (C.c_float * 8)()
        self.lib.mind_last_token_stage_ms(self.ctx, st, 8)
        return dict(layerwise=lw.value, launches=n.value, chunks=ch.value, ms=ms.value, stage_ms=[float(v) for v in st])

    def debug_set_layers(self, n):
        _lib.check(self.lib, self.ctx, self.lib.mind_debug_set_layers(self.ctx, n), "mind_debug_set_layers")

    def debug_read(self, name):
        n = self.lib.mind_debug_read(self.ctx, name.encode(), None, 0)
        if n < 0:
            raise _lib.MindError(f"mind_debug_read({name}) -> {n}")
        buf = np.empty(n, np.float32)
        got = self.lib.mind_debug_read(self.ctx, name.encode(), buf.ctypes.data_as(C.POINTER(C.c_float)), n)
        assert got == n, (got, n)
        return buf

    def synchronize(self):
        _lib.check(self.lib, self.ctx, self.lib.mind_ctx_synchronize(self.ctx), "mind_ctx_synchronize")

    def predict(self, actors, actor_off, lanes, lane_off, actor_ctrs, actor_vecs, lane_ctrs, lane_vecs,
                tgt_nodes, tgt_rpe, rpe=None, lane_feat=None, want_lane_feat=False, taps=False, aux=False):
        dev = self.device
        B = len(actor_off) - 1
        A, L = int(actor_off[-1]), int(lane_off[-1])

        def f32(t):
            if t is None:
                return None
            assert t.device == dev and t.dtype == torch.float32, (t.device, t.dtype)
            return t.contiguous()

        actors, lanes, lane_feat = f32(actors), f32(lanes), f32(lane_feat)
        actor_ctrs, actor_vecs, lane_ctrs, lane_vecs = f32(actor_ctrs), f32(actor_vecs), f32(lane_ctrs), f32(lane_vecs)
        tgt_nodes, tgt_rpe = f32(tgt_nodes), f32(tgt_rpe)
        assert actors.shape == (A, 14, 48) and tgt_nodes.shape == (B, 10, 16) and tgt_rpe.shape == (B, 20)
        ao = (C.c_int32 * (B + 1))(*[int(v) for v in actor_off])
        lo = (C.c_int32 * (B + 1))(*[int(v) for v in lane_off])
        sb = _lib.SceneBatch()
        sb.n_scenes = B
        sb.actor_off, sb.lane_off = ao, lo

        def ptr(t):
            return C.c_void_p(t.data_ptr()) if t is not None and t.numel() > 0 else None

        sb.actors, sb.lanes, sb.lane_feat = ptr(actors), ptr(lanes), ptr(lane_feat)
        sb.actor_ctrs, sb.actor_vecs, sb.lane_ctrs, sb.lane_vecs = ptr(actor_ctrs), ptr(actor_vecs), ptr(lane_ctrs), ptr(lane_vecs)
        rpe_keep = None
        if rpe is not None:
            rpe_keep = [f32(r) for r in rpe]
            arr = (C.c_void_p * B)(*[r.data_ptr() for r in rpe_keep])
            sb.rpe = arr
        sb.tgt_nodes, sb.tgt_rpe = ptr(tgt_nodes), ptr(tgt_rpe)
        out = {"cls": torch.empty(B, 6, device=dev), "reg": torch.empty(A, 6, 60, 5, device=dev),
               "vel": torch.empty(A, 6, 60, 2, device=dev)}
        po = _lib.PredOut()
        po.cls, po.reg, po.vel = ptr(out["cls"]), ptr(out["reg"]), ptr(out["vel"])
        if want_lane_feat and lane_feat is None and L > 0:
            out["lane_feat"] = torch.empty(L, 128, device=dev)
            po.lane_feat = ptr(out["lane_feat"])
        if taps:
            out["actor_emb"] = torch.empty(A, 128, device=dev)
            out["cls_emb"] = torch.empty(B, 128, device=dev)
            po.actor_emb, po.cls_emb = ptr(out["actor_emb"]), ptr(out["cls_emb"])
        if aux:
            out["cov_vel"] = torch.empty(A, 6, 60, 3, device=dev)
            out["param"] = torch.empty(A, 6, 8, 5, device=dev)
            pa = _lib.PredAux(ptr(out["cov_vel"]), ptr(out["param"]))
            rc = self.lib.mind_predict_batch_aux(self.ctx, C.byref(sb), C.byref(po), C.byref(pa))
        else:
            rc = self.lib.mind_predict_batch(self.ctx, C.byref(sb), C.byref(po))
        _lib.check(self.lib, self.ctx, rc, "mind_predict_batch")
        return out

    def ilqr_contingency(self, cfg_warm, cfg_full, flats, x0, lane, target_vel):
        call = IlqrCall(self.lib, cfg_warm, flats, x0, lane, target_vel, cfg_full=cfg_full)
        call.run(self)
        return call.finish()

    def ilqr_solve(self, cfg, flats, x0, lane, target_vel, use_exo, us_init=None):
        call = IlqrCall(self.lib, cfg, flats, x0, lane, target_vel, use_exo=use_exo, us_init=us_init)
        call.run(self)
        return call.finish()

    @staticmethod
    def _generic_tree(tree, keep):
        ct = _lib.CostTree()
        par = np.ascontiguousarray(tree["parent"], np.int32)
        fld = np.ascontiguousarray(tree["field"], np.float64)
        nw = np.ascontiguousarray(tree["node_w"], np.float64)
# ... 566 lines not shown
```

Before: 1885.

## Speculatively run next iLQR backward pass on spare workgroup during rollout

The speculative-derivative workgroup now also runs the next iteration's backward pass. It predicts the accepted step's mu from the current mu and delta, and writes gains into a second gain set in the arena. When the line search accepts the nominal slot and the speculative backward did not hit a singular matrix, the main workgroup flips its gain pointers and skips its own backward sweep. This aims to take the backward pass off the critical path of each iteration. In exchange it adds arena memory for a second k/K/Vx/Vxx set, extra spin-waits, and work that is thrown away when the speculation misses.

```diff
diff --git a/include/mind_hip.h b/include/mind_hip.h
--- a/include/mind_hip.h
+++ b/include/mind_hip.h
@@ -106,6 +106,8 @@
 
 int mind_debug_ilqr_plan(const char *const *knob_names, const int *knob_values, int n_knobs, int n_cu, int mode, int n_trees, const int *n_nodes,
                          const int32_t *parents, long long *out, int cap, int *bad);
+int mind_debug_ilqr_gains_sets(const char *const *knob_names, const int *knob_values, int n_knobs, int n_cu, int n_trees, const int *n_nodes,
+                               const int32_t *parents, long long *out);
 
 int mind_debug_aime_book(int pred_len, int max_depth, int max_rounds, int n_agents, int world, int rank, int force, int n_rounds, const int *dec_len,
                          const float *dec, int n_tokens, int bytes_per_pair, int plan_chunk_mb, int per_scene, long long *out, int cap, char *msg,
@@ -127,6 +129,8 @@
 int mind_debug_trig(mind_ctx *ctx, const double *x, int n, double *out);
 
 int mind_debug_set_layers(mind_ctx *ctx, int n);
+int mind_debug_set_ilqr_spec_backward(mind_ctx *ctx, int on);
+int mind_debug_ilqr_accept_mu(double mu, double delta, double *out2);
 int64_t mind_debug_read(mind_ctx *ctx, const char *name, float *host, int64_t max_floats);
 
 typedef struct {
diff --git a/mind_amd/_lib.py b/mind_amd/_lib.py
--- a/mind_amd/_lib.py
+++ b/mind_amd/_lib.py
@@ -223,7 +223,7 @@
 
 EXPORTS = ["mind_ctx_create", "mind_ctx_destroy", "mind_last_error_string", "mind_ctx_synchronize",
            "mind_weights_load", "mind_predict_batch", "mind_last_fusion_stats", "mind_last_actor_stats", "mind_debug_actor_lw_plan", "mind_last_token_stats", "mind_last_token_stage_ms", "mind_debug_token_lw_plan", "mind_set_profiling", "mind_debug_launch_times", "mind_debug_launch_clock",
-           "mind_ilqr_solve_trees", "mind_ilqr_contingency", "mind_ilqr_solve_fields", "mind_cost_eval", "mind_ilqr_score_trees", "mind_ilqr_gains", "mind_ilqr_policy_rollouts", "mind_lane_dist_field", "mind_aime_world", "mind_aime_rebase", "mind_debug_aime_decide", "mind_debug_set_layers",
+           "mind_ilqr_solve_trees", "mind_ilqr_contingency", "mind_ilqr_solve_fields", "mind_cost_eval", "mind_ilqr_score_trees", "mind_ilqr_gains", "mind_ilqr_policy_rollouts", "mind_lane_dist_field", "mind_aime_world", "mind_aime_rebase", "mind_debug_aime_decide", "mind_debug_set_layers", "mind_debug_set_ilqr_spec_backward", "mind_debug_ilqr_accept_mu", "mind_debug_ilqr_gains_sets",
            "mind_debug_read", "mind_set_pair_precision", "mind_get_pair_precision", "mind_debug_pack_bfrag", "mind_debug_pack_conv_frag", "mind_debug_pack", "mind_debug_weight_image", "mind_debug_weight_bind", "mind_debug_pair_schedule", "mind_debug_predict_choice", "mind_debug_ilqr_plan", "mind_debug_aime_book", "mind_set_tuning", "mind_get_tuning", "mind_debug_tuning", "mind_debug_live_handles", "mind_last_ilqr_stats", "mind_aime_plan", "mind_last_ilqr_profile", "mind_eval_traj_trees", "mind_last_ilqr_trace", "mind_ilqr_contingency_begin", "mind_ilqr_finish", "mind_fill_tracks", "mind_ilqr_contingency_begin_plan", "mind_debug_trig", "mind_aime_plan_begin", "mind_aime_plan_poll", "mind_aime_plan_finish", "mind_ctx_busy", "mind_ilqr_finish_plan",
            "mind_set_exchange", "mind_last_exchange_stats", "mind_debug_wait_word",
            "mind_predict_batch_aux", "mind_set_decoder_basis", "mind_get_decoder_basis", "mind_curve_eval", "mind_debug_curve_basis",
@@ -340,6 +340,10 @@
                                             C.POINTER(C.c_longlong), C.c_int, C.POINTER(C.c_longlong), C.c_char_p, C.c_int]
     lib.mind_debug_weight_bind.argtypes = [C.POINTER(TensorDesc), C.c_int, C.c_char_p, C.c_char_p, C.c_int]
     lib.mind_debug_set_layers.argtypes = [C.c_void_p, C.c_int]
+    lib.mind_debug_set_ilqr_spec_backward.argtypes = [C.c_void_p, C.c_int]
+    lib.mind_debug_ilqr_accept_mu.argtypes = [C.c_double, C.c_double, C.POINTER(C.c_double)]
+    lib.mind_debug_ilqr_gains_sets.argtypes = [C.POINTER(C.c_char_p), C.POINTER(C.c_int), C.c_int, C.c_int, C.c_int, C.POINTER(C.c_int), C.POINTER(C.c_int32),
+                                               C.POINTER(C.c_longlong)]
     lib.mind_debug_read.argtypes = [C.c_void_p, C.c_char_p, C.POINTER(C.c_float), C.c_int64]
     lib.mind_set_exchange.argtypes = [C.c_void_p, C.c_int, C.c_int, EXCHANGE_FN, C.c_void_p, C.c_int]
     lib.mind_last_exchange_stats.argtypes = [C.c_void_p, C.POINTER(C.c_longlong), C.POINTER(C.c_longlong)]
@@ -437,7 +441,7 @@
                     "fstep_start", "fstep_items", "fstep_q1", "fstep_nstart", "fstep_nodes")
 
 
-def ilqr_plan(knobs, parents, n_cu=256, generic=False, evaluate=False, two_fits=False):
+def ilqr_plan(knobs, parents, n_cu=256, generic=False, evaluate=False, two_fits=False, arena=False):
     lib = load()
     names = (C.c_char_p * max(1, len(knobs)))(*[k.encode() for k in knobs])
     vals = (C.c_int * max(1, len(knobs)))(*[int(v) for v in knobs.values()])
@@ -460,6 +464,12 @@
             tr[name], o = list(out[o:o + ln]), o + ln
         d["trees"].append(tr)
     assert o == n
+    if arena:
+        g = (C.c_longlong * (1 + 2 * len(parents)))()
+        assert lib.mind_debug_ilqr_gains_sets(names, vals, len(knobs), n_cu, len(parents), nn, par, g) == len(g)
+        d["spec_bw"] = g[0]
+        for i, tr in enumerate(d["trees"]):
+            tr["kspare_doubles"], tr["kset"] = g[1 + 2 * i], g[2 + 2 * i]
     return d
 
 
diff --git a/mind_amd/csrc/ilqr_choice.h b/mind_amd/csrc/ilqr_choice.h
--- a/mind_amd/csrc/ilqr_choice.h
+++ b/mind_amd/csrc/ilqr_choice.h
@@ -9,6 +9,7 @@
 struct IlqrChoice {
   int form = 0;
   int G = 1, GS = 1, spec = 0;
+  int spec_bw = 0;
   int nslot = IL_SPEC;
   int grid = 0;
   int wgs_per_tree = 1;
@@ -17,7 +18,7 @@
   bool starve_followers = false;
 };
 
-static IlqrChoice il_choose(const IlqrTuning &t, int n_cu, int n_trees, int max_nodes, long total_nodes, bool gen, bool eval) {
+static IlqrChoice il_choose(const IlqrTuning &t, int n_cu, int n_trees, int max_nodes, long total_nodes, bool gen, bool eval, bool spec_bw = true) {
   IlqrChoice ch;
   const int blocks8 = ((n_trees + 7) / 8) * 8;
   int G = t.ilqr_wgs;
@@ -31,6 +32,7 @@
   ch.G = multi ? G : 1;
   ch.GS = GS;
   ch.spec = slots && t.ilqr_spec_deriv && GS < 31 && blocks8 * (GS + 1) <= n_cu ? 1 : 0;
+  ch.spec_bw = ch.spec && spec_bw ? 1 : 0;
   ch.nslot = slots ? std::max(GS, IL_SPEC) : IL_SPEC;
   ch.grid = ch.form == 2 ? blocks8 * (GS + ch.spec) : ch.form == 1 ? blocks8 * G - (t.ilqr_test_starve ? 8 : 0) : n_trees;
   ch.wgs_per_tree = ch.form == 1 ? G : ch.form == 2 ? GS + ch.spec : 1;
@@ -142,6 +144,7 @@
   size_t us, nodew, xs, stats, trace;
   size_t relag, Fx, L, Lx, Lxx, relag2, Fx2, L2, Lx2, Lxx2;
   size_t k, K, Vx, Vxx, xsn, usn, Ln;
+  size_t kspare, kspare_n;
   size_t prob, mean, cov;
   size_t parent, lnodes, cstart, clist, rel, rel2, lstart, sstart, snodes, slstart, slsegs, segrec, fsstart, fsitems, fsq1, fsnstart, fsnodes;
   size_t field;
@@ -205,6 +208,8 @@
     L.Lxx2 = A.takeD(spec ? 36 * M : 0);
     L.k = A.takeD(nslot * 2 * M); L.K = A.takeD(nslot * 12 * M); L.Vx = A.takeD(nslot * 6 * M); L.Vxx = A.takeD(nslot * 36 * M);
     L.xsn = A.takeD(nslot * 60 * M); L.usn = A.takeD(nslot * 20 * M); L.Ln = A.takeD(nslot * 10 * M);
+    L.kspare_n = ch.spec_bw ? (L.Vxx - L.k) + 36 * M : 0;
+    L.kspare = A.takeD(L.kspare_n);
     L.prob = A.takeF(M); L.mean = A.takeF(s.dev_flat ? 0 : M * a * 2); L.cov = A.takeF(s.dev_flat ? 0 : M * a);
     L.parent = A.takeI(M); L.lnodes = A.takeI(M); L.cstart = A.takeI(M + 1); L.clist = A.takeI(M); L.rel = A.takeI(M); L.rel2 = A.takeI(spec ? M : 0);
   }
diff --git a/mind_amd/csrc/ilqr_host.hip b/mind_amd/csrc/ilqr_host.hip
--- a/mind_amd/csrc/ilqr_host.hip
+++ b/mind_amd/csrc/ilqr_host.hip
@@ -342,6 +342,7 @@
     D.h_done = ch.early ? R.h_done + t : nullptr; D.h_gen = c->il_gen; D.pad_h = 0;
     if (ch.early && ((L.xs - L0.xs) != (size_t)moff * 6 || (L.us - L0.us) != (size_t)moff * 2)) return fail(c, MIND_EINVAL, "tree-iLQR arena: results are not contiguous");
     D.dset = ch.spec ? (long long)L.Fx2 - (long long)L.Fx : 0; D.drel = ch.spec ? (long long)L.rel2 - (long long)L.rel : 0;
+    D.kset = ch.spec_bw ? (long long)L.kspare - (long long)L.k : 0;
     if (ch.spec && (L.L2 - L.L != L.Fx2 - L.Fx || L.Lx2 - L.Lx != L.Fx2 - L.Fx || L.Lxx2 - L.Lxx != L.Fx2 - L.Fx || (R.use_exo && L.relag2 - L.relag != L.Fx2 - L.Fx)))
       return fail(c, MIND_EINVAL, "tree-iLQR arena: the two derivative sets are laid out differently");
     moff += (long)M;
@@ -408,7 +409,7 @@
   const int nt = P.n_trees;
   const dim3 block(IL_THREADS);
   if (P.gen) hipLaunchKernelGGL((k_ilqr<true, 0>), dim3(nt), block, P.il_lds, P.st, P.dT, P.dK, P.n_phases, nt, 1, P.dBars, 0);
-  else if (form == 2) hipLaunchKernelGGL((k_ilqr<false, 2>), dim3(ch.grid), block, P.il_lds, P.st, P.dT, P.dK, P.n_phases, nt, ch.GS, P.dBars, ch.spec);
+  else if (form == 2) hipLaunchKernelGGL((k_ilqr<false, 2>), dim3(ch.grid), block, P.il_lds, P.st, P.dT, P.dK, P.n_phases, nt, ch.GS, P.dBars, ch.spec | ch.spec_bw << 1);
   else if (form == 1) hipLaunchKernelGGL((k_ilqr<false, 1>), dim3(ch.grid), block, P.il_lds, P.st, P.dT, P.dK, P.n_phases, nt, ch.G, P.dBars, 0);
   else hipLaunchKernelGGL((k_ilqr<false, 0>), dim3(nt), block, P.il_lds, P.st, P.dT, P.dK, P.n_phases, nt, 1, P.dBars, 0);
 }
@@ -445,10 +446,11 @@
     c->il_trace_dev[t] = P.trace_cap > 0 ? P.tree[t].trace : nullptr;
     for (int ph = 0; ph < n_phases; ++ph) c->il_trace_its[2 * t + ph] = (int)hstat(t, ph)[0];
   }
-  c->il_spec_req = 0; c->il_spec_hit = 0;
+  c->il_spec_req = 0; c->il_spec_hit = 0; c->il_spec_bw_req = 0; c->il_spec_bw_hit = 0;
 #ifndef IL_PROFILE
   for (int t = 0; t < n_trees; ++t)
-    for (int ph = 0; ph < n_phases; ++ph) { c->il_spec_req += (long long)hstat(t, ph)[9]; c->il_spec_hit += (long long)hstat(t, ph)[10]; }
+    for (int ph = 0; ph < n_phases; ++ph) { c->il_spec_req += (long long)hstat(t, ph)[9]; c->il_spec_hit += (long long)hstat(t, ph)[10];
+                                           if (P.ch.form == 2) { c->il_spec_bw_req += (long long)hstat(t, ph)[11]; c->il_spec_bw_hit += (long long)hstat(t, ph)[12]; } }
 #endif
   double best = -1.0;
   for (int t = 0; t < n_trees; ++t) {
@@ -612,7 +614,7 @@
   int maxM = 0;
   for (int t = 0; t < q.n_trees; ++t) maxM = std::max(maxM, q.trees[t].n_nodes);
   const bool other = q.ev || q.sc || q.ga || q.po;
-  R.ch = il_choose(c->it, c->n_cu, q.n_trees, maxM, R.Mtot, R.gen, other);
+  R.ch = il_choose(c->it, c->n_cu, q.n_trees, maxM, R.Mtot, R.gen, other, c->il_spec_bw != 0);
   if ((rc = il_build_tables(c, q))) return rc;
   IlShape shape{R.W, R.H, R.n_lane_pts, q.ev ? q.ev->nq : 0, q.n_trees, R.n_agents.data(), R.gen, R.use_exo != 0, R.dev_flat, R.trace_cap, q.sc ? q.sc->n_cand : 0};
   shape.gains = q.ga != nullptr;
@@ -755,7 +757,42 @@
   return il_solve(c, q);
 }
 
+extern "C" int mind_debug_ilqr_accept_mu(double mu, double delta, double *out2) {
+  if (!out2) return MIND_EINVAL;
+  il_accept_update(mu, delta);
+  out2[0] = mu; out2[1] = delta;
+  return MIND_OK;
+}
+
 #define IL_PLAN_HEADER 16
+extern "C" int mind_debug_ilqr_gains_sets(const char *const *knob_names, const int *knob_values, int n_knobs, int n_cu, int n_trees, const int *n_nodes,
+                                          const int32_t *parents, long long *out) {
+  if (n_knobs < 0 || (n_knobs > 0 && (!knob_names || !knob_values)) || n_cu <= 0 || n_trees <= 0 || !n_nodes || !parents || !out) return MIND_EINVAL;
+  IlqrTuning t;
+  const TnRefs own{nullptr, &t, nullptr};
+  for (int k = 0; k < n_knobs; ++k)
+    if (!knob_names[k] || !tn_set(own, knob_names[k], knob_values[k])) return MIND_EINVAL;
+  int maxM = 0;
+  long Mtot = 0;
+  std::vector<IlTables> tab((size_t)n_trees);
+  const int32_t *parent = parents;
+  for (int i = 0; i < n_trees; parent += n_nodes[i], ++i) {
+    if (n_nodes[i] <= 0 || il_tree_tables(parent, n_nodes[i], t.ilqr_chunk, tab[i]) >= 0) return MIND_EINVAL;
+    maxM = std::max(maxM, n_nodes[i]); Mtot += n_nodes[i];
+  }
+  const IlqrChoice ch = il_choose(t, n_cu, n_trees, maxM, Mtot, false, false);
+  const std::vector<int> ones((size_t)n_trees, 1);
+  IlShape s{};
+  s.W = 2; s.H = 2; s.n_lane_pts = 2; s.nq = 0; s.n_trees = n_trees; s.n_agents = ones.data(); s.gen = false; s.use_exo = true; s.dev_flat = false; s.trace_cap = 0;
+  IlArena A;
+  il_layout(s, ch, tab.data(), A);
+  out[0] = ch.spec_bw;
+  for (int i = 0; i < n_trees; ++i) {
+    out[1 + 2 * i] = (long long)A.tree[i].kspare_n;
+    out[2 + 2 * i] = ch.spec_bw ? (long long)A.tree[i].kspare - (long long)A.tree[i].k : 0;
+  }
+  return 1 + 2 * n_trees;
+}
 extern "C" int mind_debug_ilqr_plan(const char *const *knob_names, const int *knob_values, int n_knobs, int n_cu, int mode, int n_trees,
                                     const int *n_nodes, const int32_t *parents, long long *out, int cap, int *bad) {
   if (bad) bad[0] = bad[1] = -1;
diff --git a/mind_amd/csrc/ilqr_kernels.hip b/mind_amd/csrc/ilqr_kernels.hip
--- a/mind_amd/csrc/ilqr_kernels.hip
+++ b/mind_amd/csrc/ilqr_kernels.hip
@@ -3,6 +3,7 @@
 
 #pragma clang fp contract(off)
 #include "mind_trig.h"
+#include "ilqr_lm.h"
 
 #define IL_NS 6
 #define IL_NU 2
@@ -44,7 +45,9 @@
   unsigned done[IL_SLOTS];
   unsigned sing[IL_SLOTS];
   double Jnew[IL_SLOTS][IL_NA];
-  unsigned sreq, sdone, spad0, spad1;
+  unsigned sreq, sdone, sbdone, ssing;
+  double smu;
+  unsigned sflags, spad0;
 };
 
 struct IlqrTreeDev {
@@ -77,6 +80,7 @@
   GP<const double> field;
   GP<const double> node_w;
   long long dset, drel;
+  long long kset;
   GP<double> h_xs, h_us, h_stats;
   unsigned *h_done;
   unsigned h_gen, pad_h;
@@ -1177,6 +1181,11 @@
   T.dset = -T.dset; T.drel = -T.drel;
 }
 
+__device__ __forceinline__ void il_flip_gains(IlqrTreeDev &T) {
+  T.k.p += T.kset; T.K.p += T.kset; T.Vx.p += T.kset; T.Vxx.p += T.kset;
+  T.kset = -T.kset;
+}
+
 template <bool GEN, bool MULTI, bool SLOTS>
 __device__ __forceinline__ void il_fit(IlqrTreeDev &T, int &cur, const IlqrConst &C, int ph, double *stats, double *trace, int wg, int G, unsigned *bar, unsigned *abort_word) {
   extern __shared__ double il_dsm[];
@@ -1193,6 +1202,7 @@
   __shared__ double sh_mu, sh_delta, sh_J;
   __shared__ int sh_accepted, sh_converged, sh_stop, sh_sing, sh_pick, sh_slot, sh_it, sh_nspec, sh_hint, sh_ntot;
   __shared__ int sh_spec, sh_hit, sh_nreq, sh_nhit;
+  __shared__ int sh_bw, sh_adopt, sh_nbreq, sh_nbhit;
   __shared__ unsigned sh_gen;
   __shared__ unsigned sh_fsing[IL_SLOTS];
   const int tid = threadIdx.x, lane = tid & 63, wave = tid >> 6;
@@ -1206,6 +1216,7 @@
   if (tid == 0) {
     sh_mu = 1.0; sh_delta = 2.0; sh_accepted = 1; sh_converged = 0; sh_stop = 0; sh_J = 0.0; sh_pick = 0; sh_slot = 0; sh_it = 0; sh_hint = 1; sh_ntot = 1;
     sh_spec = 0; sh_hit = 0; sh_nreq = 0; sh_nhit = 0;
+    if (SLOTS) { sh_bw = 0; sh_adopt = 0; sh_nbreq = 0; sh_nbhit = 0; }
     if (SLOTS) sh_gen = __hip_atomic_load(&T.ctl->gen, __ATOMIC_RELAXED, __HIP_MEMORY_SCOPE_AGENT);
   }
   if (MULTI && wg == 0 && tid == 0) {
@@ -1284,12 +1295,20 @@
         __hip_atomic_store(&ctl->cmd, (unsigned)(fol ? sh_ntot : 1) | ((unsigned)ph << 8) | ((unsigned)cur << 24), __ATOMIC_RELAXED, __HIP_MEMORY_SCOPE_AGENT);
         sh_gen += 1u;
         __hip_atomic_store(&ctl->gen, sh_gen, __ATOMIC_RELEASE, __HIP_MEMORY_SCOPE_AGENT);
+        sh_adopt = 0;
+        if (sh_bw == 2) {
+          while (__hip_atomic_load(&ctl->sbdone, __ATOMIC_RELAXED, __HIP_MEMORY_SCOPE_AGENT) != sh_gen - 1u) __builtin_amdgcn_s_sleep(1);
+          __builtin_amdgcn_fence(__ATOMIC_ACQUIRE, "agent");
+          if (!__hip_atomic_load(&ctl->ssing, __ATOMIC_RELAXED, __HIP_MEMORY_SCOPE_AGENT)) { sh_adopt = 1; sh_nbhit += 1; }
+        }
+        sh_bw = 0;
       }
       if (MULTI && wg == 0) __hip_atomic_store(&bar[2 + ((n_pass + 1) & 1)], 0u, __ATOMIC_RELAXED, __HIP_MEMORY_SCOPE_AGENT);
     }
     __syncthreads();
     const int nspec = sh_nspec;
-    for (int d = T.n_slevels - 1; d >= 0; --d) {
+    if (SLOTS && sh_adopt) il_flip_gains(T);
+    for (int d = (SLOTS && sh_adopt) ? -1 : T.n_slevels - 1; d >= 0; --d) {
       const int lo = T.slevel_start[d], hi = T.slevel_start[d + 1];
       for (int w = gw; w < (hi - lo) * nspec; w += nw) {
         const int slot = w / (hi - lo), seg = T.slevel_segs[lo + w % (hi - lo)];
@@ -1380,7 +1399,15 @@
       }
       IL_SYNC();
       if (SLOTS && s == T.n_fsteps - 1 && tid == 0 && sh_spec) {
-        __hip_atomic_store(&T.ctl->sreq, sh_gen, __ATOMIC_RELEASE, __HIP_MEMORY_SCOPE_AGENT);
+        IlSlotCtl *ctl = T.ctl;
+        if (T.kset) {
+          double mu = sh_mu, de = sh_delta;
+          il_accept_update(mu, de);
+          ctl->smu = mu;
+          sh_bw = 1; sh_nbreq += 1;
+        }
+        __hip_atomic_store(&ctl->sflags, (T.kset ? 1u : 0u) | (T.kset > 0 ? 2u : 0u), __ATOMIC_RELAXED, __HIP_MEMORY_SCOPE_AGENT);
+        __hip_atomic_store(&ctl->sreq, sh_gen, __ATOMIC_RELEASE, __HIP_MEMORY_SCOPE_AGENT);
         sh_spec = 2; sh_nreq += 1;
       }
     }
@@ -1451,9 +1478,7 @@
           sh_pick = pick; sh_slot = slot;
           if (fabs((sh_J - Jnew[slot][pick]) / sh_J) < 1e-6) sh_converged = 1;
           sh_accepted = 1;
-          de = fmin(1.0, de) / 2.0;
-          mu *= de;
-          if (mu <= 1e-6) mu = 0.0;
+          il_accept_update(mu, de);
           done = true;
         } else {
           il_reject_update(mu, de);
@@ -1463,6 +1488,7 @@
       sh_mu = mu; sh_delta = de; sh_it = it;
       sh_hint = (sh_accepted && sh_slot == 0) ? 1 : IL_SPEC;
       if (SLOTS && sh_spec == 2 && sh_accepted && sh_slot == 0 && sh_pick == 0) { sh_hit = 1; sh_nhit += 1; }
+      if (SLOTS) sh_bw = (sh_bw && sh_hit && !sh_converged && it < C.max_iter) ? 2 : 0;
     }
     __syncthreads();
     IL_MARK(t_sel);
@@ -1485,6 +1511,7 @@
 #else
     stats[8] = (double)t_roll;
     stats[9] = (double)sh_nreq; stats[10] = (double)sh_nhit;
+    if (SLOTS) { stats[11] = (double)sh_nbreq; stats[12] = (double)sh_nbhit; }
 #endif
     stats[IL_NSTAT - 1] = (double)n_pass;
   }
@@ -1652,12 +1679,16 @@
   double *lsum = il_dsm + (size_t)IL_WAVES * IL_SCR;
   double *recs0 = lsum + IL_LSUM;
   float *dstg = reinterpret_cast<float *>(recs0 + IL_RECS);
-  __shared__ unsigned s_req, s_cmd;
-  const int tid = threadIdx.x;
+  double *scr = il_dsm + (size_t)(threadIdx.x >> 6) * IL_SCR;
+  __shared__ unsigned s_req, s_cmd, s_flags;
+  __shared__ double s_mu;
+  __shared__ int s_sing;
+  const int tid = threadIdx.x, lane = tid & 63, wave = tid >> 6;
   IlSlotCtl *ctl = T0.ctl;
   if (tid == 0) __hip_atomic_fetch_or(&ctl->alive, 1u << wg, __ATOMIC_RELAXED, __HIP_MEMORY_SCOPE_AGENT);
   unsigned last = 0;
   bool staged = false;
+  int ph_cst = -1;
   for (;;) {
     __syncthreads();
     if (tid == 0) {
@@ -1670,6 +1701,7 @@
       }
       __builtin_amdgcn_fence(__ATOMIC_ACQUIRE, "agent");
       s_req = r; s_cmd = __hip_atomic_load(&ctl->cmd, __ATOMIC_RELAXED, __HIP_MEMORY_SCOPE_AGENT);
+      s_flags = __hip_atomic_load(&ctl->sflags, __ATOMIC_RELAXED, __HIP_MEMORY_SCOPE_AGENT); s_mu = ctl->smu; s_sing = 0;
     }
     __syncthreads();
     const unsigned r = s_req, cmd = s_cmd;
@@ -1686,6 +1718,63 @@
     __threadfence_block();
     __syncthreads();
     if (tid == 0) __hip_atomic_store(&ctl->sdone, r, __ATOMIC_RELEASE, __HIP_MEMORY_SCOPE_AGENT);
+    if (!(s_flags & 1u)) continue;
+    const IlqrConst &C = consts[ph];
+    if (ph != ph_cst) {
+      if (lane < 12) scr[IL_CST + lane] = lane == 0 ? 1.0 : (lane == 6 ? C.dt : 0.0);
+      ph_cst = ph;
+    }
+    if (((s_flags >> 1) & 1u) != (T.kset < 0 ? 1u : 0u)) il_flip_gains(T);
+    const double mu = s_mu;
+    for (int d = T.n_slevels - 1; d >= 0; --d) {
+      const int lo = T.slevel_start[d], hi = T.slevel_start[d + 1];
+      for (int w = wave; w < hi - lo; w += IL_WAVES) {
+        const int seg = T.slevel_segs[lo + w];
+        int rec[14];
+        {
+          const int IL_AS1 *sr = T.seg_rec.g() + (size_t)seg * 16;
+#pragma unroll
+          for (int e = 0; e < 14; ++e) rec[e] = __builtin_amdgcn_readfirstlane(sr[e]);
+        }
+        {
+          const int nch = rec[5];
+          double acc = 0.0;
+          if (lane < 42) {
+            double v[6];
+#pragma unroll
+            for (int e = 0; e < 6; ++e) {
+              const int ch = rec[8 + e];
+              v[e] = lane < 36 ? T.Vxx[(size_t)ch * 36 + lane] : T.Vx[(size_t)ch * 6 + (lane - 36)];
+            }
+#pragma unroll
+            for (int e = 0; e < 6; ++e) if (e < nch) acc += v[e];
+            for (int e = rec[6] + 6; e < rec[6] + nch; ++e) {
+              const int ch = T.child_list[e];
+              acc += lane < 36 ? T.Vxx[(size_t)ch * 36 + lane] : T.Vx[(size_t)ch * 6 + (lane - 36)];
+            }
+          }
+          IL_WFENCE();
+          if (lane < 36) scr[36 + lane] = acc;
+          else if (lane < 42) scr[176 + lane - 36] = acc;
+          IL_WFENCE();
+        }
+        const int sing = il_backward_segment<GEN>(C, T, T, rec[0], rec[1], rec[2], rec[4], mu, scr IL_PROF_PASS);
+        if (sing) {
+          if (lane == 0) s_sing = 1;
+        } else {
+          const int c = rec[3];
+          if (lane < 36) T.Vxx[(size_t)c * 36 + lane] = scr[36 + lane];
+          else if (lane < 42) T.Vx[(size_t)c * 6 + lane - 36] = scr[176 + lane - 36];
+        }
+      }
+      __threadfence_block();
+      __syncthreads();
+      if (s_sing) break;
+    }
+    if (tid == 0) {
+      __hip_atomic_store(&ctl->ssing, (unsigned)s_sing, __ATOMIC_RELAXED, __HIP_MEMORY_SCOPE_AGENT);
+      __hip_atomic_store(&ctl->sbdone, r, __ATOMIC_RELEASE, __HIP_MEMORY_SCOPE_AGENT);
+    }
   }
 }
 
@@ -1693,6 +1782,8 @@
 __global__ __launch_bounds__(IL_THREADS) void k_ilqr(const IlqrTreeDev *__restrict__ trees, const IlqrConst *__restrict__ consts,
                                                      int n_phases, int n_trees, int G, unsigned *__restrict__ bars, int spec) {
   constexpr bool MULTI = MODE == 1, SLOTS = MODE == 2;
+  const bool spec_bw = (spec & 2) != 0;
+  spec &= 1;
   int t = blockIdx.x, wg = 0;
   if (MODE != 0) {
     const int Gl = G + (SLOTS ? spec : 0);
@@ -1702,6 +1793,7 @@
     if (t >= n_trees) return;
   }
   IlqrTreeDev T = trees[t];
+  if (!SLOTS || !spec_bw) T.kset = 0;
   if (SLOTS && wg > 0) {
     if (bars[4 * n_trees + 1]) return;
     if (wg >= G) il_speculate<GEN>(T, consts, wg);
diff --git a/mind_amd/csrc/ilqr_lm.h b/mind_amd/csrc/ilqr_lm.h
--- /dev/null
+++ b/mind_amd/csrc/ilqr_lm.h
@@ -0,0 +1,14 @@
+#pragma once
+#include <math.h>
+
+#if defined(__HIPCC__)
+#define IL_LM_FN __host__ __device__ __forceinline__
+#else
+#define IL_LM_FN static inline
+#endif
+
+IL_LM_FN void il_accept_update(double &mu, double &delta) {
+  delta = fmin(1.0, delta) / 2.0;
+  mu *= delta;
+  if (mu <= 1e-6) mu = 0.0;
+}
diff --git a/mind_amd/csrc/mind_hip.hip b/mind_amd/csrc/mind_hip.hip
--- a/mind_amd/csrc/mind_hip.hip
+++ b/mind_amd/csrc/mind_hip.hip
@@ -116,6 +116,8 @@
   struct IlImage { std::vector<double> hD; std::vector<float> hF; std::vector<int> hI; } il_img;
   struct IlEarly { const double *xs = nullptr, *us = nullptr; volatile unsigned *done = nullptr; unsigned gen = 0; int n_trees = 0; long nodes = 0; } il_early;
   unsigned il_gen = 0;
+  long long il_spec_bw_req = 0, il_spec_bw_hit = 0;
+  int il_spec_bw = 1;
   long long il_spec_req = 0, il_spec_hit = 0;
   DevBuf actor_lw_arena;
   std::vector<LwLaunch> actor_lw_plan;
@@ -1081,6 +1083,11 @@
   c->debug_layers = n;
   return MIND_OK;
 }
+extern "C" int mind_debug_set_ilqr_spec_backward(mind_ctx *c, int on) {
+  if (!c) return MIND_EINVAL;
+  c->il_spec_bw = on ? 1 : 0;
+  return MIND_OK;
+}
 extern "C" int64_t mind_debug_read(mind_ctx *c, const char *name, float *host, int64_t max_floats) {
   if (!c || !name) return MIND_EINVAL;
   const void *src = nullptr;
@@ -1101,6 +1108,12 @@
     if (!host) return 2;
     if (max_floats < 2) return MIND_EINVAL;
     host[0] = (float)c->il_spec_req; host[1] = (float)c->il_spec_hit;
+    return 2;
+  }
+  else if (k == "il_spec_bw") {
+    if (!host) return 2;
+    if (max_floats < 2) return MIND_EINVAL;
+    host[0] = (float)c->il_spec_bw_req; host[1] = (float)c->il_spec_bw_hit;
     return 2;
   }
   else if (k.rfind("il_", 0) == 0 && c->il_dbg[5]) {
diff --git a/mind_amd/predictor.py b/mind_amd/predictor.py
--- a/mind_amd/predictor.py
+++ b/mind_amd/predictor.py
@@ -273,6 +273,9 @@
 
     def debug_set_layers(self, n):
         _lib.check(self.lib, self.ctx, self.lib.mind_debug_set_layers(self.ctx, n), "mind_debug_set_layers")
+
+    def debug_set_ilqr_spec_backward(self, on):
+        _lib.check(self.lib, self.ctx, self.lib.mind_debug_set_ilqr_spec_backward(self.ctx, 1 if on else 0), "mind_debug_set_ilqr_spec_backward")
 
     def debug_read(self, name):
         n = self.lib.mind_debug_read(self.ctx, name.encode(), None, 0)
```

After: 1908, median of 6. 1.01x the previous value.
